# fateshelled/onnx_image_processing

Hardware: AMD Instinct MI355X
Metric: image-pairs/sec (640x480, K=512) (higher is better)
Workload: dtype f32; 1 GPU; Shi-Tomasi(3) + NMS(r=5)/top-k + sparse BAD(512, hard) + Sinkhorn(20, eps 0.05) + MNN(100, 0.1), 640x480 gray pairs, K=512 (BASELINE configs[1]); height=480, width=640, max_keypoints=512, parallelism=pair-sharded x1, input=float32 frames resident in HBM

## Files before the change

### include/mi355x_match.h

```cpp
#ifndef MI355X_MATCH_H
#define MI355X_MATCH_H

#include <stddef.h>
#include <stdint.h>

#define MI_API __attribute__((visibility("default")))

#ifdef __cplusplus
extern "C" {
#endif

typedef void *mi_stream_t;

enum {
  MI_OK = 0,
  MI_E_NULL = -1,
  MI_E_SHAPE = -2,
  MI_E_PARAM = -3,
  MI_E_CAPACITY = -4,
  MI_E_ALIGN = -5
};

enum { MI_BAD_RAW = 0, MI_BAD_SOFT = 1, MI_BAD_HARD = 2 };
enum { MI_DIST_L2 = 0, MI_DIST_L1 = 1 };
#define MI_DOTS_MIN_EPSILON 0.005
enum {
  MI_SOLVER_DEFAULT = 0,
  MI_SOLVER_MULTI_LAUNCH = 1,
  MI_SOLVER_NO_FORK = 2,
  MI_SOLVER_DOTS_BELOW_1024 = 4
};
enum {
  MI_SCHEDULE_UNDECIDED = -1,
  MI_SCHEDULE_CALLER_HELPER = 0,
  MI_SCHEDULE_TWO_HELPERS = 1,
  MI_SCHEDULE_UNSPLIT = 2
};

MI_API int mi_abi_version(void);
MI_API const char *mi_error_string(int code);
MI_API int mi_release_stream_resources(mi_stream_t stream);
MI_API int mi_sinkhorn_dots_schedule(mi_stream_t stream, int batch, int n, int m, int iterations);
MI_API int mi_sinkhorn_dots_set_schedule(mi_stream_t stream, int schedule);

MI_API int mi_corner_response(const float *image, int n, int h, int w, int block_size, float *score,
                       mi_stream_t stream);
MI_API int mi_corner_response_u8(const uint8_t *image, int n, int h, int w, int block_size, float *score,
                          mi_stream_t stream);
MI_API int mi_convert_u8_f32(const uint8_t *src, long long count, float *dst, mi_stream_t stream);
#define MI_TILE_COUNTER_BYTES 16640
MI_API int mi_corner_response_balanced(const void *image, int pixels_are_u8, int n, int h, int w, int block_size, float *score,
                                uint32_t *tile_counter, mi_stream_t stream);
MI_API int mi_corner_response_pair(const void *image_a, const void *image_b, int pixels_are_u8, int per_set, int h, int w,
                            int block_size, float *score, uint32_t *tile_counter, mi_stream_t stream);

MI_API int mi_nms_mask(const float *score, int n, int h, int w, int radius, float *mask, mi_stream_t stream);

MI_API int mi_candidate_layout(int h, int w, int *segments, int *segment_capacity);
MI_API int mi_nms_candidates(const float *score, int n, int h, int w, int radius, float score_threshold,
                      int border_margin, uint64_t *cand, uint32_t *count, mi_stream_t stream);
MI_API int mi_select_candidates(const float *score, const float *mask, int n, int h, int w,
                         float score_threshold, int border_margin, uint64_t *cand, uint32_t *count,
                         mi_stream_t stream);

MI_API int mi_topk_keypoints(const uint64_t *cand, const uint32_t *count, int segments, int segment_capacity,
                      int n, int w, int k, float *keypoints, float *kscores, mi_stream_t stream);

MI_API size_t mi_bad_plan_bytes(int num_pairs);
MI_API int mi_bad_plan_build(const uint32_t *pair_geom, const float *pair_thr, int num_pairs, void *plan,
                      mi_stream_t stream);
MI_API int mi_sparse_bad(const float *image, int n, int h, int w, const float *keypoints, int k,
                  const uint32_t *pair_geom, const float *pair_thr, int num_pairs, int mode,
                  float temperature, int normalize, float *desc, uint32_t *bits, const void *plan,
                  uint8_t *status, mi_stream_t stream);

MI_API int mi_sparse_bad_u8(const uint8_t *image, int n, int h, int w, const float *keypoints, int k,
                     const uint32_t *pair_geom, const float *pair_thr, int num_pairs, int mode,
                     float temperature, int normalize, float *desc, uint32_t *bits, const void *plan,
                     uint8_t *status, mi_stream_t stream);
MI_API int mi_sparse_bad_pair(const void *image_a, const void *image_b, int pixels_are_u8, int per_set, int h, int w,
                       const float *keypoints, int k, const uint32_t *pair_geom, const float *pair_thr, int num_pairs,
                       int mode, float temperature, int normalize, float *desc, uint32_t *bits, const void *plan,
                       uint8_t *status, mi_stream_t stream);

MI_API int mi_bad_dense(const float *image, int n, int h, int w, const uint32_t *pair_geom, const float *pair_thr,
                 int num_pairs, int mode, float temperature, float *out, mi_stream_t stream);
MI_API int mi_bad_dense_oriented(const float *image, const float *orientation, int n, int h, int w,
                          const uint32_t *pair_geom, const float *pair_thr, int num_pairs, int mode,
                          float temperature, float *out, mi_stream_t stream);
MI_API int mi_gather_descriptors(const float *descriptor_map, int batch, int d, int h, int w, const float *keypoints,
                          int nk, int bilinear, float *out, mi_stream_t stream);

MI_API int mi_angle_map(const float *image, int n, int h, int w, int patch_size, const float *moment_kernels,
                 float *angle, mi_stream_t stream);
MI_API int mi_angle_at_keypoints(const float *image, int n, int h, int w, const float *keypoints, int k,
                          int patch_size, const float *moment_kernels, float *theta, mi_stream_t stream);
MI_API int mi_angle_at_keypoints_pair(const float *image_a, const float *image_b, int per_set, int h, int w,
                               const float *keypoints, int k, int patch_size, const float *moment_kernels, float *theta,
                               mi_stream_t stream);

MI_API int mi_sparse_bad_oriented(const float *image, int n, int h, int w, const float *keypoints, int k,
                           const float *orientation_map, const float *keypoint_angles,
                           const uint32_t *pair_geom, const float *pair_thr, int num_pairs, int mode,
                           float temperature, int normalize, int bilinear, float max_reach, float *desc,
                           uint32_t *bits, uint8_t *status, mi_stream_t stream);
MI_API int mi_sparse_bad_oriented_pair(const float *image_a, const float *image_b, int per_set, int h, int w,
                                const float *keypoints, int k, const float *keypoint_angles, const uint32_t *pair_geom,
                                const float *pair_thr, int num_pairs, int mode, float temperature, int normalize,
                                int bilinear, float max_reach, float *desc, uint32_t *bits, uint8_t *status,
                                mi_stream_t stream);

MI_API int mi_cost_logscores_bits(const uint32_t *bits1, const uint32_t *bits2, int batch, int n, int m,
                           int num_bits, int normalized, double epsilon, float *z, int pitch,
                           mi_stream_t stream);
MI_API int mi_cost_logscores_f32(const float *desc1, const float *desc2, int batch, int n, int m, int d,
                          int distance, double epsilon, float *z, int pitch, mi_stream_t stream);

MI_API size_t mi_sinkhorn_workspace_bytes(int batch, int n, int m);
MI_API int mi_sinkhorn(const float *z, int batch, int n, int m, int pitch, float dustbin_logscore,
                int iterations, float *u, float *v, float *p, void *workspace, size_t workspace_bytes,
                mi_stream_t stream);

MI_API int mi_cost_dots_bits(const uint32_t *bits1, const uint32_t *bits2, int batch, int n, int m, int num_bits,
                      int normalized, uint16_t *dots, int pitch, float *row_info, float *col_info,
                      mi_stream_t stream);
MI_API size_t mi_sinkhorn_dots_workspace_bytes(int batch, int n, int m);
MI_API int mi_sinkhorn_dots(const uint16_t *dots, const float *row_info, const float *col_info, int batch, int n,
                     int m, int pitch, double epsilon, double unused_score, double sqnorm_bound, int iterations,
                     float *u, float *v, float *p, void *workspace, size_t workspace_bytes, int flags,
                     mi_stream_t stream);
MI_API const uint32_t *mi_sinkhorn_dots_status_word(const void *workspace, int batch, int n, int m);

MI_API int mi_match_filters(float *p, int batch, int n, int m, float ratio_threshold, float dustbin_margin,
                     uint8_t *valid, mi_stream_t stream);
MI_API int mi_match_filter_masks(const float *p, int batch, int n, int m, int has_dustbin, float ratio_threshold,
                          float dustbin_margin, uint8_t *valid, mi_stream_t stream);

MI_API int mi_mnn_extract(const float *p, int batch, int n, int m, const float *kpts1, const float *kpts2,
                   int max_matches, float threshold, uint64_t *row_best, uint64_t *col_best,
                   float *mk1, float *mk2, float *scores, uint8_t *valid, int32_t *match_ij,
                   mi_stream_t stream);

MI_API size_t mi_mnn_duals_workspace_bytes(int batch, int n, int m);
MI_API int mi_mnn_from_duals(const float *z, int batch, int n, int m, int pitch, const float *u, const float *v,
                      const float *kpts1, const float *kpts2, int max_matches, float threshold, void *workspace,
                      size_t workspace_bytes, float *mk1, float *mk2, float *scores, uint8_t *valid,
                      int32_t *match_ij, mi_stream_t stream);
MI_API int mi_mnn_from_duals_dots(const uint16_t *dots, const float *row_info, const float *col_info, int batch, int n,
                           int m, int pitch, double epsilon, const float *u, const float *v, const float *kpts1,
                           const float *kpts2, int max_matches, float threshold, void *workspace,
                           size_t workspace_bytes, const uint32_t *solver_status, float *mk1, float *mk2,
                           float *scores, uint8_t *valid, int32_t *match_ij, mi_stream_t stream);

MI_API int mi_akaze_diffuse(const float *l_in, int n, int h, int w, float kappa, float dt, float *l_out,
                     mi_stream_t stream);
#define MI_AKAZE_KAPPA_MIN 1e-3f
#define MI_AKAZE_KAPPA_MAX 1e6f
MI_API int mi_akaze_scale_fused(int iterations, int nms_size);
MI_API int mi_akaze_scale(const float *l_in, int n, int h, int w, int iterations, float kappa, float dt, float threshold,
                   int nms_size, float *l_out, float *scores, float *tmp, mi_stream_t stream);
MI_API int mi_akaze_scale_sets(const float *l_in_a, const float *l_in_b, int per_set, int h, int w, int iterations,
                        float kappa, float dt, float threshold, int nms_size, float *l_out, float *scores, float *tmp,
                        mi_stream_t stream);
MI_API int mi_akaze_scale_select(const float *l_in, int n, int h, int w, int iterations, float kappa, float dt,
                          float threshold, int nms_size, float *l_out, const float *prev_scores, int num_prev,
                          float *best, uint8_t *attain, float *tmp, mi_stream_t stream);
MI_API int mi_akaze_orientation_from_attain(const uint8_t *attain, const float *scale_theta, int num_scales, int n, int h,
                                     int w, const float *keypoints, int k, float *theta, mi_stream_t stream);
MI_API int mi_akaze_orientation_select(const float *scale_images, size_t scale_stride, int num_scales,
                                const uint8_t *attain, int n, int h, int w, const float *keypoints, int k,
                                int patch_size, const float *moment_kernels, float *theta, mi_stream_t stream);
MI_API int mi_akaze_hessian_scores(const float *l, int n, int h, int w, float threshold, int nms_size, float *scores,
                            mi_stream_t stream);
MI_API int mi_akaze_combine(const float *scale_scores, const float *scale_orientations, int num_scales, int n, int h,
                     int w, float *scores, float *orientations, mi_stream_t stream);
MI_API int mi_akaze_orientation_at_keypoints(const float *scale_scores, const float *scale_theta, int num_scales,
                                      int n, int h, int w, const float *keypoints, int k, float *theta,
                                      mi_stream_t stream);

MI_API int mi_core_maxima(const float *p, int batch, int n, int m, float *row_max, float *col_max, mi_stream_t stream);

MI_API int mi_normalise_keypoints(const float *keypoints, long long count, const float *k_inv, float *points,
                           mi_stream_t stream);

MI_API size_t mi_essential_matrix_workspace_bytes(int batch, int n, int m, int top_k);
MI_API int mi_essential_matrix(const float *p, int batch, int n, int m, const float *pts1, const float *pts2,
                        const uint8_t *valid1, const uint8_t *valid2, int top_k, int n_iter,
                        int n_iter_manifold, float *e, void *workspace, size_t workspace_bytes, mi_stream_t stream);
MI_API int mi_essential_matrix_dots(const uint16_t *dots, const float *row_info, const float *col_info, int pitch,
                             double epsilon, const float *u, const float *v, int batch, int n, int m,
                             const float *pts1, const float *pts2, const uint8_t *valid1, const uint8_t *valid2,
                             int top_k, int n_iter, int n_iter_manifold, float *e, void *workspace,
                             size_t workspace_bytes, mi_stream_t stream);

MI_API int mi_fast_score(const float *image, int n, int h, int w, float threshold, float *score, mi_stream_t stream);
MI_API int mi_dog_responses(const float *image, int n, int h, int w, const float *weights_1d, int num_scales,
                     int kernel_size, float *out, float *score, mi_stream_t stream);

typedef struct mi_match_params {
  int block_size;
  int nms_radius;
  int max_keypoints;
  float score_threshold;
  int border_margin;
  int num_pairs;
  const uint32_t *pair_geom;
  const float *pair_thr;
  const void *bad_plan;
  int normalize_descriptors;
  double epsilon;
  double unused_score;
  int sinkhorn_iterations;
  int max_matches;
  float match_threshold;
  int flags;
} mi_match_params;
MI_API size_t mi_match_pairs_workspace_bytes(int batch, int h, int w, const mi_match_params *params);
MI_API int mi_match_pairs(const float *image1, const float *image2, int batch, int h, int w,
                   const mi_match_params *params, float *keypoints1, float *keypoints2, float *matched1,
                   float *matched2, float *match_scores, uint8_t *match_valid, int32_t *match_ij,
                   void *workspace, size_t workspace_bytes, mi_stream_t stream);

MI_API int mi_match_pairs_u8(const uint8_t *image1, const uint8_t *image2, int batch, int h, int w,
                      const mi_match_params *params, float *keypoints1, float *keypoints2, float *matched1,
                      float *matched2, float *match_scores, uint8_t *match_valid, int32_t *match_ij,
                      void *workspace, size_t workspace_bytes, mi_stream_t stream);

MI_API size_t mi_voxel_downsample_workspace_bytes(int batch, int64_t total, int d);
MI_API int mi_voxel_downsample(const float *points, const int64_t *offsets, int batch, int64_t total, int d,
                               const float *leaf, float *out_points, uint8_t *out_mask, int64_t *out_counts,
                               void *workspace, size_t workspace_bytes, mi_stream_t stream);

MI_API int mi_depth_to_points(const void *depth, int depth_is_u16, int batch, int h, int w, const float *u_tab,
                              const float *v_tab, float z_scale, float *out_points, float *out_normals,
                              mi_stream_t stream);

MI_API int mi_depth_align(const void *depth, int depth_is_u16, int batch, int h, int w, const float *u_tab,
                          const float *v_tab, float z_scale, float rgb_cx, float rgb_cy, float rgb_fx, float rgb_fy,
                          const float *rotation, const float *translation, float *out, mi_stream_t stream);

enum { MI_PIX_U8 = 0, MI_PIX_U16 = 1, MI_PIX_I32 = 2, MI_PIX_F32 = 3 };
#define MI_THRESHOLD_MAX_BINS 65536
#define MI_THRESHOLD_MAX_CLASSES 5

MI_API int mi_histogram(const void *frames, int dtype, int batch, long long pixels, int min_val, int bins, int64_t *hist,
                        mi_stream_t stream);

MI_API int mi_otsu_threshold(const int64_t *hist, int batch, int bins, int min_val, int32_t *thresh, mi_stream_t stream);

MI_API size_t mi_multi_otsu_workspace_bytes(int batch, int bins, int n_class);
MI_API int mi_multi_otsu_threshold(const int64_t *hist, int batch, int bins, int min_val, int n_class, int32_t *thresholds,
                                   void *workspace, size_t workspace_bytes, mi_stream_t stream);

MI_API int mi_threshold_apply(const void *frames, int dtype, int batch, long long pixels, const int32_t *thresholds,
                              int n_thresh, int out_dtype, int binary, int low, int high, void *out, mi_stream_t stream);

#define MI_POSE_MAX_N 2048
#define MI_POSE_MAX_HYPOTHESES 65536
#define MI_POSE_MAX_REFINE_ROUNDS 8

MI_API int mi_essential_hypotheses(const float *pts1, const float *pts2, const uint8_t *valid, int batch, int n,
                                   int num_hypotheses, float threshold, uint32_t seed, float *e_h, float *cost,
                                   int32_t *count, mi_stream_t stream);

MI_API int mi_essential_refit(const float *pts1, const float *pts2, const uint8_t *mask, int batch, int n, float *e,
                              uint8_t *ok, mi_stream_t stream);

MI_API size_t mi_essential_ransac_workspace_bytes(int batch, int n, int num_hypotheses);
MI_API int mi_essential_ransac(const float *pts1, const float *pts2, const uint8_t *valid, int batch, int n,
                               int num_hypotheses, float threshold, int refine_rounds, uint32_t seed, float *e,
                               uint8_t *inlier, int32_t *best_h, int32_t *count, void *workspace, size_t workspace_bytes,
                               mi_stream_t stream);

MI_API int mi_recover_pose(const float *e, const float *pts1, const float *pts2, const uint8_t *mask, int batch, int n,
                           float distance_threshold, float *r, float *t, uint8_t *pose_mask, int32_t *count, uint8_t *ok,
                           mi_stream_t stream);

MI_API int mi_triangulate(const float *proj1, const float *proj2, const float *pts1, const float *pts2, int batch, int n,
                          float *points, uint8_t *finite, mi_stream_t stream);

enum { MI_INGEST_BGR = 0, MI_INGEST_RGB = 1 };
#define MI_INGEST_MAX_DIM 16384
MI_API int mi_ingest_frames(const uint8_t *src, int batch, int src_h, int src_w, int channels, long long row_pitch,
                            long long frame_pitch, int channel_order, void *dst, int dst_is_f32, int h, int w,
                            mi_stream_t stream);

#define MI_RIGID_MAX_N 2048

MI_API int mi_lift_keypoints(const float *keypoints, const void *depth, int depth_is_u16, int batch, int n, int h, int w,
                             const float *k_inv, float z_scale, float min_depth, float max_depth, const uint8_t *valid_in,
                             float *points, uint8_t *valid, mi_stream_t stream);

MI_API int mi_rigid_hypotheses(const float *pts1, const float *pts2, const uint8_t *valid, int batch, int n,
                               int num_hypotheses, float threshold, uint32_t seed, float *rt_h, float *cost, int32_t *count,
                               mi_stream_t stream);

MI_API int mi_rigid_refit(const float *pts1, const float *pts2, const uint8_t *mask, int batch, int n, float *r, float *t,
                          uint8_t *ok, mi_stream_t stream);

MI_API size_t mi_rigid_ransac_workspace_bytes(int batch, int n, int num_hypotheses);
MI_API int mi_rigid_ransac(const float *pts1, const float *pts2, const uint8_t *valid, int batch, int n, int num_hypotheses,
                           float threshold, int refine_rounds, uint32_t seed, float *r, float *t, uint8_t *inlier,
                           int32_t *best_h, int32_t *count, float *rmse, uint8_t *ok, void *workspace, size_t workspace_bytes,
                           mi_stream_t stream);

#define MI_ICP_MAX_STAGES 4
#define MI_ICP_MAX_ITERATIONS 64

MI_API int mi_surfel_maps(const void *depth, int depth_is_u16, int batch, int h, int w, const float *k_inv, float z_scale,
                          float min_depth, float max_depth, float normal_max_jump, float *vertex_out, float *normal_out,
                          mi_stream_t stream);

MI_API size_t mi_icp_workspace_bytes(int batch, int h, int w);

MI_API int mi_icp_linearise(const float *vertex1, const float *normal1, const float *vertex2, const float *normal2,
                            const float *r, const float *t, int batch, int h, int w, float fx, float fy, float cx, float cy,
                            int stride, float distance_threshold, float angle_threshold, double *sums, void *workspace,
                            size_t workspace_bytes, mi_stream_t stream);

MI_API int mi_icp_refine(const float *vertex1, const float *normal1, const float *vertex2, const float *normal2,
                         const float *r0, const float *t0, int batch, int h, int w, float fx, float fy, float cx, float cy,
                         const int32_t *strides, const int32_t *iterations, int stages, float distance_threshold,
                         float angle_threshold, int min_correspondences, float *r, float *t, float *information, float *rmse,
                         int32_t *count, int32_t *steps, uint8_t *ok, void *workspace, size_t workspace_bytes,
                         mi_stream_t stream);


MI_API int mi_intensity_maps(const void *gray, int gray_is_u8, int batch, int h, int w, float *intensity_out, mi_stream_t stream);

MI_API size_t mi_rgbd_workspace_bytes(int batch, int h, int w);

MI_API int mi_photo_linearise(const float *vertex1, const float *intensity1, const float *vertex2, const float *intensity2,
                              const float *r, const float *t, int batch, int h, int w, float fx, float fy, float cx, float cy,
                              int stride, float distance_threshold, float intensity_threshold, double *sums, void *workspace,
                              size_t workspace_bytes, mi_stream_t stream);

MI_API int mi_rgbd_refine(const float *vertex1, const float *normal1, const float *intensity1, const float *vertex2,
                          const float *normal2, const float *intensity2, const float *r0, const float *t0, int batch, int h,
                          int w, float fx, float fy, float cx, float cy, const int32_t *strides, const int32_t *iterations,
                          int stages, float distance_threshold, float angle_threshold, float photo_weight,
                          float intensity_threshold, int min_correspondences, float *r, float *t, float *information,
                          float *rmse, int32_t *count, float *rmse_photo, int32_t *count_photo, int32_t *steps, uint8_t *ok,
                          void *workspace, size_t workspace_bytes, mi_stream_t stream);


MI_API int mi_tsdf_reset(float *volume, int batch, int nz, int ny, int nx, mi_stream_t stream);

MI_API int mi_tsdf_integrate(float *volume, int batch, int nz, int ny, int nx, float origin_x, float origin_y, float origin_z,
                             float voxel_size, float truncation, float max_weight, const void *depth, int depth_is_u16, int frames,
                             int h, int w, float fx, float fy, float cx, float cy, float z_scale, float min_depth, float max_depth,
                             const float *r, const float *t, const uint8_t *active, mi_stream_t stream);

MI_API int mi_tsdf_raycast(const float *volume, int batch, int nz, int ny, int nx, float origin_x, float origin_y, float origin_z,
                           float voxel_size, float truncation, float step_fraction, const float *r, const float *t, int h, int w,
                           const float *k_inv, float min_depth, float max_depth, float *vertex_out, float *normal_out,
                           mi_stream_t stream);

MI_API int mi_pose_compose(const float *ra, const float *ta, const float *rb, const float *tb, int batch, float *r, float *t,
                           mi_stream_t stream);


MI_API size_t mi_tsdf_surface_workspace_bytes(int batch, int nz, int ny, int nx);

MI_API int mi_tsdf_surface(const float *volume, int batch, int nz, int ny, int nx, float origin_x, float origin_y, float origin_z,
                           float voxel_size, float min_weight, int max_vertices, int max_triangles, float *vertex_out,
                           float *normal_out, int32_t *triangle_out, int32_t *counts_out, void *workspace, size_t workspace_bytes,
                           mi_stream_t stream);


MI_API int mi_tsdf_gray_reset(float *intensity_volume, int batch, int nz, int ny, int nx, mi_stream_t stream);

MI_API int mi_tsdf_integrate_gray(float *volume, float *intensity_volume, int batch, int nz, int ny, int nx, float origin_x,
                                  float origin_y, float origin_z, float voxel_size, float truncation, float max_weight,
                                  const void *depth, int depth_is_u16, const void *gray, int gray_is_u8, int frames, int h, int w,
                                  float fx, float fy, float cx, float cy, float z_scale, float min_depth, float max_depth,
                                  const float *r, const float *t, const uint8_t *active, mi_stream_t stream);

MI_API int mi_tsdf_sample_gray(const float *intensity_volume, int batch, int nz, int ny, int nx, float origin_x, float origin_y,
                               float origin_z, float voxel_size, const float *points, int n, const float *r, const float *t,
                               float *intensity_out, mi_stream_t stream);

#define MI_PNP_MAX_N 2048

MI_API int mi_pnp_hypotheses(const float *pts3, const float *pts2, const uint8_t *valid, int batch, int n, int num_hypotheses,
                             float threshold, uint32_t seed, float *rt_h, float *cost, int32_t *count, mi_stream_t stream);

MI_API int mi_pnp_refit(const float *pts3, const float *pts2, const uint8_t *mask, const float *r0, const float *t0, int batch,
                        int n, float *r, float *t, float *info, uint8_t *ok, mi_stream_t stream);

MI_API size_t mi_pnp_ransac_workspace_bytes(int batch, int n, int num_hypotheses);
MI_API int mi_pnp_ransac(const float *pts3, const float *pts2, const uint8_t *valid, int batch, int n, int num_hypotheses,
                         float threshold, int refine_rounds, uint32_t seed, float *r, float *t, uint8_t *inlier,
                         int32_t *best_h, int32_t *count, float *rmse, float *info, uint8_t *ok, void *workspace,
                         size_t workspace_bytes, mi_stream_t stream);

#ifdef __cplusplus
}
#endif
#endif
```

### onnx_image_processing_amd/_native.py

```python
from __future__ import annotations

import ctypes
import os
from ctypes import c_char_p, c_double, c_float, c_int, c_size_t, c_uint32, c_void_p

import torch

_PKG = os.path.dirname(os.path.abspath(__file__))
LIB_PATH = os.environ.get("MI355X_MATCH_LIB") or os.path.join(_PKG, "lib", "libmi355x_match.so")

SIGNATURES = {
    "mi_abi_version": [],
    "mi_sinkhorn_dots_schedule": [c_void_p, c_int, c_int, c_int, c_int],
    "mi_sinkhorn_dots_set_schedule": [c_void_p, c_int],
    "mi_error_string": [c_int],
    "mi_release_stream_resources": [c_void_p],
    "mi_corner_response": [c_void_p, c_int, c_int, c_int, c_int, c_void_p, c_void_p],
    "mi_corner_response_u8": [c_void_p, c_int, c_int, c_int, c_int, c_void_p, c_void_p],
    "mi_convert_u8_f32": [c_void_p, ctypes.c_longlong, c_void_p, c_void_p],
    "mi_corner_response_balanced": [c_void_p, c_int, c_int, c_int, c_int, c_int, c_void_p, c_void_p, c_void_p],
    "mi_corner_response_pair": [c_void_p, c_void_p, c_int, c_int, c_int, c_int, c_int, c_void_p, c_void_p, c_void_p],
    "mi_nms_mask": [c_void_p, c_int, c_int, c_int, c_int, c_void_p, c_void_p],
    "mi_candidate_layout": [c_int, c_int, ctypes.POINTER(c_int), ctypes.POINTER(c_int)],
    "mi_nms_candidates": [c_void_p, c_int, c_int, c_int, c_int, c_float, c_int, c_void_p, c_void_p, c_void_p],
    "mi_select_candidates": [c_void_p, c_void_p, c_int, c_int, c_int, c_float, c_int, c_void_p, c_void_p, c_void_p],
    "mi_topk_keypoints": [c_void_p, c_void_p, c_int, c_int, c_int, c_int, c_int, c_void_p, c_void_p, c_void_p],
    "mi_bad_plan_bytes": [c_int],
    "mi_bad_plan_build": [c_void_p, c_void_p, c_int, c_void_p, c_void_p],
    "mi_sparse_bad": [c_void_p, c_int, c_int, c_int, c_void_p, c_int, c_void_p, c_void_p, c_int, c_int, c_float, c_int,
                      c_void_p, c_void_p, c_void_p, c_void_p, c_void_p],
    "mi_sparse_bad_u8": [c_void_p, c_int, c_int, c_int, c_void_p, c_int, c_void_p, c_void_p, c_int, c_int, c_float, c_int,
                         c_void_p, c_void_p, c_void_p, c_void_p, c_void_p],
    "mi_sparse_bad_pair": [c_void_p, c_void_p, c_int, c_int, c_int, c_int, c_void_p, c_int, c_void_p, c_void_p, c_int, c_int,
                           c_float, c_int, c_void_p, c_void_p, c_void_p, c_void_p, c_void_p],
    "mi_bad_dense": [c_void_p, c_int, c_int, c_int, c_void_p, c_void_p, c_int, c_int, c_float, c_void_p, c_void_p],
    "mi_bad_dense_oriented": [c_void_p, c_void_p, c_int, c_int, c_int, c_void_p, c_void_p, c_int, c_int, c_float, c_void_p,
                              c_void_p],
    "mi_gather_descriptors": [c_void_p, c_int, c_int, c_int, c_int, c_void_p, c_int, c_int, c_void_p, c_void_p],
    "mi_angle_map": [c_void_p, c_int, c_int, c_int, c_int, c_void_p, c_void_p, c_void_p],
    "mi_angle_at_keypoints": [c_void_p, c_int, c_int, c_int, c_void_p, c_int, c_int, c_void_p, c_void_p, c_void_p],
    "mi_sparse_bad_oriented": [c_void_p, c_int, c_int, c_int, c_void_p, c_int, c_void_p, c_void_p, c_void_p, c_void_p,
                               c_int, c_int, c_float, c_int, c_int, c_float, c_void_p, c_void_p, c_void_p, c_void_p],
    "mi_angle_at_keypoints_pair": [c_void_p, c_void_p, c_int, c_int, c_int, c_void_p, c_int, c_int, c_void_p, c_void_p,
                                   c_void_p],
    "mi_sparse_bad_oriented_pair": [c_void_p, c_void_p, c_int, c_int, c_int, c_void_p, c_int, c_void_p, c_void_p, c_void_p,
                                    c_int, c_int, c_float, c_int, c_int, c_float, c_void_p, c_void_p, c_void_p, c_void_p],
    "mi_cost_logscores_bits": [c_void_p, c_void_p, c_int, c_int, c_int, c_int, c_int, c_double, c_void_p, c_int, c_void_p],
    "mi_cost_logscores_f32": [c_void_p, c_void_p, c_int, c_int, c_int, c_int, c_int, c_double, c_void_p, c_int, c_void_p],
    "mi_sinkhorn_workspace_bytes": [c_int, c_int, c_int],
    "mi_sinkhorn": [c_void_p, c_int, c_int, c_int, c_int, c_float, c_int, c_void_p, c_void_p, c_void_p, c_void_p,
                    c_size_t, c_void_p],
    "mi_cost_dots_bits": [c_void_p, c_void_p, c_int, c_int, c_int, c_int, c_int, c_void_p, c_int, c_void_p, c_void_p,
                          c_void_p],
    "mi_sinkhorn_dots_workspace_bytes": [c_int, c_int, c_int],
    "mi_sinkhorn_dots": [c_void_p, c_void_p, c_void_p, c_int, c_int, c_int, c_int, c_double, c_double, c_double, c_int,
                         c_void_p, c_void_p, c_void_p, c_void_p, c_size_t, c_int, c_void_p],
    "mi_sinkhorn_dots_status_word": [c_void_p, c_int, c_int, c_int],
    "mi_match_filters": [c_void_p, c_int, c_int, c_int, c_float, c_float, c_void_p, c_void_p],
    "mi_match_filter_masks": [c_void_p, c_int, c_int, c_int, c_int, c_float, c_float, c_void_p, c_void_p],
    "mi_mnn_extract": [c_void_p, c_int, c_int, c_int, c_void_p, c_void_p, c_int, c_float, c_void_p, c_void_p,
                       c_void_p, c_void_p, c_void_p, c_void_p, c_void_p, c_void_p],
    "mi_mnn_duals_workspace_bytes": [c_int, c_int, c_int],
    "mi_mnn_from_duals": [c_void_p, c_int, c_int, c_int, c_int, c_void_p, c_void_p, c_void_p, c_void_p, c_int, c_float,
                          c_void_p, c_size_t, c_void_p, c_void_p, c_void_p, c_void_p, c_void_p, c_void_p],
    "mi_mnn_from_duals_dots": [c_void_p, c_void_p, c_void_p, c_int, c_int, c_int, c_int, c_double, c_void_p, c_void_p,
                               c_void_p, c_void_p, c_int, c_float, c_void_p, c_size_t, c_void_p, c_void_p, c_void_p,
                               c_void_p, c_void_p, c_void_p, c_void_p],
    "mi_core_maxima": [c_void_p, c_int, c_int, c_int, c_void_p, c_void_p, c_void_p],
    "mi_normalise_keypoints": [c_void_p, ctypes.c_longlong, c_void_p, c_void_p, c_void_p],
    "mi_essential_matrix_workspace_bytes": [c_int, c_int, c_int, c_int],
    "mi_essential_matrix": [c_void_p, c_int, c_int, c_int, c_void_p, c_void_p, c_void_p, c_void_p, c_int, c_int, c_int,
                            c_void_p, c_void_p, c_size_t, c_void_p],
    "mi_essential_matrix_dots": [c_void_p, c_void_p, c_void_p, c_int, c_double, c_void_p, c_void_p, c_int, c_int, c_int,
                                 c_void_p, c_void_p, c_void_p, c_void_p, c_int, c_int, c_int, c_void_p, c_void_p, c_size_t,
                                 c_void_p],
    "mi_fast_score": [c_void_p, c_int, c_int, c_int, c_float, c_void_p, c_void_p],
    "mi_dog_responses": [c_void_p, c_int, c_int, c_int, c_void_p, c_int, c_int, c_void_p, c_void_p, c_void_p],
    "mi_akaze_diffuse": [c_void_p, c_int, c_int, c_int, c_float, c_float, c_void_p, c_void_p],
    "mi_akaze_scale_fused": [c_int, c_int],
    "mi_akaze_scale": [c_void_p, c_int, c_int, c_int, c_int, c_float, c_float, c_float, c_int, c_void_p, c_void_p, c_void_p,
                       c_void_p],
    "mi_akaze_scale_sets": [c_void_p, c_void_p, c_int, c_int, c_int, c_int, c_float, c_float, c_float, c_int, c_void_p, c_void_p,
                            c_void_p, c_void_p],
    "mi_akaze_scale_select": [c_void_p, c_int, c_int, c_int, c_int, c_float, c_float, c_float, c_int, c_void_p, c_void_p,
                              c_int, c_void_p, c_void_p, c_void_p, c_void_p],
    "mi_akaze_orientation_from_attain": [c_void_p, c_void_p, c_int, c_int, c_int, c_int, c_void_p, c_int, c_void_p,
                                         c_void_p],
    "mi_akaze_orientation_select": [c_void_p, c_size_t, c_int, c_void_p, c_int, c_int, c_int, c_void_p, c_int, c_int,
                                    c_void_p, c_void_p, c_void_p],
    "mi_akaze_hessian_scores": [c_void_p, c_int, c_int, c_int, c_float, c_int, c_void_p, c_void_p],
    "mi_akaze_combine": [c_void_p, c_void_p, c_int, c_int, c_int, c_int, c_void_p, c_void_p, c_void_p],
    "mi_akaze_orientation_at_keypoints": [c_void_p, c_void_p, c_int, c_int, c_int, c_int, c_void_p, c_int, c_void_p,
                                          c_void_p],
    "mi_voxel_downsample_workspace_bytes": [c_int, ctypes.c_int64, c_int],
    "mi_voxel_downsample": [c_void_p, c_void_p, c_int, ctypes.c_int64, c_int, c_void_p, c_void_p, c_void_p, c_void_p,
                            c_void_p, c_size_t, c_void_p],
    "mi_depth_to_points": [c_void_p, c_int, c_int, c_int, c_int, c_void_p, c_void_p, c_float, c_void_p, c_void_p, c_void_p],
    "mi_depth_align": [c_void_p, c_int, c_int, c_int, c_int, c_void_p, c_void_p, c_float, c_float, c_float, c_float, c_float,
                       c_void_p, c_void_p, c_void_p, c_void_p],
    "mi_histogram": [c_void_p, c_int, c_int, ctypes.c_longlong, c_int, c_int, c_void_p, c_void_p],
    "mi_otsu_threshold": [c_void_p, c_int, c_int, c_int, c_void_p, c_void_p],
    "mi_multi_otsu_workspace_bytes": [c_int, c_int, c_int],
    "mi_multi_otsu_threshold": [c_void_p, c_int, c_int, c_int, c_int, c_void_p, c_void_p, c_size_t, c_void_p],
    "mi_threshold_apply": [c_void_p, c_int, c_int, ctypes.c_longlong, c_void_p, c_int, c_int, c_int, c_int, c_int, c_void_p,
                           c_void_p],
    "mi_essential_hypotheses": [c_void_p, c_void_p, c_void_p, c_int, c_int, c_int, c_float, c_uint32, c_void_p, c_void_p,
                                c_void_p, c_void_p],
    "mi_essential_refit": [c_void_p, c_void_p, c_void_p, c_int, c_int, c_void_p, c_void_p, c_void_p],
    "mi_essential_ransac_workspace_bytes": [c_int, c_int, c_int],
    "mi_essential_ransac": [c_void_p, c_void_p, c_void_p, c_int, c_int, c_int, c_float, c_int, c_uint32, c_void_p, c_void_p,
                            c_void_p, c_void_p, c_void_p, c_size_t, c_void_p],
    "mi_recover_pose": [c_void_p, c_void_p, c_void_p, c_void_p, c_int, c_int, c_float, c_void_p, c_void_p, c_void_p, c_void_p,
                        c_void_p, c_void_p],
    "mi_triangulate": [c_void_p, c_void_p, c_void_p, c_void_p, c_int, c_int, c_void_p, c_void_p, c_void_p],
    "mi_ingest_frames": [c_void_p, c_int, c_int, c_int, c_int, ctypes.c_longlong, ctypes.c_longlong, c_int, c_void_p, c_int,
                         c_int, c_int, c_void_p],
    "mi_lift_keypoints": [c_void_p, c_void_p, c_int, c_int, c_int, c_int, c_int, c_void_p, c_float, c_float, c_float, c_void_p,
                          c_void_p, c_void_p, c_void_p],
    "mi_rigid_hypotheses": [c_void_p, c_void_p, c_void_p, c_int, c_int, c_int, c_float, c_uint32, c_void_p, c_void_p, c_void_p,
                            c_void_p],
    "mi_rigid_refit": [c_void_p, c_void_p, c_void_p, c_int, c_int, c_void_p, c_void_p, c_void_p, c_void_p],
    "mi_rigid_ransac_workspace_bytes": [c_int, c_int, c_int],
    "mi_rigid_ransac": [c_void_p, c_void_p, c_void_p, c_int, c_int, c_int, c_float, c_int, c_uint32, c_void_p, c_void_p, c_void_p,
                        c_void_p, c_void_p, c_void_p, c_void_p, c_void_p, c_size_t, c_void_p],
    "mi_pnp_hypotheses": [c_void_p, c_void_p, c_void_p, c_int, c_int, c_int, c_float, c_uint32, c_void_p, c_void_p, c_void_p,
                          c_void_p],
    "mi_pnp_refit": [c_void_p, c_void_p, c_void_p, c_void_p, c_void_p, c_int, c_int, c_void_p, c_void_p, c_void_p, c_void_p,
                     c_void_p],
    "mi_pnp_ransac_workspace_bytes": [c_int, c_int, c_int],
    "mi_pnp_ransac": [c_void_p, c_void_p, c_void_p, c_int, c_int, c_int, c_float, c_int, c_uint32, c_void_p, c_void_p, c_void_p,
                      c_void_p, c_void_p, c_void_p, c_void_p, c_void_p, c_void_p, c_size_t, c_void_p],
    "mi_surfel_maps": [c_void_p, c_int, c_int, c_int, c_int, c_void_p, c_float, c_float, c_float, c_float, c_void_p, c_void_p,
                       c_void_p],
    "mi_icp_workspace_bytes": [c_int, c_int, c_int],
    "mi_icp_linearise": [c_void_p, c_void_p, c_void_p, c_void_p, c_void_p, c_void_p, c_int, c_int, c_int, c_float, c_float,
                         c_float, c_float, c_int, c_float, c_float, c_void_p, c_void_p, c_size_t, c_void_p],
    "mi_icp_refine": [c_void_p, c_void_p, c_void_p, c_void_p, c_void_p, c_void_p, c_int, c_int, c_int, c_float, c_float, c_float,
                      c_float, c_void_p, c_void_p, c_int, c_float, c_float, c_int, c_void_p, c_void_p, c_void_p, c_void_p,
                      c_void_p, c_void_p, c_void_p, c_void_p, c_size_t, c_void_p],
    "mi_intensity_maps": [c_void_p, c_int, c_int, c_int, c_int, c_void_p, c_void_p],
    "mi_rgbd_workspace_bytes": [c_int, c_int, c_int],
    "mi_photo_linearise": [c_void_p, c_void_p, c_void_p, c_void_p, c_void_p, c_void_p, c_int, c_int, c_int, c_float, c_float,
                           c_float, c_float, c_int, c_float, c_float, c_void_p, c_void_p, c_size_t, c_void_p],
    "mi_rgbd_refine": [c_void_p, c_void_p, c_void_p, c_void_p, c_void_p, c_void_p, c_void_p, c_void_p, c_int, c_int, c_int,
                       c_float, c_float, c_float, c_float, c_void_p, c_void_p, c_int, c_float, c_float, c_float, c_float, c_int,
                       c_void_p, c_void_p, c_void_p, c_void_p, c_void_p, c_void_p, c_void_p, c_void_p, c_void_p, c_void_p,
                       c_size_t, c_void_p],
    "mi_tsdf_reset": [c_void_p, c_int, c_int, c_int, c_int, c_void_p],
    "mi_tsdf_integrate": [c_void_p, c_int, c_int, c_int, c_int, c_float, c_float, c_float, c_float, c_float, c_float, c_void_p,
                          c_int, c_int, c_int, c_int, c_float, c_float, c_float, c_float, c_float, c_float, c_float, c_void_p,
                          c_void_p, c_void_p, c_void_p],
    "mi_tsdf_raycast": [c_void_p, c_int, c_int, c_int, c_int, c_float, c_float, c_float, c_float, c_float, c_float, c_void_p,
                        c_void_p, c_int, c_int, c_void_p, c_float, c_float, c_void_p, c_void_p, c_void_p],
    "mi_pose_compose": [c_void_p, c_void_p, c_void_p, c_void_p, c_int, c_void_p, c_void_p, c_void_p],
    "mi_tsdf_surface_workspace_bytes": [c_int, c_int, c_int, c_int],
    "mi_tsdf_surface": [c_void_p, c_int, c_int, c_int, c_int, c_float, c_float, c_float, c_float, c_float, c_int, c_int, c_void_p,
                        c_void_p, c_void_p, c_void_p, c_void_p, c_size_t, c_void_p],
    "mi_tsdf_gray_reset": [c_void_p, c_int, c_int, c_int, c_int, c_void_p],
    "mi_tsdf_integrate_gray": [c_void_p, c_void_p, c_int, c_int, c_int, c_int, c_float, c_float, c_float, c_float, c_float, c_float,
                               c_void_p, c_int, c_void_p, c_int, c_int, c_int, c_int, c_float, c_float, c_float, c_float, c_float,
                               c_float, c_float, c_void_p, c_void_p, c_void_p, c_void_p],
    "mi_tsdf_sample_gray": [c_void_p, c_int, c_int, c_int, c_int, c_float, c_float, c_float, c_float, c_void_p, c_int, c_void_p,
                            c_void_p, c_void_p, c_void_p],
}


class MatchParams(ctypes.Structure):
    _fields_ = [("block_size", c_int), ("nms_radius", c_int), ("max_keypoints", c_int), ("score_threshold", c_float),
                ("border_margin", c_int), ("num_pairs", c_int), ("pair_geom", c_void_p), ("pair_thr", c_void_p),
                ("bad_plan", c_void_p), ("normalize_descriptors", c_int), ("epsilon", c_double),
                ("unused_score", c_double), ("sinkhorn_iterations", c_int), ("max_matches", c_int),
                ("match_threshold", c_float), ("flags", c_int)]


SIGNATURES["mi_match_pairs_workspace_bytes"] = [c_int, c_int, c_int, ctypes.POINTER(MatchParams)]
SIGNATURES["mi_match_pairs"] = [c_void_p, c_void_p, c_int, c_int, c_int, ctypes.POINTER(MatchParams), c_void_p, c_void_p,
                                c_void_p, c_void_p, c_void_p, c_void_p, c_void_p, c_void_p, c_size_t, c_void_p]
DEBUG_SIGNATURES = {"mi_debug_set": [c_int, c_int], "mi_debug_topk_stamps": [c_void_p], "mi_debug_clock_probe": [c_void_p],
                    "mi_debug_bad_plan_passes": [c_void_p, c_int, ctypes.POINTER(c_int), ctypes.POINTER(c_int)],
                    "mi_debug_sinkhorn_dots_form": [c_int, c_int, c_int, c_int, c_int, c_int],
                    "mi_debug_tuner_script": [c_int, ctypes.POINTER(c_int), ctypes.POINTER(c_int), ctypes.POINTER(ctypes.c_double), ctypes.POINTER(c_int)],
                    "mi_debug_akaze_math_check": [c_int, c_float, c_uint32, c_uint32, c_void_p, c_void_p, c_void_p]}
SIGNATURES["mi_match_pairs_u8"] = SIGNATURES["mi_match_pairs"]
_RESTYPE = {"mi_essential_matrix_workspace_bytes": c_size_t, "mi_sinkhorn_dots_status_word": c_void_p, "mi_match_pairs_workspace_bytes": c_size_t, "mi_error_string": c_char_p, "mi_sinkhorn_workspace_bytes": c_size_t, "mi_bad_plan_bytes": c_size_t,
            "mi_sinkhorn_dots_workspace_bytes": c_size_t, "mi_mnn_duals_workspace_bytes": c_size_t,
            "mi_voxel_downsample_workspace_bytes": c_size_t, "mi_multi_otsu_workspace_bytes": c_size_t,
            "mi_essential_ransac_workspace_bytes": c_size_t, "mi_rigid_ransac_workspace_bytes": c_size_t,
            "mi_pnp_ransac_workspace_bytes": c_size_t,
            "mi_icp_workspace_bytes": c_size_t, "mi_rgbd_workspace_bytes": c_size_t, "mi_tsdf_surface_workspace_bytes": c_size_t}

MI_BAD_RAW, MI_BAD_SOFT, MI_BAD_HARD = 0, 1, 2
MI_DIST_L2, MI_DIST_L1 = 0, 1
MI_PIX_U8, MI_PIX_U16, MI_PIX_I32, MI_PIX_F32 = 0, 1, 2, 3
MI_INGEST_BGR, MI_INGEST_RGB = 0, 1

DEBUG_LIB_PATH = os.path.join(_PKG, "lib", "libmi355x_match_debug.so")

_lib = None
_product = None
_debug = None


def _open(path: str, signatures: dict) -> ctypes.CDLL:
    if not os.path.exists(path):
        raise RuntimeError(
            f"{path} not found: the HIP library is not built. Run "
            "`python -m onnx_image_processing_amd.build` (there is no CPU fallback)."
        )
    lib = ctypes.CDLL(path)
    for name, argtypes in signatures.items():
        fn = getattr(lib, name)
        fn.argtypes = argtypes
        fn.restype = _RESTYPE.get(name, c_int)
    return lib


def load() -> ctypes.CDLL:
    global _lib, _product
    if _lib is None:
        if _product is None:
            _product = _open(LIB_PATH, SIGNATURES)
        _lib = _product
    return _lib


class debug_library:

    def __enter__(self) -> ctypes.CDLL:
        global _lib, _debug
        load()
        if _debug is None:
            _debug = _open(DEBUG_LIB_PATH, {**SIGNATURES, **DEBUG_SIGNATURES})
        self._outer = _lib
        _lib = _debug
        return _debug

    def __exit__(self, *exc) -> None:
        global _lib
        _debug.mi_debug_set(0, 0)
        _lib = self._outer


def use_debug_library() -> ctypes.CDLL:
    return debug_library().__enter__()


def check(code: int, what: str) -> None:
    if code != 0:
        msg = load().mi_error_string(code)
        raise RuntimeError(f"{what} failed ({code}): {msg.decode() if msg else '?'}")


def stream_ptr() -> int:
    return torch.cuda.current_stream().cuda_stream


def dev(t: torch.Tensor, dtype: torch.dtype, what: str) -> int:
    if not t.is_cuda:
        raise RuntimeError(
            f"{what} must live on the GPU (got device {t.device}); this package has no CPU path"
        )
    if t.dtype != dtype:
        raise RuntimeError(f"{what} must be {dtype}, got {t.dtype}")
    if not t.is_contiguous():
        raise RuntimeError(f"{what} must be contiguous")
    return t.data_ptr()


_timers: dict | None = None


_timed_names = None


def enable_timing(on: bool, only=None) -> None:
    global _timers, _timed_names
    _timers = {} if on else None
    _timed_names = set(only) if (on and only) else None


def timings_ms() -> dict:
    torch.cuda.synchronize()
    return {k: [s.elapsed_time(e) for s, e in v] for k, v in (_timers or {}).items()}


def call(name: str, *args) -> None:
    fn = getattr(load(), name)
    if _timers is None or (_timed_names is not None and name not in _timed_names):
        check(fn(*args), name)
        return
    start, end = torch.cuda.Event(enable_timing=True), torch.cuda.Event(enable_timing=True)
    start.record()
    rc = fn(*args)
    end.record()
    check(rc, name)
    _timers.setdefault(name, []).append((start, end))
```

### onnx_image_processing_amd/csrc/common.h

```cpp
#pragma once
#include <hip/hip_runtime.h>
#include <stdint.h>

#include "../../include/mi355x_match.h"

#define MI_WAVE 64

#define MI_ENTER() (void)hipGetLastError()
static inline int mi_launch_status() {
  hipError_t e = hipGetLastError();
  return e == hipSuccess ? MI_OK : (int)e;
}
#define MI_CHECK_LAUNCH()                          \
  do {                                             \
    const int _mi_e = mi_launch_status();          \
    if (_mi_e != MI_OK) return _mi_e;              \
  } while (0)

static inline int ceil_div(int a, int b) { return (a + b - 1) / b; }

template <typename W>
static __global__ __launch_bounds__(256) void mi_zero_kernel(W *__restrict__ p, size_t n) {
  const size_t i = (size_t)blockIdx.x * 256 + threadIdx.x;
  if (i < n) p[i] = W{};
}
static inline int mi_zero_async(void *p, size_t bytes, hipStream_t s) {
  if (bytes == 0) return MI_OK;
  if (((uintptr_t)p % 4) != 0 || bytes % 4 != 0) return MI_E_ALIGN;
  if (((uintptr_t)p % 16) == 0 && bytes % 16 == 0) {
    const size_t n = bytes / 16;
    hipLaunchKernelGGL(mi_zero_kernel<uint4>, dim3((unsigned)((n + 255) / 256)), dim3(256), 0, s, reinterpret_cast<uint4 *>(p), n);
  } else {
    const size_t n = bytes / 4;
    hipLaunchKernelGGL(mi_zero_kernel<uint32_t>, dim3((unsigned)((n + 255) / 256)), dim3(256), 0, s, reinterpret_cast<uint32_t *>(p), n);
  }
  return mi_launch_status();
}

struct MiSets {
  const void *a;
  const void *b;
  int per_set;
};
static inline MiSets mi_one_set(const void *p, int n) { return MiSets{p, nullptr, n}; }
template <typename T>
__device__ __forceinline__ const T *mi_set_item(const MiSets &s, int i, size_t item_elems) {
  const bool second = i >= s.per_set;
  return static_cast<const T *>(second ? s.b : s.a) + (size_t)(second ? i - s.per_set : i) * item_elems;
}

__device__ __forceinline__ int clampi(int v, int lo, int hi) { return v < lo ? lo : (v > hi ? hi : v); }

__device__ __forceinline__ unsigned xcd_contiguous_id(unsigned bid, unsigned nblocks) {
  const unsigned q = nblocks >> 3, r = nblocks & 7u;
  const unsigned xcd = bid & 7u, k = bid >> 3;
  const unsigned base = (xcd < r) ? xcd * (q + 1u) : r * (q + 1u) + (xcd - r) * q;
  return base + k;
}

#define MI_DPP(old, src, ctrl, rmask) \
  __builtin_bit_cast(float, __builtin_amdgcn_update_dpp(__builtin_bit_cast(int, old), __builtin_bit_cast(int, src), ctrl, rmask, 0xf, false))
__device__ __forceinline__ float wave_max_dpp(float v) {
  v = fmaxf(v, MI_DPP(v, v, 0xB1, 0xf));
  v = fmaxf(v, MI_DPP(v, v, 0x4E, 0xf));
  v = fmaxf(v, MI_DPP(v, v, 0x141, 0xf));
  v = fmaxf(v, MI_DPP(v, v, 0x140, 0xf));
  v = fmaxf(v, MI_DPP(v, v, 0x142, 0xa));
  v = fmaxf(v, MI_DPP(v, v, 0x143, 0xc));
  return __builtin_bit_cast(float, __builtin_amdgcn_readlane(__builtin_bit_cast(int, v), 63));
}
__device__ __forceinline__ float wave_sum_dpp(float v) {
  v += MI_DPP(0.0f, v, 0xB1, 0xf);
  v += MI_DPP(0.0f, v, 0x4E, 0xf);
  v += MI_DPP(0.0f, v, 0x141, 0xf);
  v += MI_DPP(0.0f, v, 0x140, 0xf);
  v += MI_DPP(0.0f, v, 0x142, 0xa);
  v += MI_DPP(0.0f, v, 0x143, 0xc);
  return __builtin_bit_cast(float, __builtin_amdgcn_readlane(__builtin_bit_cast(int, v), 63));
}

#define MI_SWAP32(a, b, ra, rb)                                                                              \
  {                                                                                                           \
    auto _r = __builtin_amdgcn_permlane32_swap(__builtin_bit_cast(unsigned, a), __builtin_bit_cast(unsigned, b), \
                                               false, false);                                                \
    const unsigned _r0 = _r[0], _r1 = _r[1];  \
    ra = __builtin_bit_cast(float, _r0);                                                                      \
    rb = __builtin_bit_cast(float, _r1);                                                                      \
  }
#define MI_SWAP16(a, b, ra, rb)                                                                              \
  {                                                                                                           \
    auto _r = __builtin_amdgcn_permlane16_swap(__builtin_bit_cast(unsigned, a), __builtin_bit_cast(unsigned, b), \
                                               false, false);                                                \
    const unsigned _r0 = _r[0], _r1 = _r[1];                                                                  \
    ra = __builtin_bit_cast(float, _r0);                                                                      \
    rb = __builtin_bit_cast(float, _r1);                                                                      \
  }
__device__ __forceinline__ float mi_readlane_f(float v, int lane) {
  return __builtin_bit_cast(float, __builtin_amdgcn_readlane(__builtin_bit_cast(int, v), lane));
}
__device__ __forceinline__ void wave_max4(float *v) {
  float a0, a1, b0, b1, c0, c1;
  MI_SWAP32(v[0], v[1], a0, a1);
  MI_SWAP32(v[2], v[3], b0, b1);
  const float m01 = fmaxf(a0, a1), m23 = fmaxf(b0, b1);
  MI_SWAP16(m01, m23, c0, c1);
  float m = fmaxf(c0, c1);
  m = fmaxf(m, MI_DPP(m, m, 0xB1, 0xf));
  m = fmaxf(m, MI_DPP(m, m, 0x4E, 0xf));
  m = fmaxf(m, MI_DPP(m, m, 0x141, 0xf));
  m = fmaxf(m, MI_DPP(m, m, 0x140, 0xf));
  v[0] = mi_readlane_f(m, 0);
  v[2] = mi_readlane_f(m, 16);
  v[1] = mi_readlane_f(m, 32);
  v[3] = mi_readlane_f(m, 48);
}
#define MI_ROW_OF_GROUP(g) ((g) == 1 ? 2 : (g) == 2 ? 1 : (g))
__device__ __forceinline__ float wave_sum4_rows(const float *v) {
  float a0, a1, b0, b1, c0, c1;
  MI_SWAP32(v[0], v[1], a0, a1);
  MI_SWAP32(v[2], v[3], b0, b1);
  const float m01 = a0 + a1, m23 = b0 + b1;
  MI_SWAP16(m01, m23, c0, c1);
  float m = c0 + c1;
  m += MI_DPP(0.0f, m, 0xB1, 0xf);
  m += MI_DPP(0.0f, m, 0x4E, 0xf);
  m += MI_DPP(0.0f, m, 0x141, 0xf);
  m += MI_DPP(0.0f, m, 0x140, 0xf);
  return m;
}
__device__ __forceinline__ void wave_sum4(float *v) {
  float a0, a1, b0, b1, c0, c1;
  MI_SWAP32(v[0], v[1], a0, a1);
  MI_SWAP32(v[2], v[3], b0, b1);
  const float m01 = a0 + a1, m23 = b0 + b1;
  MI_SWAP16(m01, m23, c0, c1);
  float m = c0 + c1;
  m += MI_DPP(0.0f, m, 0xB1, 0xf);
  m += MI_DPP(0.0f, m, 0x4E, 0xf);
  m += MI_DPP(0.0f, m, 0x141, 0xf);
  m += MI_DPP(0.0f, m, 0x140, 0xf);
  v[0] = mi_readlane_f(m, 0);
  v[2] = mi_readlane_f(m, 16);
  v[1] = mi_readlane_f(m, 32);
  v[3] = mi_readlane_f(m, 48);
}

__device__ __forceinline__ float mi_prob_exp(float t) { return __builtin_amdgcn_exp2f(t * 1.4426950408889634f); }

__device__ __forceinline__ float mi_z_from_dot(float dot, float2 row, float2 col, float neg_inv_eps) {
  return __builtin_fmaf(dot * col.x, -2.0f * neg_inv_eps * row.x, col.y * neg_inv_eps) + row.y * neg_inv_eps;
}

__device__ __forceinline__ float wave_max(float v) {
#pragma unroll
  for (int o = 32; o > 0; o >>= 1) v = fmaxf(v, __shfl_xor(v, o, 64));
  return v;
}
__device__ __forceinline__ float wave_sum(float v) {
#pragma unroll
  for (int o = 32; o > 0; o >>= 1) v += __shfl_xor(v, o, 64);
  return v;
}

static inline bool mi_akaze_kappa_ok(float kappa) { return kappa >= MI_AKAZE_KAPPA_MIN && kappa <= MI_AKAZE_KAPPA_MAX; }
#define MI_AKAZE_STREAM_MAX_PREV 3
int mi_akaze_stream_supported(int h, int w, int iterations, int nms_size, const void *l_in, const void *l_out,
                              const void *scores);
int mi_akaze_scale_stream(const float *l_in, const float *l_in_b, int per_set, int n, int h, int w, int iterations, float kappa, float dt, float threshold,
                          int nms_size, float *l_out, float *scores, int mode, const float *prev_scores, int num_prev,
                          uint8_t *attain, mi_stream_t stream);

int mi_corner_response_sets(MiSets images, int pix_u8, int n, int h, int w, int block_size, float *score,
                            unsigned *tile_ctr, mi_stream_t stream);
int mi_topk_keypoints_sets(const uint64_t *cand, const uint32_t *count, int segments, int segment_capacity, int n, int w,
                           int k, MiSets keypoints, float *kscores, mi_stream_t stream);
int mi_sparse_bad_sets(MiSets images, int pix_u8, int n, int h, int w, MiSets keypoints, int k, const uint32_t *pair_geom,
                       const float *pair_thr, int num_pairs, int mode, float temperature, int normalize, float *desc,
                       uint32_t *bits, const void *plan, uint8_t *status, mi_stream_t stream);
int mi_cost_dots_bits_zeroing(const uint32_t *bits1, const uint32_t *bits2, int batch, int n, int m, int num_bits,
                              int normalized, uint16_t *dots, int pitch, float *row_info, float *col_info,
                              void *zero_ptr, size_t zero_bytes, mi_stream_t stream);
size_t mi_sinkhorn_dots_handoff_region(void *workspace, int batch, int n, int m, int flags, void **region);
int mi_sinkhorn_dots_impl(const uint16_t *dots, const float *row_info, const float *col_info, int batch, int n, int m,
                          int pitch, double epsilon, double unused_score, double sqnorm_bound, int iterations, float *u,
                          float *v, float *p, void *workspace, size_t workspace_bytes, int flags, int prezeroed,
                          mi_stream_t stream);

struct MiFork {
  int parts;
  hipStream_t stream[2];
  void *handle;
  int trial_entry, trial, first_side;
};
int mi_fork_begin(hipStream_t s, int batch, int n, int m, int key, MiFork *f);
int mi_fork_end(hipStream_t s, MiFork *f);
```

### onnx_image_processing_amd/csrc/mnn.hip

```cpp
#include "common.h"
#include "hooks.h"

#include <math.h>

namespace {

constexpr int MX_THREADS = 1024;
constexpr int MX_MAX = 4096;

__device__ __forceinline__ uint64_t best_key(float p, uint32_t idx) {
  return ((uint64_t)__float_as_uint(p) << 32) | (uint64_t)(0xFFFFFFFFu - idx);
}
__device__ __forceinline__ uint64_t wave_max_u64(uint64_t k) {
#pragma unroll
  for (int o = 32; o > 0; o >>= 1) {
    const uint64_t other = __shfl_xor(k, o, 64);
    k = other > k ? other : k;
  }
  return k;
}

__global__ __launch_bounds__(256) void mnn_row_kernel(const float *__restrict__ p, int n, int m,
                                                      uint64_t *__restrict__ row_best) {
  const int lane = threadIdx.x & 63, wave = threadIdx.x >> 6;
  const int b = blockIdx.y, i = blockIdx.x * 4 + wave;
  if (i >= n) return;
  const float *pr = p + ((size_t)b * (n + 1) + i) * (size_t)(m + 1);
  uint64_t k = 0ull;
  for (int j = lane; j < m; j += 64) {
    const uint64_t c = best_key(pr[j], (uint32_t)j);
    k = c > k ? c : k;
  }
  k = wave_max_u64(k);
  if (lane == 0) row_best[(size_t)b * n + i] = k;
}

__global__ __launch_bounds__(256) void mnn_col_kernel(const float *__restrict__ p, int n, int m,
                                                      uint64_t *__restrict__ col_best) {
  __shared__ uint64_t red[4][64];
  const int lane = threadIdx.x & 63, wave = threadIdx.x >> 6;
  const int b = blockIdx.y, j = blockIdx.x * 64 + lane;
  const float *pb = p + (size_t)b * (n + 1) * (size_t)(m + 1);
  uint64_t k = 0ull;
  if (j < m) {
    for (int i = wave; i < n; i += 4) {
      const uint64_t c = best_key(pb[(size_t)i * (m + 1) + j], (uint32_t)i);
      k = c > k ? c : k;
    }
  }
  red[wave][lane] = k;
  __syncthreads();
  if (wave == 0 && j < m) {
    for (int w = 1; w < 4; ++w) k = red[w][lane] > k ? red[w][lane] : k;
    col_best[(size_t)b * m + j] = k;
  }
}

template <int Q>
__global__ __launch_bounds__(512) void mnn_p_kernel(const float *__restrict__ p, int n, int m, uint64_t *__restrict__ row_best,
                                                    unsigned long long *__restrict__ col_best) {
  constexpr int NW = 8, RW = 4;
  __shared__ uint64_t red[NW][Q * 64];
  const int lane = threadIdx.x & 63, wave = __builtin_amdgcn_readfirstlane(threadIdx.x >> 6);
  const int b = blockIdx.y, row0 = ((int)blockIdx.x * NW + wave) * RW;
  float x[RW][Q];
#pragma unroll
  for (int r = 0; r < RW; ++r) {
    const float *pr = p + ((size_t)b * (n + 1) + min(row0 + r, n - 1)) * (size_t)(m + 1);
#pragma unroll
    for (int q = 0; q < Q; ++q) x[r][q] = pr[min(q * 64 + lane, m - 1)];
  }
  float cbest[Q];
  int cidx[Q];
#pragma unroll
  for (int q = 0; q < Q; ++q) { cbest[q] = -1.0f; cidx[q] = 0; }
#pragma unroll
  for (int r = 0; r < RW; ++r) {
    const int i = row0 + r;
    const bool live = i < n;
    float rbest = -1.0f;
    int rj = 0;
#pragma unroll
    for (int q = 0; q < Q; ++q) {
      const int j = q * 64 + lane;
      const float v = (live && j < m) ? x[r][q] : -1.0f;
      if (v > rbest) { rbest = v; rj = j; }
      if (v > cbest[q]) { cbest[q] = v; cidx[q] = i; }
    }
    uint64_t key = rbest >= 0.0f ? best_key(rbest, (uint32_t)rj) : 0ull;
    key = wave_max_u64(key);
    if (lane == 0 && live) row_best[(size_t)b * n + i] = key;
  }
#pragma unroll
  for (int q = 0; q < Q; ++q) red[wave][q * 64 + lane] = cbest[q] >= 0.0f ? best_key(cbest[q], (uint32_t)cidx[q]) : 0ull;
  __syncthreads();
  for (int c = threadIdx.x; c < Q * 64 && c < m; c += 64 * NW) {
    uint64_t k = red[0][c];
#pragma unroll
    for (int w = 1; w < NW; ++w) k = red[w][c] > k ? red[w][c] : k;
    if (k != 0ull) atomicMax(col_best + (size_t)b * m + c, (unsigned long long)k);
  }
}

__global__ __launch_bounds__(MX_THREADS) void mnn_select_kernel(
    int n, int m, const uint64_t *__restrict__ row_best, const uint64_t *__restrict__ col_best,
    const uint64_t *__restrict__ col_part, int nb,
    const float *__restrict__ kpts1, const float *__restrict__ kpts2, int max_matches, float threshold,
    const uint32_t *__restrict__ solver_status,
    float *__restrict__ mk1, float *__restrict__ mk2, float *__restrict__ scores,
    uint8_t *__restrict__ valid, int32_t *__restrict__ match_ij) {
  __shared__ uint64_t keys[MX_MAX];
  const bool dead = solver_status && *solver_status != 0u;
  __shared__ uint64_t cmerged[1024];
  const int t = threadIdx.x, b = blockIdx.x;
  const uint64_t *rb = row_best + (size_t)b * n;
  const uint64_t *cb = col_best + (size_t)b * m;
  if (col_part) {
    for (int j = t; j < m; j += MX_THREADS) {
      uint64_t k = 0ull;
      int band = 0;
      for (; band + 8 <= nb; band += 8) {
        uint64_t c[8];
#pragma unroll
        for (int q = 0; q < 8; ++q) c[q] = col_part[((size_t)b * nb + band + q) * m + j];
#pragma unroll
        for (int q = 0; q < 8; ++q) k = c[q] > k ? c[q] : k;
      }
      for (; band < nb; ++band) {
        const uint64_t c = col_part[((size_t)b * nb + band) * m + j];
        k = c > k ? c : k;
      }
      cmerged[j] = k;
    }
    __syncthreads();
    cb = cmerged;
  }
  int npad = 2;
  while (npad < n) npad <<= 1;
  for (int i = t; i < npad; i += MX_THREADS) {
    uint64_t key = 0ull;
    if (i < n) {
      const uint64_t r = rb[i];
      const uint32_t jw = 0xFFFFFFFFu - (uint32_t)(r & 0xFFFFFFFFull);
      const bool has = r != 0ull && jw < (uint32_t)m;
      const uint32_t j = has ? jw : 0u;
      const float val = __uint_as_float((uint32_t)(r >> 32));
      const uint32_t ib = 0xFFFFFFFFu - (uint32_t)(cb[j] & 0xFFFFFFFFull);
      const bool ok = has && !dead && (ib == (uint32_t)i) && (val >= threshold);
      key = ((uint64_t)(ok ? (uint32_t)(r >> 32) + 1u : 0u) << 32) | (uint64_t)(0xFFFFFFFFu - (uint32_t)i);
    }
    keys[i] = key;
  }
  __syncthreads();
  const uint64_t *sorted = keys;
  if (npad >= 128 && npad <= MX_THREADS) {
    uint64_t *ordered = keys + MX_THREADS;
    uint32_t *above_of = reinterpret_cast<uint32_t *>(keys + 2 * MX_THREADS);
    const int tpk = MX_THREADS / npad, slice = npad / tpk;
    const int ki = t & (npad - 1), part = t / npad;
    if (t < npad) { above_of[t] = 0u; ordered[t] = 0ull; }
    const uint64_t mine = keys[ki];
    uint32_t above = 0;
    if (mine != 0ull) {
      const ulonglong2 *lst = reinterpret_cast<const ulonglong2 *>(keys + part * slice);
#pragma unroll 8
      for (int j = 0; j < slice / 2; ++j) {
        const ulonglong2 two = lst[j];
        above += (two.x > mine ? 1u : 0u) + (two.y > mine ? 1u : 0u);
      }
    }
    __syncthreads();
    if (mine != 0ull && above) atomicAdd(&above_of[ki], above);
    __syncthreads();
    if (part == 0 && mine != 0ull) ordered[above_of[ki]] = mine;
    __syncthreads();
    sorted = ordered;
  } else {
    for (int size = 2; size <= npad; size <<= 1) {
      for (int stride = size >> 1; stride > 0; stride >>= 1) {
        for (int i = t; i < (npad >> 1); i += MX_THREADS) {
          const int pos = 2 * i - (i & (stride - 1));
          const int par = pos + stride;
          const bool desc = ((pos & size) == 0);
          const uint64_t a = keys[pos], c = keys[par];
          if ((a < c) == desc) { keys[pos] = c; keys[par] = a; }
        }
        __syncthreads();
      }
    }
  }
  const int cnt = max_matches < n ? max_matches : n;
  for (int s = t; s < max_matches; s += MX_THREADS) {
    float sc = 0.0f;
    uint32_t i = 0;
    bool matched = false;
    if (s < cnt) {
      const uint64_t key = sorted[s];
      i = 0xFFFFFFFFu - (uint32_t)(key & 0xFFFFFFFFull);
      const uint32_t hi = (uint32_t)(key >> 32);
      matched = hi != 0u;
      sc = matched ? __uint_as_float(hi - 1u) : -1.0f;
    }
    const uint32_t jw = 0xFFFFFFFFu - (uint32_t)(rb[i] & 0xFFFFFFFFull);
    const uint32_t j = jw < (uint32_t)m ? jw : 0u;
    const size_t o = (size_t)b * max_matches + s;
    mk1[o * 2 + 0] = kpts1[((size_t)b * n + i) * 2 + 0];
    mk1[o * 2 + 1] = kpts1[((size_t)b * n + i) * 2 + 1];
    mk2[o * 2 + 0] = kpts2[((size_t)b * m + j) * 2 + 0];
    mk2[o * 2 + 1] = kpts2[((size_t)b * m + j) * 2 + 1];
    scores[o] = sc;
    const bool ok = sc > 0.0f;
    valid[o] = ok ? 1 : 0;
    if (match_ij) {
      match_ij[o * 2 + 0] = ok ? (int32_t)i : -1;
      match_ij[o * 2 + 1] = ok ? (int32_t)j : -1;
    }
  }
}

struct ZSourceF32 {
  const float *z;
  int pitch;
  struct Raw { float4 a, c; };
  struct Row {};
  __device__ __forceinline__ Raw load_raw(int b, int n, int i, int j, int m) const {
    const float *src = z + ((size_t)b * n + i) * pitch + j;
    Raw r;
    r.a = make_float4(0.f, 0.f, 0.f, 0.f);
    r.c = r.a;
    if (j < m) r.a = *reinterpret_cast<const float4 *>(src);
    if (j + 4 < m) r.c = *reinterpret_cast<const float4 *>(src + 4);
    return r;
  }
  __device__ __forceinline__ void decode(const Raw &r, float (&out)[8]) const {
    out[0] = r.a.x; out[1] = r.a.y; out[2] = r.a.z; out[3] = r.a.w;
    out[4] = r.c.x; out[5] = r.c.y; out[6] = r.c.z; out[7] = r.c.w;
  }
  __device__ __forceinline__ Row load_row(int, int, int) const { return Row(); }
  __device__ __forceinline__ void begin_row(const Row &) {}
  __device__ __forceinline__ float col(int, int) const { return 0.0f; }
  __device__ __forceinline__ void finish(float (&)[8], const float2 (&)[8]) const {}
};

struct ZSourceDots {
  const uint16_t *dots;
  int pitch;
  const float2 *row_info, *col_info;
  float neg_inv_eps;
  float2 ri;
  typedef uint4 Raw;
  typedef float2 Row;
  __device__ __forceinline__ Raw load_raw(int b, int n, int i, int j, int m) const {
    return *reinterpret_cast<const uint4 *>(dots + ((size_t)b * n + i) * pitch + min(j, pitch - 8));
  }
  __device__ __forceinline__ void decode(const Raw &r, float (&out)[8]) const {
    const uint32_t w[4] = {r.x, r.y, r.z, r.w};
#pragma unroll
    for (int q = 0; q < 8; ++q) out[q] = (float)((q & 1) ? (w[q >> 1] >> 16) : (w[q >> 1] & 0xFFFFu));
  }
  __device__ __forceinline__ Row load_row(int b, int n, int i) const { return row_info[(size_t)b * n + i]; }
  __device__ __forceinline__ void begin_row(const Row &r) { ri = r; }
  __device__ __forceinline__ void finish(float (&x)[8], const float2 (&ci)[8]) const {
#pragma unroll
    for (int q = 0; q < 8; ++q) x[q] = mi_z_from_dot(x[q], ri, ci[q], neg_inv_eps);
  }
};

template <typename SRC, int E8, int RW, int NW, bool FULL = false, bool SPLIT = false>
__global__ __launch_bounds__(64 * NW) __attribute__((amdgpu_waves_per_eu(SPLIT ? 8 : 1, 8))) void mnn_band_kernel(SRC src, int n, int m, const float *__restrict__ u,
                                                           const float *__restrict__ v,
                                                           const float2 *__restrict__ col_info,
                                                           uint64_t *__restrict__ row_best,
                                                           uint64_t *__restrict__ col_part) {
  static_assert(!SPLIT || (E8 == 1 && NW % 2 == 0), "the split form runs the one-chunk code on wave pairs");
  constexpr int RG = SPLIT ? NW / 2 : NW;
  constexpr int BAND = RG * RW;
  constexpr int NC = 512 * E8 * (SPLIT ? 2 : 1);
  __shared__ uint64_t red[RG][NC];
  __shared__ uint64_t halfkey[SPLIT ? NW : 1][RW];
  const int lane = threadIdx.x & 63, wave = __builtin_amdgcn_readfirstlane(threadIdx.x >> 6);
  const int b = blockIdx.y, band = blockIdx.x, nb = gridDim.x;
  const int rg = SPLIT ? wave >> 1 : wave, half = SPLIT ? wave & 1 : 0, cbase = half * 512;
  const int row0 = band * BAND + rg * RW;

  typename SRC::Raw raw[RW][E8];
  typename SRC::Row rowd[RW];
  float uis[RW];
#pragma unroll
  for (int r = 0; r < RW; ++r) {
    const int ic = min(row0 + r, n - 1);
    uis[r] = u[(size_t)b * (n + 1) + ic];
    rowd[r] = src.load_row(b, n, ic);
#pragma unroll
    for (int e = 0; e < E8; ++e) raw[r][e] = src.load_raw(b, n, ic, cbase + e * 512 + lane * 8, m);
  }
  __shared__ float s_v[NC];
  __shared__ float2 s_ci[NC];
  {
    constexpr int PER = NC / (64 * NW);
    float tv[PER];
    float2 tc[PER];
#pragma unroll
    for (int q = 0; q < PER; ++q) {
      const int c = threadIdx.x + q * 64 * NW;
      tv[q] = c < m ? v[(size_t)b * (m + 1) + c] : 0.0f;
      tc[q] = (col_info && c < m) ? col_info[(size_t)b * m + c] : make_float2(0.f, 0.f);
    }
#pragma unroll
    for (int q = 0; q < PER; ++q) {
      const int c = threadIdx.x + q * 64 * NW;
      s_v[c] = tv[q];
      s_ci[c] = tc[q];
    }
  }
  __syncthreads();
  float vv[E8][8];
  float2 ci[E8][8];
#pragma unroll
  for (int e = 0; e < E8; ++e)
#pragma unroll
    for (int q = 0; q < 8; ++q) {
      vv[e][q] = s_v[cbase + e * 512 + lane * 8 + q];
      ci[e][q] = s_ci[cbase + e * 512 + lane * 8 + q];
    }

  float cbest[E8][8];
  int cidx[E8][8];
#pragma unroll
  for (int e = 0; e < E8; ++e)
#pragma unroll
    for (int q = 0; q < 8; ++q) { cbest[e][q] = -1.0f; cidx[e][q] = 0; }

#pragma unroll
  for (int r = 0; r < RW; ++r) {
    const int i = row0 + r;
    const bool live = i < n;
    const float ui = uis[r];
    src.begin_row(rowd[r]);
    float rbest = -1.0f;
    int rj = 0;
#pragma unroll
    for (int e = 0; e < E8; ++e) {
      float x[8];
      src.decode(raw[r][e], x);
      src.finish(x, ci[e]);
#pragma unroll
      for (int q = 0; q < 8; ++q) {
        const int j = cbase + e * 512 + lane * 8 + q;
        float p = mi_prob_exp((x[q] + ui) + vv[e][q]);
        if constexpr (!FULL) p = (live && j < m) ? p : -1.0f;
        if (p > rbest) { rbest = p; rj = j; }
        if (p > cbest[e][q]) { cbest[e][q] = p; cidx[e][q] = i; }
      }
    }
    uint64_t key = rbest >= 0.0f ? best_key(rbest, (uint32_t)rj) : 0ull;
    key = wave_max_u64(key);
    if constexpr (SPLIT) {
      if (lane == 0) halfkey[wave][r] = key;
    } else {
      if (lane == 0 && live) row_best[(size_t)b * n + i] = key;
    }
  }
#pragma unroll
  for (int e = 0; e < E8; ++e)
#pragma unroll
    for (int q = 0; q < 8; ++q)
      red[rg][cbase + e * 512 + lane * 8 + q] = cbest[e][q] >= 0.0f ? best_key(cbest[e][q], (uint32_t)cidx[e][q]) : 0ull;
  __syncthreads();
  if constexpr (SPLIT) {
    if (half == 0 && lane < RW && row0 + lane < n) {
      const uint64_t a = halfkey[wave][lane], c = halfkey[wave + 1][lane];
      row_best[(size_t)b * n + row0 + lane] = c > a ? c : a;
    }
  }
  for (int c = threadIdx.x; c < NC && c < m; c += 64 * NW) {
    uint64_t k = red[0][c];
#pragma unroll
    for (int w = 1; w < RG; ++w) k = red[w][c] > k ? red[w][c] : k;
    col_part[((size_t)b * nb + band) * m + c] = k;
  }
}

__global__ __launch_bounds__(256) void mnn_colmerge_kernel(const uint64_t *__restrict__ col_part, int nb, int m,
                                                           uint64_t *__restrict__ col_best) {
  const int b = blockIdx.y, j = blockIdx.x * 256 + threadIdx.x;
  if (j >= m) return;
  uint64_t k = 0ull;
  int band = 0;
  for (; band + 8 <= nb; band += 8) {
    uint64_t c[8];
#pragma unroll
    for (int q = 0; q < 8; ++q) c[q] = col_part[((size_t)b * nb + band + q) * m + j];
#pragma unroll
    for (int q = 0; q < 8; ++q) k = c[q] > k ? c[q] : k;
  }
  for (; band < nb; ++band) {
    const uint64_t c = col_part[((size_t)b * nb + band) * m + j];
    k = c > k ? c : k;
  }
  col_best[(size_t)b * m + j] = k;
}

constexpr int DUALS_BAND = 32;

struct DualsWork {
  uint64_t *row_best, *col_best, *col_part;
};
size_t duals_bytes(int batch, int n, int m) {
  return ((size_t)batch * n + (size_t)batch * m + (size_t)batch * ceil_div(n, DUALS_BAND) * m) * sizeof(uint64_t);
}
DualsWork duals_carve(void *workspace, int batch, int n, int m) {
  DualsWork w;
  w.row_best = reinterpret_cast<uint64_t *>(workspace);
  w.col_best = w.row_best + (size_t)batch * n;
  w.col_part = w.col_best + (size_t)batch * m;
  return w;
}

template <typename SRC>
int mnn_from_source(SRC src, const float2 *col_info, int batch, int n, int m, const float *u, const float *v,
                    const float *kpts1, const float *kpts2, int max_matches, float threshold, void *workspace,
                    size_t workspace_bytes, const uint32_t *solver_status, float *mk1, float *mk2, float *scores,
                    uint8_t *valid, int32_t *match_ij, hipStream_t s) {
  if (!u || !v || !kpts1 || !kpts2 || !workspace || !mk1 || !mk2 || !scores || !valid) return MI_E_NULL;
  if (batch <= 0 || n <= 0 || m <= 0 || batch > 65535) return MI_E_SHAPE;
  if (n > MX_MAX || m > 1024 || max_matches <= 0) return MI_E_PARAM;
  if (((uintptr_t)workspace % 8) != 0) return MI_E_ALIGN;
  if (workspace_bytes < duals_bytes(batch, n, m)) return MI_E_CAPACITY;
  const DualsWork w = duals_carve(workspace, batch, n, m);
  const int nb = ceil_div(n, DUALS_BAND);
  const bool full = n % DUALS_BAND == 0;
  if (m == 512 && full) {
    hipLaunchKernelGGL((mnn_band_kernel<SRC, 1, 4, 8, true>), dim3(nb, batch), dim3(512), 0, s, src, n, m, u, v, col_info,
                       w.row_best, w.col_part);
  } else if (m <= 512) {
    hipLaunchKernelGGL((mnn_band_kernel<SRC, 1, 4, 8>), dim3(nb, batch), dim3(512), 0, s, src, n, m, u, v, col_info,
                       w.row_best, w.col_part);
  } else if (MI_HOOK(mnn_pair_waves, 1) == 0) {
    hipLaunchKernelGGL((mnn_band_kernel<SRC, 2, 4, 8>), dim3(nb, batch), dim3(512), 0, s, src, n, m, u, v, col_info,
                       w.row_best, w.col_part);
  } else if (m == 1024 && full) {
    hipLaunchKernelGGL((mnn_band_kernel<SRC, 1, 4, 16, true, true>), dim3(nb, batch), dim3(1024), 0, s, src, n, m, u, v,
                       col_info, w.row_best, w.col_part);
  } else {
    hipLaunchKernelGGL((mnn_band_kernel<SRC, 1, 4, 16, false, true>), dim3(nb, batch), dim3(1024), 0, s, src, n, m, u, v,
                       col_info, w.row_best, w.col_part);
  }
  if (batch <= 32) {
    hipLaunchKernelGGL(mnn_select_kernel, dim3(batch), dim3(MX_THREADS), 0, s, n, m, w.row_best, w.col_best,
                       (const uint64_t *)w.col_part, nb, kpts1, kpts2, max_matches, threshold, solver_status, mk1, mk2,
                       scores, valid, match_ij);
    return mi_launch_status();
  }
  hipLaunchKernelGGL(mnn_colmerge_kernel, dim3(ceil_div(m, 256), batch), dim3(256), 0, s, w.col_part, nb, m,
                     w.col_best);
  hipLaunchKernelGGL(mnn_select_kernel, dim3(batch), dim3(MX_THREADS), 0, s, n, m, w.row_best, w.col_best,
                     (const uint64_t *)nullptr, 0, kpts1, kpts2, max_matches, threshold, solver_status, mk1, mk2, scores,
                     valid, match_ij);
  return mi_launch_status();
}

}

extern "C" size_t mi_mnn_duals_workspace_bytes(int batch, int n, int m) {
  if (batch <= 0 || n <= 0 || m <= 0 || m > 1024 || n > MX_MAX) return 0;
  return duals_bytes(batch, n, m);
}

extern "C" int mi_mnn_from_duals(const float *z, int batch, int n, int m, int pitch, const float *u, const float *v,
                                 const float *kpts1, const float *kpts2, int max_matches, float threshold,
                                 void *workspace, size_t workspace_bytes, float *mk1, float *mk2, float *scores,
                                 uint8_t *valid, int32_t *match_ij, mi_stream_t stream) {
  MI_ENTER();
  if (!z) return MI_E_NULL;
  if (pitch < m || pitch % 4 != 0 || ((uintptr_t)z % 16) != 0) return MI_E_ALIGN;
  ZSourceF32 src;
  src.z = z;
  src.pitch = pitch;
  return mnn_from_source(src, nullptr, batch, n, m, u, v, kpts1, kpts2, max_matches, threshold, workspace,
                         workspace_bytes, nullptr, mk1, mk2, scores, valid, match_ij, (hipStream_t)stream);
}

extern "C" int mi_mnn_from_duals_dots(const uint16_t *dots, const float *row_info, const float *col_info, int batch,
                                      int n, int m, int pitch, double epsilon, const float *u, const float *v,
                                      const float *kpts1, const float *kpts2, int max_matches, float threshold,
                                      void *workspace, size_t workspace_bytes, const uint32_t *solver_status,
                                      float *mk1, float *mk2, float *scores, uint8_t *valid, int32_t *match_ij,
                                      mi_stream_t stream) {
  MI_ENTER();
  if (!dots || !row_info || !col_info) return MI_E_NULL;
  if (pitch < m || pitch % 8 != 0 || ((uintptr_t)dots % 16) != 0) return MI_E_ALIGN;
  if (!(epsilon > 0.0)) return MI_E_PARAM;
  ZSourceDots src;
  src.dots = dots;
  src.pitch = pitch;
  src.row_info = reinterpret_cast<const float2 *>(row_info);
  src.col_info = reinterpret_cast<const float2 *>(col_info);
  src.neg_inv_eps = (float)(-1.0 / epsilon);
  src.ri = make_float2(0.f, 0.f);
  if (solver_status && ((uintptr_t)solver_status % 4) != 0) return MI_E_ALIGN;
  return mnn_from_source(src, src.col_info, batch, n, m, u, v, kpts1, kpts2, max_matches, threshold, workspace,
                         workspace_bytes, solver_status, mk1, mk2, scores, valid, match_ij, (hipStream_t)stream);
}

extern "C" int mi_mnn_extract(const float *p, int batch, int n, int m, const float *kpts1, const float *kpts2,
                              int max_matches, float threshold, uint64_t *row_best, uint64_t *col_best,
                              float *mk1, float *mk2, float *scores, uint8_t *valid, int32_t *match_ij,
                              mi_stream_t stream) {
  MI_ENTER();
  if (!p || !kpts1 || !kpts2 || !row_best || !col_best || !mk1 || !mk2 || !scores || !valid) return MI_E_NULL;
  if (batch <= 0 || n <= 0 || m <= 0 || batch > 65535) return MI_E_SHAPE;
  if (n > MX_MAX || max_matches <= 0) return MI_E_PARAM;
  if (((uintptr_t)row_best % 8) != 0 || ((uintptr_t)col_best % 8) != 0) return MI_E_ALIGN;
  hipStream_t s = (hipStream_t)stream;
  if (m <= 1024 && MI_HOOK(mnn_one_pass, 1) != 0) {
    const int e = mi_zero_async(col_best, (size_t)batch * m * sizeof(uint64_t), s);
    if (e != MI_OK) return e;
    if (m <= 512)
      hipLaunchKernelGGL(mnn_p_kernel<8>, dim3(ceil_div(n, 32), batch), dim3(512), 0, s, p, n, m, row_best,
                         reinterpret_cast<unsigned long long *>(col_best));
    else
      hipLaunchKernelGGL(mnn_p_kernel<16>, dim3(ceil_div(n, 32), batch), dim3(512), 0, s, p, n, m, row_best,
                         reinterpret_cast<unsigned long long *>(col_best));
  } else {
    hipLaunchKernelGGL(mnn_row_kernel, dim3(ceil_div(n, 4), batch), dim3(256), 0, s, p, n, m, row_best);
    hipLaunchKernelGGL(mnn_col_kernel, dim3(ceil_div(m, 64), batch), dim3(256), 0, s, p, n, m, col_best);
  }
  hipLaunchKernelGGL(mnn_select_kernel, dim3(batch), dim3(MX_THREADS), 0, s, n, m, row_best, col_best,
                     (const uint64_t *)nullptr, 0, kpts1, kpts2, max_matches, threshold, (const uint32_t *)nullptr, mk1,
                     mk2, scores, valid, match_ij);
  return mi_launch_status();
}

namespace {
template <bool REWRITE, bool HAS_DUST>
__global__ __launch_bounds__(256) void match_filters_kernel(float *__restrict__ p, int n, int m, size_t row_stride,
                                                            size_t plane_stride, float ratio_threshold,
                                                            float dustbin_margin, uint8_t *__restrict__ valid) {
  const int lane = threadIdx.x & 63, wave = threadIdx.x >> 6;
  const int b = blockIdx.y, i = blockIdx.x * 4 + wave;
  if (i >= n) return;
  float *pr = p + (size_t)b * plane_stride + (size_t)i * row_stride;
  float a1 = -INFINITY, a2 = -INFINITY;
  for (int j0 = 0; j0 < m; j0 += 512) {
    float x[8];
#pragma unroll
    for (int q = 0; q < 8; ++q) {
      const int j = j0 + q * 64 + lane;
      x[q] = j < m ? pr[j] : -INFINITY;
    }
#pragma unroll
    for (int q = 0; q < 8; ++q) {
      if (x[q] > a1) { a2 = a1; a1 = x[q]; } else if (x[q] > a2) { a2 = x[q]; }
    }
  }
#pragma unroll
  for (int o = 32; o > 0; o >>= 1) {
    const float b1 = __shfl_xor(a1, o, 64), b2 = __shfl_xor(a2, o, 64);
    const float hi = fmaxf(a1, b1), lo = fminf(a1, b1);
    a2 = fmaxf(lo, fmaxf(a2, b2));
    a1 = hi;
  }
  const float best = a1;
  const float second = (m >= 2) ? a2 : 0.0f;
  const float dust = HAS_DUST ? pr[m] : 0.0f;
  bool ok = true;
  if (ratio_threshold > 0.0f) ok = ok && (best / (second + 1e-8f) >= ratio_threshold);
  if (HAS_DUST && dustbin_margin >= 0.0f) ok = ok && ((best - dust) >= dustbin_margin);
  if (lane == 0) valid[(size_t)b * n + i] = ok ? 1 : 0;
  if (REWRITE && !ok) {
    for (int j = lane; j < m; j += 64) pr[j] = pr[j] * 0.0f;
    if (lane == 0) pr[m] = 1.0f + 0.0f * dust;
  }
}
}

extern "C" int mi_match_filters(float *p, int batch, int n, int m, float ratio_threshold, float dustbin_margin,
                                uint8_t *valid, mi_stream_t stream) {
  MI_ENTER();
  if (!p || !valid) return MI_E_NULL;
  if (batch <= 0 || n <= 0 || m <= 0 || batch > 65535) return MI_E_SHAPE;
  hipLaunchKernelGGL((match_filters_kernel<true, true>), dim3(ceil_div(n, 4), batch), dim3(256), 0, (hipStream_t)stream, p,
                     n, m, (size_t)(m + 1), (size_t)(n + 1) * (size_t)(m + 1), ratio_threshold, dustbin_margin, valid);
  return mi_launch_status();
}

extern "C" int mi_match_filter_masks(const float *p, int batch, int n, int m, int has_dustbin, float ratio_threshold,
                                     float dustbin_margin, uint8_t *valid, mi_stream_t stream) {
  MI_ENTER();
  if (!p || !valid) return MI_E_NULL;
  if (batch <= 0 || n <= 0 || m <= 0 || batch > 65535) return MI_E_SHAPE;
  if (!has_dustbin && dustbin_margin >= 0.0f) return MI_E_PARAM;
  float *q = const_cast<float *>(p);
  const dim3 grid(ceil_div(n, 4), batch);
  if (has_dustbin)
    hipLaunchKernelGGL((match_filters_kernel<false, true>), grid, dim3(256), 0, (hipStream_t)stream, q, n, m,
                       (size_t)(m + 1), (size_t)(n + 1) * (size_t)(m + 1), ratio_threshold, dustbin_margin, valid);
  else
    hipLaunchKernelGGL((match_filters_kernel<false, false>), grid, dim3(256), 0, (hipStream_t)stream, q, n, m, (size_t)m,
                       (size_t)n * (size_t)m, ratio_threshold, dustbin_margin, valid);
  return mi_launch_status();
}

namespace {
__global__ __launch_bounds__(256) void core_rowmax_kernel(const float *__restrict__ p, int n, int m,
                                                          float *__restrict__ out) {
  const int lane = threadIdx.x & 63, wave = threadIdx.x >> 6;
  const int b = blockIdx.y, i = blockIdx.x * 4 + wave;
  if (i >= n) return;
  const float *pr = p + ((size_t)b * (n + 1) + i) * (size_t)(m + 1);
  float mx = -INFINITY;
  for (int j = lane; j < m; j += 64) mx = fmaxf(mx, pr[j]);
  mx = wave_max_dpp(mx);
  if (lane == 0) out[(size_t)b * n + i] = mx;
}
__global__ __launch_bounds__(256) void core_colmax_kernel(const float *__restrict__ p, int n, int m,
                                                          float *__restrict__ out) {
  const int b = blockIdx.y, j = blockIdx.x * 256 + threadIdx.x;
  if (j >= m) return;
  const float *pb = p + (size_t)b * (n + 1) * (size_t)(m + 1) + j;
  float mx = -INFINITY;
  for (int i = 0; i < n; ++i) mx = fmaxf(mx, pb[(size_t)i * (m + 1)]);
  out[(size_t)b * m + j] = mx;
}
}

extern "C" int mi_core_maxima(const float *p, int batch, int n, int m, float *row_max, float *col_max,
                              mi_stream_t stream) {
  MI_ENTER();
  if (!p || !row_max || !col_max) return MI_E_NULL;
  if (batch <= 0 || n <= 0 || m <= 0 || batch > 65535) return MI_E_SHAPE;
  hipLaunchKernelGGL(core_rowmax_kernel, dim3(ceil_div(n, 4), batch), dim3(256), 0, (hipStream_t)stream, p, n, m, row_max);
  hipLaunchKernelGGL(core_colmax_kernel, dim3(ceil_div(m, 256), batch), dim3(256), 0, (hipStream_t)stream, p, n, m,
                     col_max);
  return mi_launch_status();
}

extern "C" int mi_abi_version(void) { return 3; }

extern "C" const char *mi_error_string(int code) {
  switch (code) {
    case MI_OK: return "ok";
    case MI_E_NULL: return "required pointer is NULL";
    case MI_E_SHAPE: return "non-positive or inconsistent extent";
    case MI_E_PARAM: return "parameter outside the supported set";
    case MI_E_CAPACITY: return "workspace or capacity too small";
    case MI_E_ALIGN: return "pointer or pitch not aligned as documented";
    default: return code > 0 ? hipGetErrorString((hipError_t)code) : "unknown error";
  }
}
```

### onnx_image_processing_amd/csrc/sinkhorn_dots.hip

```cpp
#include "common.h"

#include <mutex>
#include "sk_tuner.h"
#include "stream_registry.h"

#include <math.h>

#include <atomic>

#include "hooks.h"

namespace {

__device__ __forceinline__ int ceil_div_dev(int a, int b) { return (a + b - 1) / b; }
__device__ __forceinline__ float sk_exp(float d) { return __builtin_amdgcn_exp2f(d * 1.4426950408889634f); }

constexpr float SKD_L2E = 1.4426950408889634f, SKD_LN2 = 0.6931471805599453f;

struct ZParams {
  float neg_inv_eps;
  float dust;
  float g_bound;
  float d_bound;
};

__device__ __forceinline__ float z_of(float dot, float2 row, float2 col, float neg_inv_eps) {
  return mi_z_from_dot(dot, row, col, neg_inv_eps);
}

constexpr int SKD_AUX = 20;
constexpr float SKD_FAST_LIMIT = 90.0f;

__device__ __forceinline__ void publish_wave_max(float x, float *__restrict__ aux_pair) {
  x = wave_max_dpp(x);
  if ((threadIdx.x & 63) == 0) aux_pair[blockIdx.x * 4 + (threadIdx.x >> 6)] = x;
}

__device__ __forceinline__ float max32_lane31(float v) {
  asm volatile(
      "s_nop 1\n\tv_max_f32_dpp %0, %0, %0 quad_perm:[1,0,3,2] row_mask:0xf bank_mask:0xf\n\t"
      "s_nop 1\n\tv_max_f32_dpp %0, %0, %0 quad_perm:[2,3,0,1] row_mask:0xf bank_mask:0xf\n\t"
      "s_nop 1\n\tv_max_f32_dpp %0, %0, %0 row_half_mirror row_mask:0xf bank_mask:0xf\n\t"
      "s_nop 1\n\tv_max_f32_dpp %0, %0, %0 row_mirror row_mask:0xf bank_mask:0xf\n\t"
      "s_nop 1\n\tv_max_f32_dpp %0, %0, %0 row_bcast:15 row_mask:0xa bank_mask:0xf\n\t"
      "s_nop 0"
      : "+v"(v));
  return __builtin_bit_cast(float, __builtin_amdgcn_readlane(__builtin_bit_cast(int, v), 31));
}

__device__ __forceinline__ float combine_column(const float *__restrict__ part_b, int nparts, int m, int j,
                                                float vold, float log_n) {
  const float *p = part_b + j;
  const size_t stride = (size_t)(m + 1);
  const float bj = p[(size_t)(nparts - 1) * stride];
  float s = 0.0f;
  int k = 0;
  for (; k + 16 <= nparts - 1; k += 16) {
    float t[16];
#pragma unroll
    for (int q = 0; q < 16; ++q) t[q] = p[(size_t)(k + q) * stride];
#pragma unroll
    for (int q = 0; q < 16; ++q) s += t[q];
  }
  for (; k + 4 <= nparts - 1; k += 4) {
    float t[4];
#pragma unroll
    for (int q = 0; q < 4; ++q) t[q] = p[(size_t)(k + q) * stride];
#pragma unroll
    for (int q = 0; q < 4; ++q) s += t[q];
  }
  for (; k < nparts - 1; ++k) s += p[(size_t)k * stride];
  const float a = s > 0.0f ? __builtin_amdgcn_logf(s) * SKD_LN2 : -INFINITY;
  const float hi = fmaxf(a, bj), lo = fminf(a, bj);
  const float lse = hi + __builtin_amdgcn_logf(1.0f + __builtin_amdgcn_exp2f((lo - hi) * SKD_L2E)) * SKD_LN2;
  return (vold + ((j == m) ? log_n : 0.0f)) - lse;
}

__device__ __forceinline__ float mix_mul_lo(uint32_t w, float t) {
  float p;
  asm("v_fma_mix_f32 %0, %1, %2, 0 op_sel_hi:[1,0,0]" : "=v"(p) : "v"(w), "v"(t));
  return p;
}
__device__ __forceinline__ float mix_mul_hi(uint32_t w, float t) {
  float p;
  asm("v_fma_mix_f32 %0, %1, %2, 0 op_sel:[1,0,0] op_sel_hi:[1,0,0]" : "=v"(p) : "v"(w), "v"(t));
  return p;
}

template <int E8, int RW, int NW, bool FAST, bool MIX = false, bool SPLIT = false>
__global__ __launch_bounds__(64 * NW) void sk_band_dots_kernel(const uint16_t *__restrict__ dots, int n, int m,
                                                               int pitch, const float2 *__restrict__ row_info,
                                                               ZParams zp, const float *__restrict__ v,
                                                               float *__restrict__ u, float *__restrict__ part,
                                                               float log_m, int v_is_zero,
                                                               const float *__restrict__ wp,
                                                               const float *__restrict__ tp, int cpitch,
                                                               const float *__restrict__ aux) {
  static_assert(!SPLIT || (E8 == 1 && RW == 4 && NW % 2 == 0 && FAST), "the split form is the one-chunk bounded-shift kernel");
  constexpr int RG = SPLIT ? NW / 2 : NW;
  constexpr int BAND = RG * RW;
  constexpr int NT = 64 * NW;
  constexpr int NC = 512 * E8;
  constexpr int NCW = SPLIT ? 2 * NC : NC;
  __shared__ float red[RG][NCW + 1];
  __shared__ float halfsum[SPLIT ? NW : 1][4];
  const int lane = threadIdx.x & 63, wave = __builtin_amdgcn_readfirstlane(threadIdx.x >> 6);
  const int b = blockIdx.y, band = blockIdx.x, nb = gridDim.x - 1;
  const float *vb = v + (size_t)b * (m + 1);
  float *pb = part + ((size_t)b * (nb + 1) + band) * (size_t)(m + 1);
  const float vd = v_is_zero ? 0.0f : vb[m];
  const float dust = zp.dust;
  const int rg = SPLIT ? wave >> 1 : wave, half = SPLIT ? wave & 1 : 0, cbase = half * NC;
  const int row0 = band * BAND + rg * RW;

  if (band == nb) {
    auto scr = [&](int w, int i) -> float & { if constexpr (SPLIT) return halfsum[w][i]; else return red[w][i]; };
    float mx = dust + vd;
    for (int j = threadIdx.x; j < m; j += NT) mx = fmaxf(mx, dust + (v_is_zero ? 0.0f : vb[j]));
    mx = wave_max_dpp(mx);
    if (lane == 0) scr(wave, 0) = mx;
    __syncthreads();
    mx = scr(0, 0);
#pragma unroll
    for (int w = 1; w < NW; ++w) mx = fmaxf(mx, scr(w, 0));
    float s = 0.0f;
    for (int j = threadIdx.x; j < m; j += NT) s += expf((dust + (v_is_zero ? 0.0f : vb[j])) - mx);
    s = wave_sum_dpp(s);
    if (lane == 0) scr(wave, 1) = s;
    __syncthreads();
    s = scr(0, 1);
#pragma unroll
    for (int w = 1; w < NW; ++w) s += scr(w, 1);
    s += expf((dust + vd) - mx);
    const float un = log_m - (logf(s) + mx);
    if (threadIdx.x == 0) u[(size_t)b * (n + 1) + n] = un;
    for (int j = threadIdx.x; j <= m; j += NT) pb[j] = (dust + un) + (v_is_zero ? 0.0f : vb[j]);
    return;
  }

  float4 tl[E8][2], wl[E8][2];
#pragma unroll
  for (int e = 0; e < E8; ++e) {
    const int j = cbase + e * 512 + lane * 8;
    tl[e][0] = *reinterpret_cast<const float4 *>(tp + (size_t)b * cpitch + j);
    tl[e][1] = *reinterpret_cast<const float4 *>(tp + (size_t)b * cpitch + j + 4);
    wl[e][0] = *reinterpret_cast<const float4 *>(wp + (size_t)b * cpitch + j);
    wl[e][1] = *reinterpret_cast<const float4 *>(wp + (size_t)b * cpitch + j + 4);
  }
  uint4 raw[RW][E8];
#pragma unroll
  for (int r = 0; r < RW; ++r) {
    const int i = min(row0 + r, n - 1);
    const uint16_t *src = dots + ((size_t)b * n + i) * pitch;
#pragma unroll
    for (int e = 0; e < E8; ++e) {
      const int j = cbase + e * 512 + lane * 8;
      raw[r][e] = *reinterpret_cast<const uint4 *>(src + min(j, pitch - 8));
    }
  }

  float tq[E8][8], wq[E8][8];
#pragma unroll
  for (int e = 0; e < E8; ++e) {
    const float4 t0 = tl[e][0], t1 = tl[e][1], w0 = wl[e][0], w1 = wl[e][1];
    tq[e][0] = t0.x; tq[e][1] = t0.y; tq[e][2] = t0.z; tq[e][3] = t0.w;
    tq[e][4] = t1.x; tq[e][5] = t1.y; tq[e][6] = t1.z; tq[e][7] = t1.w;
    wq[e][0] = w0.x; wq[e][1] = w0.y; wq[e][2] = w0.z; wq[e][3] = w0.w;
    wq[e][4] = w1.x; wq[e][5] = w1.y; wq[e][6] = w1.z; wq[e][7] = w1.w;
  }
  const float xd0 = dust + vd;

  float nm_pair = 0.0f;
  if constexpr (FAST) {
    static_assert(SKD_AUX <= 64, "one aux slot per lane");
    static_assert(SKD_AUX <= 32, "max32_to_lane31 folds the low 32 lanes");
    const float wmax = max32_lane31(lane < SKD_AUX ? aux[(size_t)b * SKD_AUX + lane] : -INFINITY);
    const float S = fmaxf(wmax + zp.g_bound, xd0 + zp.d_bound);
    nm_pair = -(S * SKD_L2E);
#pragma unroll
    for (int e = 0; e < E8; ++e)
#pragma unroll
      for (int q = 0; q < 8; ++q) wq[e][q] = __builtin_fmaf(wq[e][q], SKD_L2E, nm_pair);
  }

  float colsum[E8][8];
#pragma unroll
  for (int e = 0; e < E8; ++e)
#pragma unroll
    for (int q = 0; q < 8; ++q) colsum[e][q] = 0.0f;
  float dustcol = 0.0f;
  float x[RW][E8][8];
  float mx[RW], xd[RW], ci[RW];
  bool live[RW];
  constexpr bool ROWS = RW == 4;
  const int myrow = MI_ROW_OF_GROUP(lane >> 4);
  float civ = 0.0f, giv = 0.0f, xdv = 0.0f;
  if constexpr (ROWS) {
    const float2 riv = row_info[(size_t)b * n + min(row0 + myrow, n - 1)];
    const float g0 = -2.0f * zp.neg_inv_eps * riv.x;
    giv = FAST ? g0 * SKD_L2E : g0;
    if constexpr (MIX) giv *= 16777216.0f;
    civ = riv.y * zp.neg_inv_eps;
    xdv = xd0 - civ;
  }
#pragma unroll
  for (int r = 0; r < RW; ++r) {
    const int i = row0 + r;
    live[r] = i < n;
    float gi;
    if constexpr (ROWS) {
      gi = mi_readlane_f(giv, 16 * MI_ROW_OF_GROUP(r));
      if constexpr (!FAST) { ci[r] = mi_readlane_f(civ, 16 * MI_ROW_OF_GROUP(r)); xd[r] = xd0 - ci[r]; }
    } else {
      const float2 ri = row_info[(size_t)b * n + min(i, n - 1)];
      const float g0 = -2.0f * zp.neg_inv_eps * ri.x;
      gi = FAST ? g0 * SKD_L2E : g0;
      if constexpr (MIX) gi *= 16777216.0f;
      ci[r] = ri.y * zp.neg_inv_eps;
      xd[r] = xd0 - ci[r];
    }
#pragma unroll
    for (int e = 0; e < E8; ++e) {
      const uint32_t w4[4] = {raw[r][e].x, raw[r][e].y, raw[r][e].z, raw[r][e].w};
      if constexpr (E8 == 1) {
#pragma unroll
        for (int q = 0; q < 8; q += 2) {
          typedef float v2f __attribute__((ext_vector_type(2)));
          const v2f tt = {tq[e][q], tq[e][q + 1]}, ww = {wq[e][q], wq[e][q + 1]}, gg = {gi, gi};
          v2f dt;
          if constexpr (MIX) {
            dt.x = mix_mul_lo(w4[q >> 1], tt.x);
            dt.y = mix_mul_hi(w4[q >> 1], tt.y);
          } else {
            const v2f dot = {(float)(w4[q >> 1] & 0xFFFFu), (float)(w4[q >> 1] >> 16)};
            dt = dot * tt;
          }
          const v2f xx = __builtin_elementwise_fma(dt, gg, ww);
          x[r][e][q] = xx.x;
          x[r][e][q + 1] = xx.y;
        }
      } else {
#pragma unroll
        for (int q = 0; q < 8; ++q) {
          float dt;
          if constexpr (MIX) dt = (q & 1) ? mix_mul_hi(w4[q >> 1], tq[e][q]) : mix_mul_lo(w4[q >> 1], tq[e][q]);
          else dt = (float)((q & 1) ? (w4[q >> 1] >> 16) : (w4[q >> 1] & 0xFFFFu)) * tq[e][q];
          x[r][e][q] = __builtin_fmaf(dt, gi, wq[e][q]);
        }
      }
      if constexpr (!FAST)
        mx[r] = fmaxf(e == 0 ? xd[r] : mx[r], fmaxf(fmaxf(fmaxf(x[r][e][0], x[r][e][1]), fmaxf(x[r][e][2], x[r][e][3])),
                                                    fmaxf(fmaxf(x[r][e][4], x[r][e][5]), fmaxf(x[r][e][6], x[r][e][7]))));
    }
  }
  float nm[RW], s[RW], ed[RW];
  if constexpr (FAST) {
#pragma unroll
    for (int r = 0; r < RW; ++r) {
      nm[r] = nm_pair;
      s[r] = 0.0f;
#pragma unroll
      for (int e = 0; e < E8; ++e) {
#pragma unroll
        for (int q = 0; q < 8; ++q) x[r][e][q] = __builtin_amdgcn_exp2f(x[r][e][q]);
        const float tree = ((x[r][e][0] + x[r][e][1]) + (x[r][e][2] + x[r][e][3])) + ((x[r][e][4] + x[r][e][5]) + (x[r][e][6] + x[r][e][7]));
        s[r] = e == 0 ? tree : s[r] + tree;
      }
      if constexpr (!ROWS) ed[r] = __builtin_amdgcn_exp2f(__builtin_fmaf(xd[r], SKD_L2E, nm[r]));
    }
  } else {
    if constexpr (RW % 4 == 0) {
#pragma unroll
      for (int r = 0; r < RW; r += 4) wave_max4(mx + r);
    } else {
#pragma unroll
      for (int r = 0; r < RW; ++r) mx[r] = wave_max_dpp(mx[r]);
    }
#pragma unroll
    for (int r = 0; r < RW; ++r) {
      nm[r] = -(mx[r] * SKD_L2E);
      s[r] = 0.0f;
#pragma unroll
      for (int e = 0; e < E8; ++e) {
#pragma unroll
        for (int q = 0; q < 8; ++q)
          x[r][e][q] = __builtin_amdgcn_exp2f(__builtin_fmaf(x[r][e][q], SKD_L2E, nm[r]));
        const float tree = ((x[r][e][0] + x[r][e][1]) + (x[r][e][2] + x[r][e][3])) + ((x[r][e][4] + x[r][e][5]) + (x[r][e][6] + x[r][e][7]));
        s[r] = e == 0 ? tree : s[r] + tree;
      }
      if constexpr (!ROWS) ed[r] = __builtin_amdgcn_exp2f(__builtin_fmaf(xd[r], SKD_L2E, nm[r]));
    }
  }
  float wgtv = 0.0f, edv = 0.0f;
  if constexpr (ROWS) {
    float nmv = nm[0];
    if constexpr (!FAST) nmv = myrow == 1 ? nm[1] : myrow == 2 ? nm[2] : myrow == 3 ? nm[3] : nm[0];
    edv = __builtin_amdgcn_exp2f(__builtin_fmaf(xdv, SKD_L2E, nmv));
    float rowsum = wave_sum4_rows(s);
    if constexpr (SPLIT) {
      if ((lane & 15) == 0) halfsum[wave][lane >> 4] = rowsum;
      __syncthreads();
      const float other = halfsum[wave ^ 1][lane >> 4];
      rowsum = half == 0 ? rowsum + other : other + rowsum;
    }
    const float stv = rowsum + edv;
    const bool livev = row0 + myrow < n;
    if ((lane & 15) == 0 && livev && half == 0)
      u[(size_t)b * (n + 1) + row0 + myrow] = (nmv - __builtin_amdgcn_logf(stv)) * SKD_LN2 - civ;
    wgtv = livev ? __builtin_amdgcn_rcpf(stv) : 0.0f;
  } else {
#pragma unroll
    for (int r = 0; r < RW; ++r) s[r] = wave_sum_dpp(s[r]);
  }
#pragma unroll
  for (int r = 0; r < RW; ++r) {
    float wgt;
    if constexpr (ROWS) {
      wgt = mi_readlane_f(wgtv, 16 * MI_ROW_OF_GROUP(r));
      ed[r] = mi_readlane_f(edv, 16 * MI_ROW_OF_GROUP(r));
    } else {
      const float st = s[r] + ed[r];
      if (lane == 0 && live[r])
        u[(size_t)b * (n + 1) + row0 + r] = (nm[r] - __builtin_amdgcn_logf(st)) * SKD_LN2 - ci[r];
      wgt = live[r] ? __builtin_amdgcn_rcpf(st) : 0.0f;
    }
#pragma unroll
    for (int e = 0; e < E8; ++e)
#pragma unroll
      for (int q = 0; q < 8; ++q) colsum[e][q] = __builtin_fmaf(x[r][e][q], wgt, colsum[e][q]);
    dustcol = __builtin_fmaf(ed[r], wgt, dustcol);
  }
#pragma unroll
  for (int e = 0; e < E8; ++e)
#pragma unroll
    for (int q = 0; q < 8; ++q) red[rg][cbase + e * 512 + lane * 8 + q] = colsum[e][q];
  if (lane == 0 && half == 0) red[rg][NCW] = dustcol;
  __syncthreads();
  for (int c = threadIdx.x; c <= NCW; c += NT) {
    const int j = (c == NCW) ? m : c;
    if (c < NCW && j >= m) continue;
    float t = red[0][c];
#pragma unroll
    for (int w = 1; w < RG; ++w) t += red[w][c];
    pb[j] = t;
  }
}

__global__ __launch_bounds__(256) void sk_vcombine_dots_kernel(const float *__restrict__ part, int m, int nparts,
                                                               float *__restrict__ v, float log_n,
                                                               int v_is_zero, const float2 *__restrict__ col_info,
                                                               float neg_inv_eps, float *__restrict__ wp,
                                                               int cpitch, float *__restrict__ aux) {
  const int b = blockIdx.y;
  const int j = blockIdx.x * 256 + threadIdx.x;
  float w = -INFINITY;
  if (j <= m) {
    const float vold = v_is_zero ? 0.0f : v[(size_t)b * (m + 1) + j];
    const float vnew = combine_column(part + (size_t)b * nparts * (size_t)(m + 1), nparts, m, j, vold, log_n);
    v[(size_t)b * (m + 1) + j] = vnew;
    if (j < m) {
      w = col_info[(size_t)b * m + j].y * neg_inv_eps + vnew;
      wp[(size_t)b * cpitch + j] = w;
    }
  }
  publish_wave_max(w, aux + (size_t)b * SKD_AUX);
}

__global__ __launch_bounds__(256) void sk_dots_init_kernel(const float2 *__restrict__ col_info, int m, int cpitch,
                                                           float neg_inv_eps, float *__restrict__ wp,
                                                           float *__restrict__ tp, float *__restrict__ aux,
                                                           unsigned *__restrict__ status) {
  const int b = blockIdx.y;
  const int j = blockIdx.x * 256 + threadIdx.x;
  if (b == 0 && j == 0) *status = 0u;
  const float2 c = (j < m) ? col_info[(size_t)b * m + j] : make_float2(0.0f, 0.0f);
  const float w = (j < m) ? c.y * neg_inv_eps : -INFINITY;
  tp[(size_t)b * cpitch + j] = c.x;
  wp[(size_t)b * cpitch + j] = w;
  publish_wave_max(w, aux + (size_t)b * SKD_AUX);
  if (blockIdx.x == 0 && threadIdx.x >= 4 * gridDim.x && threadIdx.x < SKD_AUX) aux[(size_t)b * SKD_AUX + threadIdx.x] = -INFINITY;
}

__global__ __launch_bounds__(256) void sk_exp_dots_kernel(const uint16_t *__restrict__ dots, int n, int m, int pitch,
                                                          const float2 *__restrict__ row_info,
                                                          const float2 *__restrict__ col_info, ZParams zp,
                                                          const float *__restrict__ u, const float *__restrict__ v,
                                                          float *__restrict__ p) {
  const int lane = threadIdx.x & 63, wave = threadIdx.x >> 6;
  const int b = blockIdx.y;
  const int i = blockIdx.x * 4 + wave;
// ... 790 lines not shown
```

### onnx_image_processing_amd/distributed.py

```python
from __future__ import annotations

import os

import torch
import torch.distributed as dist

RECORD_FIELDS = 6


def env_world() -> tuple[int, int, int]:
    return (int(os.environ.get("RANK", "0")), int(os.environ.get("WORLD_SIZE", "1")),
            int(os.environ.get("LOCAL_RANK", "0")))


def init(backend: str | None = None, force: bool = False) -> tuple[int, int, int]:
    rank, world, local = env_world()
    if (world > 1 or force) and not dist.is_initialized():
        os.environ.setdefault("MASTER_ADDR", "127.0.0.1")
        if world == 1 and "MASTER_PORT" not in os.environ:
            import socket
            with socket.socket() as sck:
                sck.bind(("127.0.0.1", 0))
                os.environ["MASTER_PORT"] = str(sck.getsockname()[1])
        os.environ.setdefault("HSA_ENABLE_IPC_MODE_LEGACY", "0")
        if backend is None:
            backend = "nccl" if torch.cuda.is_available() else "gloo"
        kw = {}
        if backend == "nccl":
            torch.cuda.set_device(local)
            kw["device_id"] = torch.device("cuda", local)
        dist.init_process_group(backend=backend, rank=rank, world_size=world, **kw)
    return rank, world, local


def shard_range(total: int, rank: int, world: int) -> tuple[int, int]:
    if total < 0 or world <= 0 or not (0 <= rank < world):
        raise ValueError(f"bad shard request total={total} rank={rank} world={world}")
    base, extra = divmod(total, world)
    begin = rank * base + min(rank, extra)
    return begin, begin + base + (1 if rank < extra else 0)


def pack_records(mk1: torch.Tensor, mk2: torch.Tensor, scores: torch.Tensor, valid: torch.Tensor) -> torch.Tensor:
    return torch.cat([mk1, mk2, scores.unsqueeze(-1), valid.to(scores.dtype).unsqueeze(-1)], dim=-1).contiguous()


def unpack_records(rec: torch.Tensor):
    return rec[..., 0:2], rec[..., 2:4], rec[..., 4], rec[..., 5] > 0.5


def shard_sizes(total: int, world: int) -> list[int]:
    return [e - b for b, e in (shard_range(total, r, world) for r in range(world))]


def gather_records(rec: torch.Tensor, dst: int = 0, total: int | None = None,
                   collective: str = "gather") -> torch.Tensor | None:
    if collective not in ("gather", "all_gather"):
        raise ValueError(f"collective must be 'gather' or 'all_gather', got {collective!r}")
    if not dist.is_initialized() or dist.get_world_size() == 1:
        if total is not None and rec.shape[0] != total:
            raise ValueError(f"single process holds {rec.shape[0]} rows but total={total}")
        return rec
    world, rank = dist.get_world_size(), dist.get_rank()
    sizes = None
    if total is not None:
        sizes = shard_sizes(total, world)
        if rec.shape[0] != sizes[rank]:
            raise ValueError(f"rank {rank} holds {rec.shape[0]} rows, shard_range({total}, {rank}, {world}) says {sizes[rank]}")
        rows = max(sizes)
        if rec.shape[0] < rows:
            pad = torch.zeros((rows - rec.shape[0],) + tuple(rec.shape[1:]), dtype=rec.dtype, device=rec.device)
            rec = torch.cat([rec, pad], dim=0)
    rec = rec.contiguous()
    if collective == "gather":
        out = [torch.empty_like(rec) for _ in range(world)] if rank == dst else None
        dist.gather(rec, out, dst=dst)
        if rank != dst:
            return None
    else:
        full = torch.empty((world * rec.shape[0],) + tuple(rec.shape[1:]), dtype=rec.dtype, device=rec.device)
        dist.all_gather_into_tensor(full, rec)
        if rank != dst:
            return None
        out = list(full.split(rec.shape[0], dim=0)) if rec.shape[0] > 0 else [rec] * world
    if sizes is not None:
        out = [slab[:sz] for slab, sz in zip(out, sizes)]
    return torch.cat(out, dim=0)


class PendingGather:

    def __init__(self, work, out, rank, dst, sizes, rec):
        self._work, self._out, self._rank, self._dst, self._sizes, self._rec = work, out, rank, dst, sizes, rec

    def wait(self) -> torch.Tensor | None:
        if self._work is not None:
            self._work.wait()
            self._work = None
        if self._rank != self._dst:
            return None
        out = self._out
        if self._sizes is not None:
            out = [slab[:sz] for slab, sz in zip(out, self._sizes)]
        return out[0] if len(out) == 1 else torch.cat(out, dim=0)


def gather_records_async(rec: torch.Tensor, dst: int = 0, total: int | None = None) -> PendingGather:
    if not dist.is_initialized():
        if total is not None and rec.shape[0] != total:
            raise ValueError(f"single process holds {rec.shape[0]} rows but total={total}")
        return PendingGather(None, [rec], 0, 0, None, rec)
    world, rank = dist.get_world_size(), dist.get_rank()
    sizes = None
    if total is not None:
        sizes = shard_sizes(total, world)
        if rec.shape[0] != sizes[rank]:
            raise ValueError(f"rank {rank} holds {rec.shape[0]} rows, shard_range({total}, {rank}, {world}) says {sizes[rank]}")
        rows = max(sizes)
        if rec.shape[0] < rows:
            pad = torch.zeros((rows - rec.shape[0],) + tuple(rec.shape[1:]), dtype=rec.dtype, device=rec.device)
            rec = torch.cat([rec, pad], dim=0)
    rec = rec.contiguous()
    out = [torch.empty_like(rec) for _ in range(world)] if rank == dst else None
    work = dist.gather(rec, out, dst=dst, async_op=True)
    return PendingGather(work, out, rank, dst, sizes, rec)


def barrier_max_ms(elapsed_ms: float, device: torch.device | str) -> float:
    if not dist.is_initialized() or dist.get_world_size() == 1:
        return elapsed_ms
    t = torch.tensor([elapsed_ms], dtype=torch.float64, device=device)
    dist.all_reduce(t, op=dist.ReduceOp.MAX)
    return float(t.item())
```

### onnx_image_processing_amd/ops.py

```python
from __future__ import annotations

import torch

from . import _native as N

F32 = torch.float32


U8 = torch.uint8


def convert_u8(image: torch.Tensor) -> torch.Tensor:
    src = image.contiguous()
    out = torch.empty(src.shape, dtype=F32, device=src.device)
    if src.numel():
        N.call("mi_convert_u8_f32", N.dev(src, U8, "image"), src.numel(), out.data_ptr(), N.stream_ptr())
    return out


class ImagePair:

    def __init__(self, a: torch.Tensor, b: torch.Tensor):
        if a.shape != b.shape or a.dtype != b.dtype or a.device != b.device:
            raise RuntimeError(f"image batches differ: {tuple(a.shape)} {a.dtype} {a.device} vs {tuple(b.shape)} {b.dtype} {b.device}")
        self.a, self.b = a, b

    @property
    def device(self):
        return self.a.device

    @property
    def dtype(self):
        return self.a.dtype

    @property
    def shape(self):
        return torch.Size((2 * self.a.shape[0],) + tuple(self.a.shape[1:]))


def _images(image, what: str, keep_u8: bool = False):
    if isinstance(image, ImagePair):
        return ImagePair(_images(image.a, what, keep_u8), _images(image.b, what, keep_u8))
    if image.dim() != 4 or image.shape[1] != 1:
        raise RuntimeError(f"{what} must have shape (N, 1, H, W), got {tuple(image.shape)}")
    if image.dtype == U8:
        return image.contiguous() if keep_u8 else convert_u8(image)
    return image.float().contiguous()


TILE_COUNTER_BYTES = 16640

MI_SOLVER_DEFAULT, MI_SOLVER_MULTI_LAUNCH, MI_SOLVER_NO_FORK = 0, 1, 2
MI_SOLVER_DOTS_BELOW_1024 = 4
_solver_flags = MI_SOLVER_DEFAULT


def set_solver_flags(flags: int) -> None:
    global _solver_flags
    if not isinstance(flags, int) or flags & ~(MI_SOLVER_MULTI_LAUNCH | MI_SOLVER_NO_FORK):
        raise ValueError("solver flags must be MI_SOLVER_DEFAULT (0) or an OR of MI_SOLVER_MULTI_LAUNCH (1) and "
                         f"MI_SOLVER_NO_FORK (2), got {flags}")
    _solver_flags = int(flags)


MI_SCHEDULE_UNDECIDED, MI_SCHEDULE_CALLER_HELPER, MI_SCHEDULE_TWO_HELPERS, MI_SCHEDULE_UNSPLIT = -1, 0, 1, 2


def sinkhorn_schedule(batch: int, n: int, m: int, iterations: int) -> int:
    return int(N.load().mi_sinkhorn_dots_schedule(N.stream_ptr(), int(batch), int(n), int(m), int(iterations)))


def set_sinkhorn_schedule(schedule: int) -> None:
    N.check(N.load().mi_sinkhorn_dots_set_schedule(N.stream_ptr(), int(schedule)), "mi_sinkhorn_dots_set_schedule")


def corner_response(image: torch.Tensor, block_size: int) -> torch.Tensor:
    img = _images(image, "image", keep_u8=True)
    n, _, h, w = img.shape
    out = torch.empty(img.shape, dtype=F32, device=img.device)
    u8 = img.dtype == U8
    ctr = torch.empty(TILE_COUNTER_BYTES // 4, dtype=torch.int32, device=img.device)
    if isinstance(img, ImagePair):
        N.call("mi_corner_response_pair", N.dev(img.a, U8 if u8 else F32, "image"), N.dev(img.b, U8 if u8 else F32, "image"),
               int(u8), n // 2, h, w, int(block_size), N.dev(out, F32, "score"), ctr.data_ptr(), N.stream_ptr())
        return out
    N.call("mi_corner_response_balanced", N.dev(img, U8 if u8 else F32, "image"), int(u8), n, h, w, int(block_size),
           N.dev(out, F32, "score"), ctr.data_ptr(), N.stream_ptr())
    return out


def _score_maps(scores: torch.Tensor) -> torch.Tensor:
    if scores.dim() != 3:
        raise RuntimeError(f"scores must have shape (B, H, W), got {tuple(scores.shape)}")
    return scores.float().contiguous()


def nms_mask(scores: torch.Tensor, radius: int) -> torch.Tensor:
    s = _score_maps(scores)
    b, h, w = s.shape
    mask = torch.empty_like(s)
    N.call("mi_nms_mask", N.dev(s, F32, "scores"), b, h, w, int(radius), N.dev(mask, F32, "mask"), N.stream_ptr())
    return mask


def candidate_layout(h: int, w: int) -> tuple[int, int]:
    import ctypes
    seg, cap = ctypes.c_int(0), ctypes.c_int(0)
    N.check(N.load().mi_candidate_layout(int(h), int(w), ctypes.byref(seg), ctypes.byref(cap)), "mi_candidate_layout")
    return seg.value, cap.value


def _candidate_buffers(b: int, h: int, w: int, device):
    seg, cap = candidate_layout(h, w)
    cand = torch.empty((b, seg, cap), dtype=torch.int64, device=device)
    count = torch.empty((b, seg), dtype=torch.int32, device=device)
    return cand, count, seg, cap


def _topk_from_candidates(cand, count, seg, cap, b, h, w, k):
    if h * w < k:
        raise RuntimeError(f"selected index k out of range (k={k} > H*W={h * w})")
    kpts = torch.empty((b, k, 2), dtype=F32, device=cand.device)
    ksc = torch.empty((b, k), dtype=F32, device=cand.device)
    N.call("mi_topk_keypoints", cand.data_ptr(), count.data_ptr(), seg, cap, b, w, int(k), kpts.data_ptr(),
           ksc.data_ptr(), N.stream_ptr())
    return kpts, ksc


def nms_topk(scores: torch.Tensor, radius: int, k: int, score_threshold: float = 0.0, border_margin: int = 0):
    s = _score_maps(scores)
    b, h, w = s.shape
    cand, count, seg, cap = _candidate_buffers(b, h, w, s.device)
    N.call("mi_nms_candidates", N.dev(s, F32, "scores"), b, h, w, int(radius), float(score_threshold),
           int(border_margin), cand.data_ptr(), count.data_ptr(), N.stream_ptr())
    return _topk_from_candidates(cand, count, seg, cap, b, h, w, k)


def select_topk(scores: torch.Tensor, mask: torch.Tensor, k: int, score_threshold: float = 0.0,
                border_margin: int = 0):
    s = _score_maps(scores)
    mk = _score_maps(mask)
    if mk.shape != s.shape:
        raise RuntimeError(f"nms_mask shape {tuple(mk.shape)} != scores shape {tuple(s.shape)}")
    b, h, w = s.shape
    cand, count, seg, cap = _candidate_buffers(b, h, w, s.device)
    N.call("mi_select_candidates", N.dev(s, F32, "scores"), N.dev(mk, F32, "nms_mask"), b, h, w,
           float(score_threshold), int(border_margin), cand.data_ptr(), count.data_ptr(), N.stream_ptr())
    return _topk_from_candidates(cand, count, seg, cap, b, h, w, k)


def bad_plan(pair_geom: torch.Tensor, pair_thr: torch.Tensor) -> torch.Tensor:
    p = pair_geom.numel()
    nbytes = int(N.load().mi_bad_plan_bytes(p))
    plan = torch.empty(((nbytes + 15) // 16 * 2,), dtype=torch.int64, device=pair_geom.device)
    N.call("mi_bad_plan_build", N.dev(pair_geom, torch.int32, "pair_geom"), N.dev(pair_thr, F32, "pair_thr"), p,
           plan.data_ptr(), N.stream_ptr())
    return plan


def sparse_bad(image: torch.Tensor, keypoints: torch.Tensor, pair_geom: torch.Tensor, pair_thr: torch.Tensor,
               mode: int, temperature: float, normalize: bool, want_desc: bool = True, want_bits: bool = False,
               plan: torch.Tensor | None = None):
    img = _images(image, "image", keep_u8=True)
    n, _, h, w = img.shape
    if keypoints.dim() != 3 or keypoints.shape[0] != n or keypoints.shape[2] != 2:
        raise RuntimeError(f"keypoints must have shape ({n}, K, 2), got {tuple(keypoints.shape)}")
    kp = keypoints.float().contiguous()
    k = kp.shape[1]
    p = pair_geom.numel()
    desc = torch.empty((n, k, p), dtype=F32, device=img.device) if want_desc else None
    bits = torch.empty((n, k, p // 32), dtype=torch.int32, device=img.device) if want_bits else None
    u8 = img.dtype == U8
    if isinstance(img, ImagePair):
        N.call("mi_sparse_bad_pair", N.dev(img.a, U8 if u8 else F32, "image"), N.dev(img.b, U8 if u8 else F32, "image"),
               int(u8), n // 2, h, w, N.dev(kp, F32, "keypoints"), k,
               N.dev(pair_geom, torch.int32, "pair_geom"), N.dev(pair_thr, F32, "pair_thr"), p, int(mode),
               float(temperature), int(bool(normalize)), desc.data_ptr() if want_desc else None,
               bits.data_ptr() if want_bits else None, plan.data_ptr() if plan is not None else None,
               torch.empty((n * k,), dtype=torch.uint8, device=img.device).data_ptr() if plan is not None else None,
               N.stream_ptr())
        return desc, bits
    N.call("mi_sparse_bad_u8" if u8 else "mi_sparse_bad", N.dev(img, U8 if u8 else F32, "image"), n, h, w,
           N.dev(kp, F32, "keypoints"), k,
           N.dev(pair_geom, torch.int32, "pair_geom"), N.dev(pair_thr, F32, "pair_thr"), p, int(mode),
           float(temperature), int(bool(normalize)), desc.data_ptr() if want_desc else None,
           bits.data_ptr() if want_bits else None, plan.data_ptr() if plan is not None else None,
           torch.empty((n * k,), dtype=torch.uint8, device=img.device).data_ptr() if plan is not None else None,
           N.stream_ptr())
    return desc, bits


def bad_dense(image: torch.Tensor, pair_geom: torch.Tensor, pair_thr: torch.Tensor, mode: int,
              temperature: float) -> torch.Tensor:
    img = _images(image, "x")
    n, _, h, w = img.shape
    p = pair_geom.numel()
    out = torch.empty((n, p, h, w), dtype=F32, device=img.device)
    N.call("mi_bad_dense", N.dev(img, F32, "x"), n, h, w, N.dev(pair_geom, torch.int32, "pair_geom"),
           N.dev(pair_thr, F32, "pair_thr"), p, int(mode), float(temperature), out.data_ptr(), N.stream_ptr())
    return out


def bad_dense_oriented(image: torch.Tensor, orientation: torch.Tensor, pair_geom: torch.Tensor, pair_thr: torch.Tensor,
                       mode: int, temperature: float) -> torch.Tensor:
    img = _images(image, "x")
    n, _, h, w = img.shape
    ori = orientation.float().contiguous()
    if tuple(ori.shape) != (n, 1, h, w):
        raise RuntimeError(f"orientation must have shape ({n}, 1, {h}, {w}), got {tuple(ori.shape)}")
    p = pair_geom.numel()
    out = torch.empty((n, p, h, w), dtype=F32, device=img.device)
    N.call("mi_bad_dense_oriented", N.dev(img, F32, "x"), N.dev(ori, F32, "orientation"), n, h, w,
           N.dev(pair_geom, torch.int32, "pair_geom"), N.dev(pair_thr, F32, "pair_thr"), p, int(mode),
           float(temperature), out.data_ptr(), N.stream_ptr())
    return out


def gather_descriptors(descriptor_map: torch.Tensor, keypoints: torch.Tensor, bilinear: bool) -> torch.Tensor:
    if descriptor_map.dim() != 4 or keypoints.dim() != 3 or keypoints.shape[0] != descriptor_map.shape[0]:
        raise RuntimeError(f"expected (B,D,H,W) and (B,N,2), got {tuple(descriptor_map.shape)} {tuple(keypoints.shape)}")
    dm = descriptor_map.float().contiguous()
    kp = keypoints.float().contiguous()
    b, d, h, w = dm.shape
    out = torch.empty((b, kp.shape[1], d), dtype=F32, device=dm.device)
    N.call("mi_gather_descriptors", N.dev(dm, F32, "descriptor_map"), b, d, h, w, N.dev(kp, F32, "keypoints"),
           kp.shape[1], int(bool(bilinear)), out.data_ptr(), N.stream_ptr())
    return out


def angle_map(image: torch.Tensor, moment_kernels: torch.Tensor, patch_size: int) -> torch.Tensor:
    img = _images(image, "image")
    n, _, h, w = img.shape
    out = torch.empty_like(img)
    N.call("mi_angle_map", N.dev(img, F32, "image"), n, h, w, int(patch_size),
           N.dev(moment_kernels.contiguous(), F32, "moment_kernels"), out.data_ptr(), N.stream_ptr())
    return out


def angle_at_keypoints(image: torch.Tensor, keypoints: torch.Tensor, moment_kernels: torch.Tensor,
                       patch_size: int) -> torch.Tensor:
    img = _images(image, "image")
    n, _, h, w = img.shape
    kp = keypoints.float().contiguous()
    theta = torch.empty((n, kp.shape[1]), dtype=F32, device=img.device)
    if isinstance(img, ImagePair):
        N.call("mi_angle_at_keypoints_pair", N.dev(img.a, F32, "image"), N.dev(img.b, F32, "image"), n // 2, h, w,
               N.dev(kp, F32, "keypoints"), kp.shape[1], int(patch_size),
               N.dev(moment_kernels.contiguous(), F32, "moment_kernels"), theta.data_ptr(), N.stream_ptr())
        return theta
    N.call("mi_angle_at_keypoints", N.dev(img, F32, "image"), n, h, w, N.dev(kp, F32, "keypoints"), kp.shape[1],
           int(patch_size), N.dev(moment_kernels.contiguous(), F32, "moment_kernels"), theta.data_ptr(),
           N.stream_ptr())
    return theta


def sparse_bad_oriented(image: torch.Tensor, keypoints: torch.Tensor, orientation: torch.Tensor,
                        pair_geom: torch.Tensor, pair_thr: torch.Tensor, mode: int, temperature: float,
                        normalize: bool, want_desc: bool = True, want_bits: bool = False, bilinear: bool = False,
                        max_reach: float = 0.0):
    img = _images(image, "image")
    n, _, h, w = img.shape
    if keypoints.dim() != 3 or keypoints.shape[0] != n or keypoints.shape[2] != 2:
        raise RuntimeError(f"keypoints must have shape ({n}, K, 2), got {tuple(keypoints.shape)}")
    kp = keypoints.float().contiguous()
    k = kp.shape[1]
    ang = orientation.float().contiguous()
    if ang.dim() == 4 and tuple(ang.shape) == (n, 1, h, w):
        amap, akp = N.dev(ang, F32, "orientation"), None
    elif ang.dim() == 2 and tuple(ang.shape) == (n, k):
        amap, akp = None, N.dev(ang, F32, "orientation")
    else:
        raise RuntimeError(f"orientation must be ({n}, 1, {h}, {w}) or ({n}, {k}), got {tuple(ang.shape)}")
    p = pair_geom.numel()
    desc = torch.empty((n, k, p), dtype=F32, device=img.device) if want_desc else None
    bits = torch.empty((n, k, p // 32), dtype=torch.int32, device=img.device) if want_bits else None
    status = torch.empty((n, k), dtype=torch.uint8, device=img.device)
    if isinstance(img, ImagePair):
        if akp is None:
            raise RuntimeError("an ImagePair takes per-keypoint angles (2B, K), not a dense orientation map")
        N.call("mi_sparse_bad_oriented_pair", N.dev(img.a, F32, "image"), N.dev(img.b, F32, "image"), n // 2, h, w,
               N.dev(kp, F32, "keypoints"), k, akp, N.dev(pair_geom, torch.int32, "pair_geom"),
               N.dev(pair_thr, F32, "pair_thr"), p, int(mode), float(temperature), int(bool(normalize)),
               int(bool(bilinear)), float(max_reach), desc.data_ptr() if want_desc else None,
               bits.data_ptr() if want_bits else None, status.data_ptr(), N.stream_ptr())
        return desc, bits
    N.call("mi_sparse_bad_oriented", N.dev(img, F32, "image"), n, h, w, N.dev(kp, F32, "keypoints"), k, amap, akp,
           N.dev(pair_geom, torch.int32, "pair_geom"), N.dev(pair_thr, F32, "pair_thr"), p, int(mode),
           float(temperature), int(bool(normalize)), int(bool(bilinear)), float(max_reach),
           desc.data_ptr() if want_desc else None, bits.data_ptr() if want_bits else None, status.data_ptr(),
           N.stream_ptr())
    return desc, bits


def _pitch(m: int) -> int:
    return (m + 3) // 4 * 4


def cost_logscores_bits(bits1: torch.Tensor, bits2: torch.Tensor, normalized: bool, epsilon: float):
    b, n, words = bits1.shape
    m = bits2.shape[1]
    pitch = _pitch(m)
    z = torch.empty((b, n, pitch), dtype=F32, device=bits1.device)
    N.call("mi_cost_logscores_bits", N.dev(bits1, torch.int32, "bits1"), N.dev(bits2, torch.int32, "bits2"), b, n, m,
           words * 32, int(bool(normalized)), float(epsilon), z.data_ptr(), pitch, N.stream_ptr())
    return z, pitch


def cost_logscores_f32(desc1: torch.Tensor, desc2: torch.Tensor, distance: int, epsilon: float):
    if desc1.dim() != 3 or desc2.dim() != 3 or desc1.shape[0] != desc2.shape[0] or desc1.shape[2] != desc2.shape[2]:
        raise RuntimeError(f"descriptor shapes do not match: {tuple(desc1.shape)} vs {tuple(desc2.shape)}")
    d1 = desc1.float().contiguous()
    d2 = desc2.float().contiguous()
    b, n, d = d1.shape
    m = d2.shape[1]
    pitch = _pitch(m)
    z = torch.empty((b, n, pitch), dtype=F32, device=d1.device)
    N.call("mi_cost_logscores_f32", N.dev(d1, F32, "desc1"), N.dev(d2, F32, "desc2"), b, n, m, d, int(distance),
           float(epsilon), z.data_ptr(), pitch, N.stream_ptr())
    return z, pitch


def sinkhorn(z: torch.Tensor, m: int, pitch: int, dustbin_logscore: float, iterations: int,
             return_duals: bool = False, use_workspace: bool = True, want_p: bool = True):
    b, n, _ = z.shape
    u = torch.empty((b, n + 1), dtype=F32, device=z.device)
    v = torch.empty((b, m + 1), dtype=F32, device=z.device)
    p = torch.empty((b, n + 1, m + 1), dtype=F32, device=z.device) if want_p else None
    wbytes = int(N.load().mi_sinkhorn_workspace_bytes(b, n, m))
    work = torch.empty((max(wbytes, 8) // 8,), dtype=torch.int64, device=z.device) if use_workspace else None
    N.call("mi_sinkhorn", N.dev(z, F32, "z"), b, n, m, pitch, float(dustbin_logscore), int(iterations),
           u.data_ptr(), v.data_ptr(), p.data_ptr() if p is not None else None,
           work.data_ptr() if work is not None else None, wbytes if work is not None else 0, N.stream_ptr())
    return (p, u, v) if (return_duals or not want_p) else p


DOTS_MIN_EPSILON = 0.005


def dots_supported(b: int, n: int, m: int, epsilon: float = 1.0) -> bool:
    return epsilon >= DOTS_MIN_EPSILON and int(N.load().mi_sinkhorn_dots_workspace_bytes(b, n, m)) > 0


def sinkhorn_bits(bits1: torch.Tensor, bits2: torch.Tensor, normalized: bool, epsilon: float, unused_score: float,
                  iterations: int, return_duals: bool = False, want_p: bool = True, return_state: bool = False):
    b, n, words = bits1.shape
    m = bits2.shape[1]
    dev = bits1.device
    wbytes = int(N.load().mi_sinkhorn_dots_workspace_bytes(b, n, m)) if epsilon >= DOTS_MIN_EPSILON else 0
    if wbytes == 0:
        if return_state or not want_p:
            raise RuntimeError(f"the dot-product Sinkhorn form supports M <= 1024 and epsilon >= {DOTS_MIN_EPSILON}, "
                               f"got M = {m}, epsilon = {epsilon}")
        z, pitch = cost_logscores_bits(bits1, bits2, normalized, epsilon)
        return sinkhorn(z, m, pitch, -unused_score / epsilon, iterations, return_duals=return_duals)
    pitch = (m + 7) // 8 * 8
    dots = torch.empty((b, n, pitch), dtype=torch.int16, device=dev)
    row_info = torch.empty((b, n, 2), dtype=F32, device=dev)
    col_info = torch.empty((b, m, 2), dtype=F32, device=dev)
    N.call("mi_cost_dots_bits", N.dev(bits1, torch.int32, "bits1"), N.dev(bits2, torch.int32, "bits2"), b, n, m,
           words * 32, int(bool(normalized)), dots.data_ptr(), pitch, row_info.data_ptr(), col_info.data_ptr(),
           N.stream_ptr())
    u = torch.empty((b, n + 1), dtype=F32, device=dev)
    v = torch.empty((b, m + 1), dtype=F32, device=dev)
    p = torch.empty((b, n + 1, m + 1), dtype=F32, device=dev) if want_p else None
    work = torch.empty(((wbytes + 7) // 8,), dtype=torch.int64, device=dev)
    N.call("mi_sinkhorn_dots", dots.data_ptr(), row_info.data_ptr(), col_info.data_ptr(), b, n, m, pitch,
           float(epsilon), float(unused_score), 1.0 if normalized else float(words * 32), int(iterations),
           u.data_ptr(), v.data_ptr(), p.data_ptr() if p is not None else None, work.data_ptr(), wbytes,
           _solver_flags | (MI_SOLVER_DOTS_BELOW_1024 if words * 32 < 1024 else 0), N.stream_ptr())
    if return_state:
        status = N.load().mi_sinkhorn_dots_status_word(work.data_ptr(), b, n, m)
        return p, u, v, (dots, row_info, col_info, pitch, (work, status))
    return (p, u, v) if (return_duals or not want_p) else p


def match_filters(p: torch.Tensor, ratio_threshold: float, dustbin_margin: float):
    b, n1, m1 = p.shape
    valid = torch.empty((b, n1 - 1), dtype=torch.bool, device=p.device)
    N.call("mi_match_filters", N.dev(p, F32, "P"), b, n1 - 1, m1 - 1, float(ratio_threshold), float(dustbin_margin),
           valid.data_ptr(), N.stream_ptr())
    return p, valid


def match_filter_masks(p: torch.Tensor, has_dustbin: bool, ratio_threshold: float, dustbin_margin: float) -> torch.Tensor:
    pp = p.float().contiguous()
    b, n, m = pp.shape[0], pp.shape[1] - int(has_dustbin), pp.shape[2] - int(has_dustbin)
    valid = torch.empty((b, n), dtype=torch.bool, device=pp.device)
    N.call("mi_match_filter_masks", N.dev(pp, F32, "P"), b, n, m, int(has_dustbin), float(ratio_threshold),
           float(dustbin_margin), valid.data_ptr(), N.stream_ptr())
    return valid


def mnn_extract(p: torch.Tensor, kpts1: torch.Tensor, kpts2: torch.Tensor, max_matches: int, threshold: float,
                return_indices: bool = False):
    if p.dim() != 3:
        raise RuntimeError(f"P must have shape (B, N+1, M+1), got {tuple(p.shape)}")
    pp = p.float().contiguous()
    k1 = kpts1.float().contiguous()
    k2 = kpts2.float().contiguous()
    b, n, m = pp.shape[0], k1.shape[1], k2.shape[1]
    if pp.shape[1] != n + 1 or pp.shape[2] != m + 1:
        raise RuntimeError(f"P shape {tuple(pp.shape)} does not match keypoints ({n}, {m})")
    dev = pp.device
    row_best = torch.empty((b, n), dtype=torch.int64, device=dev)
    col_best = torch.empty((b, m), dtype=torch.int64, device=dev)
    mk1 = torch.empty((b, max_matches, 2), dtype=F32, device=dev)
    mk2 = torch.empty((b, max_matches, 2), dtype=F32, device=dev)
    sc = torch.empty((b, max_matches), dtype=F32, device=dev)
    valid = torch.empty((b, max_matches), dtype=torch.bool, device=dev)
    ij = torch.empty((b, max_matches, 2), dtype=torch.int32, device=dev)
    N.call("mi_mnn_extract", N.dev(pp, F32, "P"), b, n, m, N.dev(k1, F32, "keypoints1"), N.dev(k2, F32, "keypoints2"),
           int(max_matches), float(threshold), row_best.data_ptr(), col_best.data_ptr(), mk1.data_ptr(),
           mk2.data_ptr(), sc.data_ptr(), valid.data_ptr(), ij.data_ptr(), N.stream_ptr())
    out = (mk1, mk2, sc, valid)
    return out + (ij,) if return_indices else out


def _mnn_outputs(b, max_matches, dev):
    return (torch.empty((b, max_matches, 2), dtype=F32, device=dev), torch.empty((b, max_matches, 2), dtype=F32, device=dev),
            torch.empty((b, max_matches), dtype=F32, device=dev), torch.empty((b, max_matches), dtype=torch.bool, device=dev),
            torch.empty((b, max_matches, 2), dtype=torch.int32, device=dev))


def mnn_duals_supported(b: int, n: int, m: int) -> bool:
    return int(N.load().mi_mnn_duals_workspace_bytes(b, n, m)) > 0


def mnn_from_duals(z: torch.Tensor, m: int, pitch: int, u: torch.Tensor, v: torch.Tensor, kpts1: torch.Tensor,
                   kpts2: torch.Tensor, max_matches: int, threshold: float, return_indices: bool = False):
    b, n, _ = z.shape
    k1, k2 = kpts1.float().contiguous(), kpts2.float().contiguous()
    wbytes = int(N.load().mi_mnn_duals_workspace_bytes(b, n, m))
    if wbytes == 0:
        raise RuntimeError(f"mnn_from_duals supports N <= 4096 and M <= 1024, got ({n}, {m})")
    work = torch.empty((wbytes // 8,), dtype=torch.int64, device=z.device)
    mk1, mk2, sc, valid, ij = _mnn_outputs(b, max_matches, z.device)
    N.call("mi_mnn_from_duals", N.dev(z, F32, "z"), b, n, m, pitch, N.dev(u, F32, "u"), N.dev(v, F32, "v"),
           N.dev(k1, F32, "keypoints1"), N.dev(k2, F32, "keypoints2"), int(max_matches), float(threshold),
           work.data_ptr(), wbytes, mk1.data_ptr(), mk2.data_ptr(), sc.data_ptr(), valid.data_ptr(), ij.data_ptr(),
           N.stream_ptr())
    out = (mk1, mk2, sc, valid)
    return out + (ij,) if return_indices else out


def mnn_from_duals_dots(state, m: int, epsilon: float, u: torch.Tensor, v: torch.Tensor, kpts1: torch.Tensor,
                        kpts2: torch.Tensor, max_matches: int, threshold: float, return_indices: bool = False):
    dots, row_info, col_info, pitch = state[:4]
    status = state[4][1] if len(state) > 4 else None
    b, n, _ = dots.shape
    k1, k2 = kpts1.float().contiguous(), kpts2.float().contiguous()
    wbytes = int(N.load().mi_mnn_duals_workspace_bytes(b, n, m))
    if wbytes == 0:
        raise RuntimeError(f"mnn_from_duals_dots supports N <= 4096 and M <= 1024, got ({n}, {m})")
    work = torch.empty((wbytes // 8,), dtype=torch.int64, device=dots.device)
    mk1, mk2, sc, valid, ij = _mnn_outputs(b, max_matches, dots.device)
    N.call("mi_mnn_from_duals_dots", dots.data_ptr(), row_info.data_ptr(), col_info.data_ptr(), b, n, m, pitch,
           float(epsilon), N.dev(u, F32, "u"), N.dev(v, F32, "v"), N.dev(k1, F32, "keypoints1"),
           N.dev(k2, F32, "keypoints2"), int(max_matches), float(threshold), work.data_ptr(), wbytes, status,
           mk1.data_ptr(), mk2.data_ptr(), sc.data_ptr(), valid.data_ptr(), ij.data_ptr(), N.stream_ptr())
    out = (mk1, mk2, sc, valid)
    return out + (ij,) if return_indices else out



def akaze_diffuse(image: torch.Tensor, iterations: int, kappa: float, dt: float = 0.25) -> torch.Tensor:
    img = _images(image, "image")
    n, _, h, w = img.shape
    if iterations <= 0:
        return img
    bufs = [torch.empty_like(img), torch.empty_like(img) if iterations > 1 else None]
    cur = img
    for i in range(int(iterations)):
        dst = bufs[i & 1]
        N.call("mi_akaze_diffuse", N.dev(cur, F32, "image"), n, h, w, float(kappa), float(dt), dst.data_ptr(),
               N.stream_ptr())
        cur = dst
    return cur


def akaze_scale(image: torch.Tensor, iterations: int, kappa: float, dt: float, threshold: float, nms_size: int,
                scores_out: torch.Tensor | None = None, image_out: torch.Tensor | None = None):
    img = _images(image, "image")
    n, _, h, w = img.shape
    out = image_out if image_out is not None else torch.empty_like(img)
    scores = scores_out if scores_out is not None else torch.empty_like(img)
    fused = bool(N.load().mi_akaze_scale_fused(int(iterations), int(nms_size)))
    tmp = None if fused or iterations <= 1 else torch.empty_like(img)
    N.call("mi_akaze_scale", N.dev(img, F32, "image"), n, h, w, int(iterations), float(kappa), float(dt), float(threshold),
           int(nms_size), N.dev(out, F32, "image_out"), N.dev(scores, F32, "scores"), tmp.data_ptr() if tmp is not None else None,
           N.stream_ptr())
    return out, scores


def akaze_scale_sets(image1: torch.Tensor, image2: torch.Tensor, iterations: int, kappa: float, dt: float, threshold: float,
                     nms_size: int, scores_out: torch.Tensor, image_out: torch.Tensor):
    a, b = _images(image1, "image1"), _images(image2, "image2")
    if a.shape != b.shape:
        raise RuntimeError(f"image shapes differ: {tuple(a.shape)} vs {tuple(b.shape)}")
    n, _, h, w = a.shape
    if tuple(image_out.shape) != (2 * n, 1, h, w) or tuple(scores_out.shape) != (2 * n, 1, h, w):
        raise RuntimeError("image_out / scores_out must be (2N,1,H,W)")
    fused = bool(N.load().mi_akaze_scale_fused(int(iterations), int(nms_size)))
    tmp = None if fused or iterations <= 1 else torch.empty_like(a)
    N.call("mi_akaze_scale_sets", N.dev(a, F32, "image1"), N.dev(b, F32, "image2"), n, h, w, int(iterations), float(kappa),
           float(dt), float(threshold), int(nms_size), N.dev(image_out, F32, "image_out"), N.dev(scores_out, F32, "scores"),
           tmp.data_ptr() if tmp is not None else None, N.stream_ptr())
    return image_out, scores_out


AKAZE_KAPPA_MIN, AKAZE_KAPPA_MAX = 1e-3, 1e6


def akaze_kappa_fused(kappa: float) -> bool:
    return AKAZE_KAPPA_MIN <= float(kappa) <= AKAZE_KAPPA_MAX


def akaze_attain(scale_scores: torch.Tensor, scores: torch.Tensor) -> torch.Tensor:
    bits = torch.zeros(scores.shape, dtype=torch.int32, device=scores.device)
    for s in range(scale_scores.shape[0]):
        bits |= (scale_scores[s] == scores).to(torch.int32) << s
    return bits.to(U8)


def akaze_scale_select(image: torch.Tensor, iterations: int, kappa: float, dt: float, threshold: float, nms_size: int,
                       prev_scores: torch.Tensor | None, image_out: torch.Tensor | None = None):
    img = _images(image, "image")
    n, _, h, w = img.shape
    num_prev = 0 if prev_scores is None else int(prev_scores.shape[0])
    if num_prev > 7:
        raise RuntimeError(f"at most 8 scales, got {num_prev + 1}")
    if num_prev and tuple(prev_scores.shape[1:]) != (n, 1, h, w):
        raise RuntimeError(f"prev_scores must be (S-1,{n},1,{h},{w}), got {tuple(prev_scores.shape)}")
    out = image_out if image_out is not None else torch.empty_like(img)
    best = torch.empty_like(img)
    attain = torch.empty((n, 1, h, w), dtype=U8, device=img.device)
    fused = bool(N.load().mi_akaze_scale_fused(int(iterations), int(nms_size)))
    tmp = None if fused or iterations <= 1 else torch.empty_like(img)
    N.call("mi_akaze_scale_select", N.dev(img, F32, "image"), n, h, w, int(iterations), float(kappa), float(dt),
           float(threshold), int(nms_size), N.dev(out, F32, "image_out"),
           N.dev(prev_scores, F32, "prev_scores") if num_prev else None, num_prev, best.data_ptr(), attain.data_ptr(),
           tmp.data_ptr() if tmp is not None else None, N.stream_ptr())
    return out, best, attain


def akaze_orientation_from_attain(attain: torch.Tensor, scale_theta: torch.Tensor, keypoints: torch.Tensor) -> torch.Tensor:
    n, _, h, w = attain.shape
    s = int(scale_theta.shape[0])
    kp = keypoints.float().contiguous()
    k = kp.shape[1]
    theta = torch.empty((n, k), dtype=F32, device=attain.device)
    N.call("mi_akaze_orientation_from_attain", N.dev(attain, U8, "attain"), N.dev(scale_theta, F32, "scale_theta"), s, n,
           h, w, N.dev(kp, F32, "keypoints"), k, theta.data_ptr(), N.stream_ptr())
    return theta


def akaze_orientation_select(scale_images: torch.Tensor, attain: torch.Tensor, keypoints: torch.Tensor,
                             moment_kernels: torch.Tensor, patch_size: int) -> torch.Tensor:
    s, n, _, h, w = scale_images.shape
    kp = keypoints.float().contiguous()
    k = kp.shape[1]
    theta = torch.empty((n, k), dtype=F32, device=attain.device)
    N.call("mi_akaze_orientation_select", N.dev(scale_images, F32, "scale_images"), n * h * w, s,
           N.dev(attain, U8, "attain"), n, h, w, N.dev(kp, F32, "keypoints"), k, int(patch_size),
           N.dev(moment_kernels.float().contiguous(), F32, "moment_kernels"), theta.data_ptr(), N.stream_ptr())
    return theta


def akaze_hessian_scores(image: torch.Tensor, threshold: float, nms_size: int,
                         out: torch.Tensor | None = None) -> torch.Tensor:
    img = _images(image, "image")
    n, _, h, w = img.shape
    if out is None:
        out = torch.empty_like(img)
    N.call("mi_akaze_hessian_scores", N.dev(img, F32, "image"), n, h, w, float(threshold), int(nms_size),
           N.dev(out, F32, "scores"), N.stream_ptr())
    return out


def akaze_combine(scale_scores: torch.Tensor, scale_orientations: torch.Tensor | None):
    s, n, _, h, w = scale_scores.shape
    scores = torch.empty((n, 1, h, w), dtype=F32, device=scale_scores.device)
    oris = torch.empty_like(scores) if scale_orientations is not None else None
    N.call("mi_akaze_combine", N.dev(scale_scores, F32, "scale_scores"),
           N.dev(scale_orientations, F32, "scale_orientations") if scale_orientations is not None else None,
           s, n, h, w, scores.data_ptr(), oris.data_ptr() if oris is not None else None, N.stream_ptr())
    return scores, oris


def akaze_orientation_at_keypoints(scale_scores: torch.Tensor, scale_theta: torch.Tensor,
                                   keypoints: torch.Tensor) -> torch.Tensor:
    s, n, _, h, w = scale_scores.shape
    kp = keypoints.float().contiguous()
    k = kp.shape[1]
    theta = torch.empty((n, k), dtype=F32, device=scale_scores.device)
    N.call("mi_akaze_orientation_at_keypoints", N.dev(scale_scores, F32, "scale_scores"),
           N.dev(scale_theta, F32, "scale_theta"), s, n, h, w, N.dev(kp, F32, "keypoints"), k, theta.data_ptr(),
           N.stream_ptr())
    return theta



def _validity_bytes(valid: torch.Tensor | None) -> torch.Tensor | None:
    if valid is None:
        return None
    if valid.dtype == torch.bool:
        return valid.contiguous().view(torch.uint8)
    return (valid != 0).contiguous().view(torch.uint8)


def essential_matrix(p: torch.Tensor, pts1_n: torch.Tensor, pts2_n: torch.Tensor, valid1: torch.Tensor | None,
                     valid2: torch.Tensor | None, top_k: int, n_iter: int, n_iter_manifold: int,
                     banded: bool = True) -> torch.Tensor:
    if p.dim() != 3:
        raise RuntimeError(f"P must have shape (B, N+1, M+1), got {tuple(p.shape)}")
    pp = p.float().contiguous()
    b, n, m = pp.shape[0], pp.shape[1] - 1, pp.shape[2] - 1
    q1, q2 = pts1_n.float().contiguous(), pts2_n.float().contiguous()
    if tuple(q1.shape) != (b, n, 2) or tuple(q2.shape) != (b, m, 2):
        raise RuntimeError(f"points must be ({b},{n},2) and ({b},{m},2), got {tuple(q1.shape)}, {tuple(q2.shape)}")
    if (valid1 is None) != (valid2 is None):
        raise RuntimeError("valid1 and valid2 must be given together")
    v1, v2 = _validity_bytes(valid1), _validity_bytes(valid2)
    e = torch.empty((b, 3, 3), dtype=F32, device=pp.device)
    wbytes = int(N.load().mi_essential_matrix_workspace_bytes(b, n, m, int(top_k))) if banded else 0
    work = torch.empty(((wbytes + 7) // 8,), dtype=torch.int64, device=pp.device) if wbytes else None
    N.call("mi_essential_matrix", N.dev(pp, F32, "P"), b, n, m, N.dev(q1, F32, "pts1"), N.dev(q2, F32, "pts2"),
           N.dev(v1, torch.uint8, "valid1") if v1 is not None else None,
           N.dev(v2, torch.uint8, "valid2") if v2 is not None else None, int(top_k), int(n_iter), int(n_iter_manifold),
           e.data_ptr(), work.data_ptr() if work is not None else None, wbytes, N.stream_ptr())
    return e


def essential_matrix_dots(state, m: int, epsilon: float, u: torch.Tensor, v: torch.Tensor, pts1_n: torch.Tensor,
                          pts2_n: torch.Tensor, valid1: torch.Tensor | None, valid2: torch.Tensor | None, top_k: int,
                          n_iter: int, n_iter_manifold: int, banded: bool = True) -> torch.Tensor:
    dots, row_info, col_info, pitch = state[:4]
    b, n = dots.shape[0], dots.shape[1]
    q1, q2 = pts1_n.float().contiguous(), pts2_n.float().contiguous()
    if tuple(q1.shape) != (b, n, 2) or tuple(q2.shape) != (b, m, 2):
        raise RuntimeError(f"points must be ({b},{n},2) and ({b},{m},2), got {tuple(q1.shape)}, {tuple(q2.shape)}")
    if (valid1 is None) != (valid2 is None):
        raise RuntimeError("valid1 and valid2 must be given together")
    v1, v2 = _validity_bytes(valid1), _validity_bytes(valid2)
    e = torch.empty((b, 3, 3), dtype=F32, device=dots.device)
    wbytes = int(N.load().mi_essential_matrix_workspace_bytes(b, n, m, int(top_k))) if banded else 0
    work = torch.empty(((wbytes + 7) // 8,), dtype=torch.int64, device=dots.device) if wbytes else None
    N.call("mi_essential_matrix_dots", dots.data_ptr(), row_info.data_ptr(), col_info.data_ptr(), int(pitch), float(epsilon),
           N.dev(u, F32, "u"), N.dev(v, F32, "v"), b, n, m, N.dev(q1, F32, "pts1"), N.dev(q2, F32, "pts2"),
           N.dev(v1, torch.uint8, "valid1") if v1 is not None else None,
           N.dev(v2, torch.uint8, "valid2") if v2 is not None else None, int(top_k), int(n_iter), int(n_iter_manifold),
           e.data_ptr(), work.data_ptr() if work is not None else None, wbytes, N.stream_ptr())
    return e



def fast_score(image: torch.Tensor, threshold: float) -> torch.Tensor:
    img = _images(image, "image")
    n, _, h, w = img.shape
    out = torch.empty_like(img)
    N.call("mi_fast_score", N.dev(img, F32, "image"), n, h, w, float(threshold), out.data_ptr(), N.stream_ptr())
    return out


def dog_responses(image: torch.Tensor, weights_1d: torch.Tensor, want_maps: bool = True, want_score: bool = False):
    img = _images(image, "image")
    n, _, h, w = img.shape
    s, ks = weights_1d.shape
    out = torch.empty((n, s - 1, h, w), dtype=F32, device=img.device) if want_maps else None
    score = torch.empty((n, 1, h, w), dtype=F32, device=img.device) if want_score else None
    N.call("mi_dog_responses", N.dev(img, F32, "image"), n, h, w, N.dev(weights_1d.contiguous(), F32, "weights_1d"), s,
           ks, out.data_ptr() if out is not None else None, score.data_ptr() if score is not None else None,
           N.stream_ptr())
    return out, score


def normalise_keypoints(keypoints: torch.Tensor, k_inv: torch.Tensor) -> torch.Tensor:
    kp = keypoints.float().contiguous()
    ki = k_inv.float().contiguous()
    out = torch.empty_like(kp)
    N.call("mi_normalise_keypoints", N.dev(kp, F32, "keypoints"), kp.numel() // 2, N.dev(ki, F32, "K_inv"),
           out.data_ptr(), N.stream_ptr())
    return out


def core_maxima(p: torch.Tensor):
    pp = p.float().contiguous()
    b, n, m = pp.shape[0], pp.shape[1] - 1, pp.shape[2] - 1
    r = torch.empty((b, n), dtype=F32, device=pp.device)
    c = torch.empty((b, m), dtype=F32, device=pp.device)
    N.call("mi_core_maxima", N.dev(pp, F32, "P"), b, n, m, r.data_ptr(), c.data_ptr(), N.stream_ptr())
    return r, c


def match_pairs(image1: torch.Tensor, image2: torch.Tensor, *, block_size: int, nms_radius: int, max_keypoints: int,
                score_threshold: float, border_margin: int, pair_geom: torch.Tensor, pair_thr: torch.Tensor,
                plan: torch.Tensor | None, normalize_descriptors: bool, epsilon: float, unused_score: float,
                sinkhorn_iterations: int, max_matches: int, match_threshold: float, want_ij: bool = False):
    u8 = image1.dtype == U8 and image2.dtype == U8
    a, b2 = _images(image1, "image1", keep_u8=u8), _images(image2, "image2", keep_u8=u8)
    if a.shape != b2.shape:
        raise RuntimeError(f"image shapes differ: {tuple(a.shape)} vs {tuple(b2.shape)}")
    n, _, h, w = a.shape
    dev = a.device
    prm = N.MatchParams(int(block_size), int(nms_radius), int(max_keypoints), float(score_threshold), int(border_margin),
                        int(pair_geom.numel()), N.dev(pair_geom, torch.int32, "pair_geom"), N.dev(pair_thr, F32, "pair_thr"),
                        plan.data_ptr() if plan is not None else None, int(bool(normalize_descriptors)), float(epsilon),
                        float(unused_score), int(sinkhorn_iterations), int(max_matches), float(match_threshold),
                        _solver_flags)
    import ctypes
    wbytes = int(N.load().mi_match_pairs_workspace_bytes(n, h, w, ctypes.byref(prm)))
    if wbytes == 0:
        raise RuntimeError("mi_match_pairs does not cover these parameters (K <= 1024, P % 64 == 0, odd block size ...)")
    work = torch.empty(((wbytes + 7) // 8,), dtype=torch.int64, device=dev)
    k, mx = int(max_keypoints), int(max_matches)
    kp1 = torch.empty((n, k, 2), dtype=F32, device=dev)
    kp2 = torch.empty((n, k, 2), dtype=F32, device=dev)
    mk1 = torch.empty((n, mx, 2), dtype=F32, device=dev)
    mk2 = torch.empty((n, mx, 2), dtype=F32, device=dev)
    sc = torch.empty((n, mx), dtype=F32, device=dev)
    valid = torch.empty((n, mx), dtype=torch.bool, device=dev)
    ij = torch.empty((n, mx, 2), dtype=torch.int32, device=dev) if want_ij else None
    N.call("mi_match_pairs_u8" if u8 else "mi_match_pairs", N.dev(a, U8 if u8 else F32, "image1"),
           N.dev(b2, U8 if u8 else F32, "image2"), n, h, w, ctypes.byref(prm), kp1.data_ptr(),
           kp2.data_ptr(), mk1.data_ptr(), mk2.data_ptr(), sc.data_ptr(), valid.data_ptr(),
           ij.data_ptr() if ij is not None else None, work.data_ptr(), wbytes, N.stream_ptr())
    out = (kp1, kp2, mk1, mk2, sc, valid)
    return out + (ij,) if want_ij else out



def _leaf_array(leaf_size, batch: int, device) -> torch.Tensor:
    if isinstance(leaf_size, torch.Tensor):
        if leaf_size.is_cuda:
            lf = leaf_size.to(device=device, dtype=F32).reshape(-1)
            if lf.numel() == 1:
                return lf.expand(batch).contiguous() if batch > 1 else lf.contiguous()
            if lf.numel() != batch:
                raise RuntimeError(f"leaf_size has {lf.numel()} values for {batch} clouds")
            return lf.contiguous()
        leaf_size = leaf_size.reshape(-1).tolist()
        if len(leaf_size) == 1:
            leaf_size = leaf_size[0]
    if isinstance(leaf_size, (list, tuple)):
        if len(leaf_size) != batch:
            raise RuntimeError(f"leaf_size has {len(leaf_size)} values for {batch} clouds")
        return torch.tensor([float(x) for x in leaf_size], dtype=F32).to(device)
    return torch.full((batch,), float(leaf_size), dtype=F32, device=device)


def _voxel_launch(pts: torch.Tensor, offsets: torch.Tensor, batch: int, leaf: torch.Tensor):
    total, d = pts.shape
    if d < 3:
        raise RuntimeError(f"points must have at least 3 columns, got {d}")
    if total >= 2 ** 31:
        raise RuntimeError(f"{total} points: at most 2^31 - 1 per call")
    dev = pts.device
    out = torch.empty((total, d), dtype=F32, device=dev)
    mask = torch.empty((total,), dtype=torch.bool, device=dev)
    counts = torch.empty((batch,), dtype=torch.int64, device=dev)
    wbytes = N.load().mi_voxel_downsample_workspace_bytes(batch, total, d)
    work = torch.empty(((wbytes + 15) // 16 * 2,), dtype=torch.int64, device=dev)
    N.call("mi_voxel_downsample", pts.data_ptr() if total else None, N.dev(offsets, torch.int64, "offsets"), batch, total,
           d, N.dev(leaf, F32, "leaf_size"), out.data_ptr() if total else None, mask.data_ptr() if total else None,
           counts.data_ptr(), work.data_ptr(), work.numel() * 8, N.stream_ptr())
# ... 884 lines not shown
```

Before: 215,700 image-pairs/sec.

## Write MNN outputs as packed records and restructure dual-space argmax with mixed-precision decode

The MNN select kernel now writes keypoints, score and valid flag straight into one packed 6-float record, and Python exposes mk1/mk2/scores as views tagged so pack_records can return the buffer without a torch.cat. The duals band kernel is restructured: it precomputes per-row and per-column constants, decodes fp16 dots with v_fma_mix when bits < 1024, keeps all four rows' probabilities and finds row argmax through a batched wave_max4 plus ballots instead of per-row 64-bit wave reductions. This aims to remove a concat/copy pass and cut ALU and cross-lane reduction work, at the cost of more registers and fragile view/version tagging.

```diff
diff --git a/include/mi355x_match.h b/include/mi355x_match.h
--- a/include/mi355x_match.h
+++ b/include/mi355x_match.h
@@ -151,6 +151,15 @@
                            const float *kpts2, int max_matches, float threshold, void *workspace,
                            size_t workspace_bytes, const uint32_t *solver_status, float *mk1, float *mk2,
                            float *scores, uint8_t *valid, int32_t *match_ij, mi_stream_t stream);
+MI_API int mi_mnn_from_duals_records(const float *z, int batch, int n, int m, int pitch, const float *u, const float *v,
+                              const float *kpts1, const float *kpts2, int max_matches, float threshold,
+                              void *workspace, size_t workspace_bytes, float *record, uint8_t *valid,
+                              int32_t *match_ij, mi_stream_t stream);
+MI_API int mi_mnn_from_duals_dots_records(const uint16_t *dots, const float *row_info, const float *col_info, int batch,
+                                   int n, int m, int pitch, double epsilon, const float *u, const float *v,
+                                   const float *kpts1, const float *kpts2, int max_matches, float threshold,
+                                   void *workspace, size_t workspace_bytes, const uint32_t *solver_status, int flags,
+                                   float *record, uint8_t *valid, int32_t *match_ij, mi_stream_t stream);
 
 MI_API int mi_akaze_diffuse(const float *l_in, int n, int h, int w, float kappa, float dt, float *l_out,
                      mi_stream_t stream);
diff --git a/onnx_image_processing_amd/_native.py b/onnx_image_processing_amd/_native.py
--- a/onnx_image_processing_amd/_native.py
+++ b/onnx_image_processing_amd/_native.py
@@ -66,6 +66,11 @@
     "mi_mnn_from_duals_dots": [c_void_p, c_void_p, c_void_p, c_int, c_int, c_int, c_int, c_double, c_void_p, c_void_p,
                                c_void_p, c_void_p, c_int, c_float, c_void_p, c_size_t, c_void_p, c_void_p, c_void_p,
                                c_void_p, c_void_p, c_void_p, c_void_p],
+    "mi_mnn_from_duals_records": [c_void_p, c_int, c_int, c_int, c_int, c_void_p, c_void_p, c_void_p, c_void_p, c_int,
+                                  c_float, c_void_p, c_size_t, c_void_p, c_void_p, c_void_p, c_void_p],
+    "mi_mnn_from_duals_dots_records": [c_void_p, c_void_p, c_void_p, c_int, c_int, c_int, c_int, c_double, c_void_p,
+                                       c_void_p, c_void_p, c_void_p, c_int, c_float, c_void_p, c_size_t, c_void_p, c_int,
+                                       c_void_p, c_void_p, c_void_p, c_void_p],
     "mi_core_maxima": [c_void_p, c_int, c_int, c_int, c_void_p, c_void_p, c_void_p],
     "mi_normalise_keypoints": [c_void_p, ctypes.c_longlong, c_void_p, c_void_p, c_void_p],
     "mi_essential_matrix_workspace_bytes": [c_int, c_int, c_int, c_int],
diff --git a/onnx_image_processing_amd/csrc/common.h b/onnx_image_processing_amd/csrc/common.h
--- a/onnx_image_processing_amd/csrc/common.h
+++ b/onnx_image_processing_amd/csrc/common.h
@@ -151,6 +151,17 @@
   return __builtin_fmaf(dot * col.x, -2.0f * neg_inv_eps * row.x, col.y * neg_inv_eps) + row.y * neg_inv_eps;
 }
 
+__device__ __forceinline__ float mix_mul_lo(uint32_t w, float t) {
+  float p;
+  asm("v_fma_mix_f32 %0, %1, %2, 0 op_sel_hi:[1,0,0]" : "=v"(p) : "v"(w), "v"(t));
+  return p;
+}
+__device__ __forceinline__ float mix_mul_hi(uint32_t w, float t) {
+  float p;
+  asm("v_fma_mix_f32 %0, %1, %2, 0 op_sel:[1,0,0] op_sel_hi:[1,0,0]" : "=v"(p) : "v"(w), "v"(t));
+  return p;
+}
+
 __device__ __forceinline__ float wave_max(float v) {
 #pragma unroll
   for (int o = 32; o > 0; o >>= 1) v = fmaxf(v, __shfl_xor(v, o, 64));
diff --git a/onnx_image_processing_amd/csrc/mnn.hip b/onnx_image_processing_amd/csrc/mnn.hip
--- a/onnx_image_processing_amd/csrc/mnn.hip
+++ b/onnx_image_processing_amd/csrc/mnn.hip
@@ -107,7 +107,7 @@
     const uint64_t *__restrict__ col_part, int nb,
     const float *__restrict__ kpts1, const float *__restrict__ kpts2, int max_matches, float threshold,
     const uint32_t *__restrict__ solver_status,
-    float *__restrict__ mk1, float *__restrict__ mk2, float *__restrict__ scores,
+    float *__restrict__ mk1, float *__restrict__ mk2, float *__restrict__ scores, float *__restrict__ record,
     uint8_t *__restrict__ valid, int32_t *__restrict__ match_ij) {
   __shared__ uint64_t keys[MX_MAX];
   const bool dead = solver_status && *solver_status != 0u;
@@ -204,12 +204,21 @@
     const uint32_t jw = 0xFFFFFFFFu - (uint32_t)(rb[i] & 0xFFFFFFFFull);
     const uint32_t j = jw < (uint32_t)m ? jw : 0u;
     const size_t o = (size_t)b * max_matches + s;
-    mk1[o * 2 + 0] = kpts1[((size_t)b * n + i) * 2 + 0];
-    mk1[o * 2 + 1] = kpts1[((size_t)b * n + i) * 2 + 1];
-    mk2[o * 2 + 0] = kpts2[((size_t)b * m + j) * 2 + 0];
-    mk2[o * 2 + 1] = kpts2[((size_t)b * m + j) * 2 + 1];
-    scores[o] = sc;
+    const float y1 = kpts1[((size_t)b * n + i) * 2 + 0], x1 = kpts1[((size_t)b * n + i) * 2 + 1];
+    const float y2 = kpts2[((size_t)b * m + j) * 2 + 0], x2 = kpts2[((size_t)b * m + j) * 2 + 1];
     const bool ok = sc > 0.0f;
+    if (record) {
+      float2 *rec = reinterpret_cast<float2 *>(record + o * 6);
+      rec[0] = make_float2(y1, x1);
+      rec[1] = make_float2(y2, x2);
+      rec[2] = make_float2(sc, ok ? 1.0f : 0.0f);
+    } else {
+      mk1[o * 2 + 0] = y1;
+      mk1[o * 2 + 1] = x1;
+      mk2[o * 2 + 0] = y2;
+      mk2[o * 2 + 1] = x2;
+      scores[o] = sc;
+    }
     valid[o] = ok ? 1 : 0;
     if (match_ij) {
       match_ij[o * 2 + 0] = ok ? (int32_t)i : -1;
@@ -218,7 +227,10 @@
   }
 }
 
+typedef float v2f __attribute__((ext_vector_type(2)));
+
 struct ZSourceF32 {
+  static constexpr bool HAS_CONSTS = false;
   const float *z;
   int pitch;
   struct Raw { float4 a, c; };
@@ -232,37 +244,40 @@
     if (j + 4 < m) r.c = *reinterpret_cast<const float4 *>(src + 4);
     return r;
   }
-  __device__ __forceinline__ void decode(const Raw &r, float (&out)[8]) const {
-    out[0] = r.a.x; out[1] = r.a.y; out[2] = r.a.z; out[3] = r.a.w;
-    out[4] = r.c.x; out[5] = r.c.y; out[6] = r.c.z; out[7] = r.c.w;
-  }
   __device__ __forceinline__ Row load_row(int, int, int) const { return Row(); }
-  __device__ __forceinline__ void begin_row(const Row &) {}
-  __device__ __forceinline__ float col(int, int) const { return 0.0f; }
-  __device__ __forceinline__ void finish(float (&)[8], const float2 (&)[8]) const {}
+  __device__ __forceinline__ float2 row_consts(const Row &) const { return make_float2(0.f, 0.f); }
+  __device__ __forceinline__ float2 col_consts(float2) const { return make_float2(0.f, 0.f); }
+  __device__ __forceinline__ v2f z_pair(const Raw &r, int q, float2, v2f, v2f) const {
+    const float x[8] = {r.a.x, r.a.y, r.a.z, r.a.w, r.c.x, r.c.y, r.c.z, r.c.w};
+    return v2f{x[q], x[q + 1]};
+  }
 };
 
+template <bool MIX>
 struct ZSourceDots {
+  static constexpr bool HAS_CONSTS = true;
   const uint16_t *dots;
   int pitch;
-  const float2 *row_info, *col_info;
+  const float2 *row_info;
   float neg_inv_eps;
-  float2 ri;
   typedef uint4 Raw;
   typedef float2 Row;
   __device__ __forceinline__ Raw load_raw(int b, int n, int i, int j, int m) const {
     return *reinterpret_cast<const uint4 *>(dots + ((size_t)b * n + i) * pitch + min(j, pitch - 8));
   }
-  __device__ __forceinline__ void decode(const Raw &r, float (&out)[8]) const {
-    const uint32_t w[4] = {r.x, r.y, r.z, r.w};
-#pragma unroll
-    for (int q = 0; q < 8; ++q) out[q] = (float)((q & 1) ? (w[q >> 1] >> 16) : (w[q >> 1] & 0xFFFFu));
-  }
   __device__ __forceinline__ Row load_row(int b, int n, int i) const { return row_info[(size_t)b * n + i]; }
-  __device__ __forceinline__ void begin_row(const Row &r) { ri = r; }
-  __device__ __forceinline__ void finish(float (&x)[8], const float2 (&ci)[8]) const {
-#pragma unroll
-    for (int q = 0; q < 8; ++q) x[q] = mi_z_from_dot(x[q], ri, ci[q], neg_inv_eps);
+  __device__ __forceinline__ float2 row_consts(const Row &r) const {
+    const float g = -2.0f * neg_inv_eps * r.x;
+    return make_float2(MIX ? g * 16777216.0f : g, r.y * neg_inv_eps);
+  }
+  __device__ __forceinline__ float2 col_consts(float2 c) const { return make_float2(c.x, c.y * neg_inv_eps); }
+  __device__ __forceinline__ v2f z_pair(const Raw &r, int q, float2 rk, v2f cx, v2f cy) const {
+    const uint32_t w4[4] = {r.x, r.y, r.z, r.w};
+    const uint32_t w = w4[q >> 1];
+    v2f t;
+    if constexpr (MIX) t = v2f{mix_mul_lo(w, cx.x), mix_mul_hi(w, cx.y)};
+    else t = v2f{(float)(w & 0xFFFFu), (float)(w >> 16)} * cx;
+    return __builtin_elementwise_fma(t, v2f{rk.x, rk.x}, cy) + v2f{rk.y, rk.y};
   }
 };
 
@@ -273,6 +288,7 @@
                                                            uint64_t *__restrict__ row_best,
                                                            uint64_t *__restrict__ col_part) {
   static_assert(!SPLIT || (E8 == 1 && NW % 2 == 0), "the split form runs the one-chunk code on wave pairs");
+  static_assert(RW == 4, "the rows' maxima are reduced four at a time (wave_max4)");
   constexpr int RG = SPLIT ? NW / 2 : NW;
   constexpr int BAND = RG * RW;
   constexpr int NC = 512 * E8 * (SPLIT ? 2 : 1);
@@ -295,7 +311,7 @@
     for (int e = 0; e < E8; ++e) raw[r][e] = src.load_raw(b, n, ic, cbase + e * 512 + lane * 8, m);
   }
   __shared__ float s_v[NC];
-  __shared__ float2 s_ci[NC];
+  __shared__ float s_cx[SRC::HAS_CONSTS ? NC : 1], s_cy[SRC::HAS_CONSTS ? NC : 1];
   {
     constexpr int PER = NC / (64 * NW);
     float tv[PER];
@@ -304,68 +320,98 @@
     for (int q = 0; q < PER; ++q) {
       const int c = threadIdx.x + q * 64 * NW;
       tv[q] = c < m ? v[(size_t)b * (m + 1) + c] : 0.0f;
-      tc[q] = (col_info && c < m) ? col_info[(size_t)b * m + c] : make_float2(0.f, 0.f);
+      if constexpr (SRC::HAS_CONSTS) tc[q] = c < m ? col_info[(size_t)b * m + c] : make_float2(0.f, 0.f);
     }
 #pragma unroll
     for (int q = 0; q < PER; ++q) {
       const int c = threadIdx.x + q * 64 * NW;
       s_v[c] = tv[q];
-      s_ci[c] = tc[q];
+      if constexpr (SRC::HAS_CONSTS) {
+        const float2 ck = src.col_consts(tc[q]);
+        s_cx[c] = ck.x;
+        s_cy[c] = ck.y;
+      }
     }
   }
   __syncthreads();
-  float vv[E8][8];
-  float2 ci[E8][8];
+  v2f vv[E8][4], cx[E8][4], cy[E8][4];
 #pragma unroll
   for (int e = 0; e < E8; ++e)
 #pragma unroll
+    for (int q = 0; q < 8; q += 2) {
+      const int c = cbase + e * 512 + lane * 8 + q;
+      vv[e][q >> 1] = v2f{s_v[c], s_v[c + 1]};
+      cx[e][q >> 1] = SRC::HAS_CONSTS ? v2f{s_cx[c], s_cx[c + 1]} : v2f{0.f, 0.f};
+      cy[e][q >> 1] = SRC::HAS_CONSTS ? v2f{s_cy[c], s_cy[c + 1]} : v2f{0.f, 0.f};
+    }
+
+  float p[RW][E8][8];
+  float rmax[RW];
+#pragma unroll
+  for (int r = 0; r < RW; ++r) {
+    const bool live = row0 + r < n;
+    const float ui = uis[r];
+    const float2 rk = src.row_consts(rowd[r]);
+    float lm = -1.0f;
+#pragma unroll
+    for (int e = 0; e < E8; ++e) {
+#pragma unroll
+      for (int q = 0; q < 8; q += 2) {
+        const v2f z = src.z_pair(raw[r][e], q, rk, cx[e][q >> 1], cy[e][q >> 1]);
+        const v2f t = ((z + v2f{ui, ui}) + vv[e][q >> 1]) * v2f{1.4426950408889634f, 1.4426950408889634f};
+        const float x[2] = {__builtin_amdgcn_exp2f(t.x), __builtin_amdgcn_exp2f(t.y)};
+#pragma unroll
+        for (int h = 0; h < 2; ++h) {
+          const int j = cbase + e * 512 + lane * 8 + q + h;
+          p[r][e][q + h] = (FULL || (live && j < m)) ? x[h] : -1.0f;
+        }
+      }
+#pragma unroll
+      for (int q = 0; q < 8; q += 2) lm = fmaxf(fmaxf(lm, p[r][e][q]), p[r][e][q + 1]);
+    }
+    rmax[r] = lm;
+  }
+  wave_max4(rmax);
+  uint64_t rkey[RW];
+#pragma unroll
+  for (int r = 0; r < RW; ++r) {
+    const float rm = rmax[r];
+    uint32_t jw = 0u;
+#pragma unroll
+    for (int e = E8 - 1; e >= 0; --e) {
+      uint64_t hit[8], any = 0ull;
+#pragma unroll
+      for (int q = 0; q < 8; ++q) {
+        hit[q] = __builtin_amdgcn_ballot_w64(p[r][e][q] == rm);
+        any |= hit[q];
+      }
+      const uint64_t first = any & (0ull - any);
+      uint32_t qw = 7u;
+#pragma unroll
+      for (int q = 6; q >= 0; --q) qw = (hit[q] & first) != 0ull ? (uint32_t)q : qw;
+      const uint32_t le = any != 0ull ? (uint32_t)__builtin_ctzll(any) : 0u;
+      jw = any != 0ull ? (uint32_t)(cbase + e * 512) + le * 8u + qw : jw;
+    }
+    rkey[r] = rm >= 0.0f ? best_key(rm, jw) : 0ull;
+  }
+  {
+    const uint64_t mine = lane == 0 ? rkey[0] : lane == 1 ? rkey[1] : lane == 2 ? rkey[2] : rkey[3];
+    if constexpr (SPLIT) {
+      if (lane < RW) halfkey[wave][lane] = mine;
+    } else {
+      if (lane < RW && row0 + lane < n) row_best[(size_t)b * n + row0 + lane] = mine;
+    }
+  }
+#pragma unroll
+  for (int e = 0; e < E8; ++e)
+#pragma unroll
     for (int q = 0; q < 8; ++q) {
-      vv[e][q] = s_v[cbase + e * 512 + lane * 8 + q];
-      ci[e][q] = s_ci[cbase + e * 512 + lane * 8 + q];
-    }
-
-  float cbest[E8][8];
-  int cidx[E8][8];
-#pragma unroll
-  for (int e = 0; e < E8; ++e)
-#pragma unroll
-    for (int q = 0; q < 8; ++q) { cbest[e][q] = -1.0f; cidx[e][q] = 0; }
-
-#pragma unroll
-  for (int r = 0; r < RW; ++r) {
-    const int i = row0 + r;
-    const bool live = i < n;
-    const float ui = uis[r];
-    src.begin_row(rowd[r]);
-    float rbest = -1.0f;
-    int rj = 0;
-#pragma unroll
-    for (int e = 0; e < E8; ++e) {
-      float x[8];
-      src.decode(raw[r][e], x);
-      src.finish(x, ci[e]);
-#pragma unroll
-      for (int q = 0; q < 8; ++q) {
-        const int j = cbase + e * 512 + lane * 8 + q;
-        float p = mi_prob_exp((x[q] + ui) + vv[e][q]);
-        if constexpr (!FULL) p = (live && j < m) ? p : -1.0f;
-        if (p > rbest) { rbest = p; rj = j; }
-        if (p > cbest[e][q]) { cbest[e][q] = p; cidx[e][q] = i; }
-      }
-    }
-    uint64_t key = rbest >= 0.0f ? best_key(rbest, (uint32_t)rj) : 0ull;
-    key = wave_max_u64(key);
-    if constexpr (SPLIT) {
-      if (lane == 0) halfkey[wave][r] = key;
-    } else {
-      if (lane == 0 && live) row_best[(size_t)b * n + i] = key;
-    }
-  }
-#pragma unroll
-  for (int e = 0; e < E8; ++e)
-#pragma unroll
-    for (int q = 0; q < 8; ++q)
-      red[rg][cbase + e * 512 + lane * 8 + q] = cbest[e][q] >= 0.0f ? best_key(cbest[e][q], (uint32_t)cidx[e][q]) : 0ull;
+      const float cm = fmaxf(fmaxf(fmaxf(fmaxf(p[0][e][q], p[1][e][q]), p[2][e][q]), p[3][e][q]), -1.0f);
+      uint32_t t = 3u;
+#pragma unroll
+      for (int r = 2; r >= 0; --r) t = p[r][e][q] == cm ? (uint32_t)r : t;
+      red[rg][cbase + e * 512 + lane * 8 + q] = cm >= 0.0f ? best_key(cm, (uint32_t)row0 + t) : 0ull;
+    }
   __syncthreads();
   if constexpr (SPLIT) {
     if (half == 0 && lane < RW && row0 + lane < n) {
@@ -417,15 +463,21 @@
   return w;
 }
 
+struct MatchOut {
+  float *mk1, *mk2, *scores, *record;
+  uint8_t *valid;
+  int32_t *match_ij;
+};
+
 template <typename SRC>
 int mnn_from_source(SRC src, const float2 *col_info, int batch, int n, int m, const float *u, const float *v,
                     const float *kpts1, const float *kpts2, int max_matches, float threshold, void *workspace,
-                    size_t workspace_bytes, const uint32_t *solver_status, float *mk1, float *mk2, float *scores,
-                    uint8_t *valid, int32_t *match_ij, hipStream_t s) {
-  if (!u || !v || !kpts1 || !kpts2 || !workspace || !mk1 || !mk2 || !scores || !valid) return MI_E_NULL;
+                    size_t workspace_bytes, const uint32_t *solver_status, const MatchOut &out, hipStream_t s) {
+  if (!u || !v || !kpts1 || !kpts2 || !workspace || !out.valid) return MI_E_NULL;
+  if (!out.record && (!out.mk1 || !out.mk2 || !out.scores)) return MI_E_NULL;
   if (batch <= 0 || n <= 0 || m <= 0 || batch > 65535) return MI_E_SHAPE;
   if (n > MX_MAX || m > 1024 || max_matches <= 0) return MI_E_PARAM;
-  if (((uintptr_t)workspace % 8) != 0) return MI_E_ALIGN;
+  if (((uintptr_t)workspace % 8) != 0 || ((uintptr_t)out.record % 8) != 0) return MI_E_ALIGN;
   if (workspace_bytes < duals_bytes(batch, n, m)) return MI_E_CAPACITY;
   const DualsWork w = duals_carve(workspace, batch, n, m);
   const int nb = ceil_div(n, DUALS_BAND);
@@ -448,37 +500,84 @@
   }
   if (batch <= 32) {
     hipLaunchKernelGGL(mnn_select_kernel, dim3(batch), dim3(MX_THREADS), 0, s, n, m, w.row_best, w.col_best,
-                       (const uint64_t *)w.col_part, nb, kpts1, kpts2, max_matches, threshold, solver_status, mk1, mk2,
-                       scores, valid, match_ij);
+                       (const uint64_t *)w.col_part, nb, kpts1, kpts2, max_matches, threshold, solver_status, out.mk1,
+                       out.mk2, out.scores, out.record, out.valid, out.match_ij);
     return mi_launch_status();
   }
   hipLaunchKernelGGL(mnn_colmerge_kernel, dim3(ceil_div(m, 256), batch), dim3(256), 0, s, w.col_part, nb, m,
                      w.col_best);
   hipLaunchKernelGGL(mnn_select_kernel, dim3(batch), dim3(MX_THREADS), 0, s, n, m, w.row_best, w.col_best,
-                     (const uint64_t *)nullptr, 0, kpts1, kpts2, max_matches, threshold, solver_status, mk1, mk2, scores,
-                     valid, match_ij);
+                     (const uint64_t *)nullptr, 0, kpts1, kpts2, max_matches, threshold, solver_status, out.mk1, out.mk2,
+                     out.scores, out.record, out.valid, out.match_ij);
   return mi_launch_status();
 }
 
-}
-
-extern "C" size_t mi_mnn_duals_workspace_bytes(int batch, int n, int m) {
-  if (batch <= 0 || n <= 0 || m <= 0 || m > 1024 || n > MX_MAX) return 0;
-  return duals_bytes(batch, n, m);
-}
-
-extern "C" int mi_mnn_from_duals(const float *z, int batch, int n, int m, int pitch, const float *u, const float *v,
-                                 const float *kpts1, const float *kpts2, int max_matches, float threshold,
-                                 void *workspace, size_t workspace_bytes, float *mk1, float *mk2, float *scores,
-                                 uint8_t *valid, int32_t *match_ij, mi_stream_t stream) {
-  MI_ENTER();
+int mnn_from_z(const float *z, int batch, int n, int m, int pitch, const float *u, const float *v, const float *kpts1,
+               const float *kpts2, int max_matches, float threshold, void *workspace, size_t workspace_bytes,
+               const MatchOut &out, hipStream_t s) {
   if (!z) return MI_E_NULL;
   if (pitch < m || pitch % 4 != 0 || ((uintptr_t)z % 16) != 0) return MI_E_ALIGN;
   ZSourceF32 src;
   src.z = z;
   src.pitch = pitch;
   return mnn_from_source(src, nullptr, batch, n, m, u, v, kpts1, kpts2, max_matches, threshold, workspace,
-                         workspace_bytes, nullptr, mk1, mk2, scores, valid, match_ij, (hipStream_t)stream);
+                         workspace_bytes, nullptr, out, s);
+}
+
+template <bool MIX>
+int mnn_from_dots_as(const uint16_t *dots, const float *row_info, const float *col_info, int batch, int n, int m,
+                     int pitch, double epsilon, const float *u, const float *v, const float *kpts1, const float *kpts2,
+                     int max_matches, float threshold, void *workspace, size_t workspace_bytes,
+                     const uint32_t *solver_status, const MatchOut &out, hipStream_t s) {
+  ZSourceDots<MIX> src;
+  src.dots = dots;
+  src.pitch = pitch;
+  src.row_info = reinterpret_cast<const float2 *>(row_info);
+  src.neg_inv_eps = (float)(-1.0 / epsilon);
+  return mnn_from_source(src, reinterpret_cast<const float2 *>(col_info), batch, n, m, u, v, kpts1, kpts2, max_matches,
+                         threshold, workspace, workspace_bytes, solver_status, out, s);
+}
+
+int mnn_from_dots(const uint16_t *dots, const float *row_info, const float *col_info, int batch, int n, int m, int pitch,
+                  double epsilon, const float *u, const float *v, const float *kpts1, const float *kpts2,
+                  int max_matches, float threshold, void *workspace, size_t workspace_bytes,
+                  const uint32_t *solver_status, int flags, const MatchOut &out, hipStream_t s) {
+  if (!dots || !row_info || !col_info) return MI_E_NULL;
+  if (pitch < m || pitch % 8 != 0 || ((uintptr_t)dots % 16) != 0) return MI_E_ALIGN;
+  if (!(epsilon > 0.0) || (flags & ~MI_SOLVER_DOTS_BELOW_1024) != 0) return MI_E_PARAM;
+  if (solver_status && ((uintptr_t)solver_status % 4) != 0) return MI_E_ALIGN;
+  if ((flags & MI_SOLVER_DOTS_BELOW_1024) != 0 && epsilon >= MI_DOTS_MIN_EPSILON)
+    return mnn_from_dots_as<true>(dots, row_info, col_info, batch, n, m, pitch, epsilon, u, v, kpts1, kpts2, max_matches,
+                                  threshold, workspace, workspace_bytes, solver_status, out, s);
+  return mnn_from_dots_as<false>(dots, row_info, col_info, batch, n, m, pitch, epsilon, u, v, kpts1, kpts2, max_matches,
+                                 threshold, workspace, workspace_bytes, solver_status, out, s);
+}
+
+}
+
+extern "C" size_t mi_mnn_duals_workspace_bytes(int batch, int n, int m) {
+  if (batch <= 0 || n <= 0 || m <= 0 || m > 1024 || n > MX_MAX) return 0;
+  return duals_bytes(batch, n, m);
+}
+
+extern "C" int mi_mnn_from_duals(const float *z, int batch, int n, int m, int pitch, const float *u, const float *v,
+                                 const float *kpts1, const float *kpts2, int max_matches, float threshold,
+                                 void *workspace, size_t workspace_bytes, float *mk1, float *mk2, float *scores,
+                                 uint8_t *valid, int32_t *match_ij, mi_stream_t stream) {
+  MI_ENTER();
+  if (!mk1 || !mk2 || !scores) return MI_E_NULL;
+  return mnn_from_z(z, batch, n, m, pitch, u, v, kpts1, kpts2, max_matches, threshold, workspace, workspace_bytes,
+                    MatchOut{mk1, mk2, scores, nullptr, valid, match_ij}, (hipStream_t)stream);
+}
+
+extern "C" int mi_mnn_from_duals_records(const float *z, int batch, int n, int m, int pitch, const float *u,
+                                         const float *v, const float *kpts1, const float *kpts2, int max_matches,
+                                         float threshold, void *workspace, size_t workspace_bytes, float *record,
+                                         uint8_t *valid, int32_t *match_ij, mi_stream_t stream) {
+  MI_ENTER();
+  if (!record) return MI_E_NULL;
+  return mnn_from_z(z, batch, n, m, pitch, u, v, kpts1, kpts2, max_matches, threshold, workspace, workspace_bytes,
+                    MatchOut{nullptr, nullptr, nullptr, record, valid, match_ij}, (hipStream_t)stream);
 }
 
 extern "C" int mi_mnn_from_duals_dots(const uint16_t *dots, const float *row_info, const float *col_info, int batch,
@@ -488,19 +587,23 @@
                                       float *mk1, float *mk2, float *scores, uint8_t *valid, int32_t *match_ij,
                                       mi_stream_t stream) {
   MI_ENTER();
-  if (!dots || !row_info || !col_info) return MI_E_NULL;
-  if (pitch < m || pitch % 8 != 0 || ((uintptr_t)dots % 16) != 0) return MI_E_ALIGN;
-  if (!(epsilon > 0.0)) return MI_E_PARAM;
-  ZSourceDots src;
-  src.dots = dots;
-  src.pitch = pitch;
-  src.row_info = reinterpret_cast<const float2 *>(row_info);
-  src.col_info = reinterpret_cast<const float2 *>(col_info);
-  src.neg_inv_eps = (float)(-1.0 / epsilon);
-  src.ri = make_float2(0.f, 0.f);
-  if (solver_status && ((uintptr_t)solver_status % 4) != 0) return MI_E_ALIGN;
-  return mnn_from_source(src, src.col_info, batch, n, m, u, v, kpts1, kpts2, max_matches, threshold, workspace,
-                         workspace_bytes, solver_status, mk1, mk2, scores, valid, match_ij, (hipStream_t)stream);
+  if (!mk1 || !mk2 || !scores) return MI_E_NULL;
+  return mnn_from_dots(dots, row_info, col_info, batch, n, m, pitch, epsilon, u, v, kpts1, kpts2, max_matches, threshold,
+                       workspace, workspace_bytes, solver_status, 0, MatchOut{mk1, mk2, scores, nullptr, valid, match_ij},
+                       (hipStream_t)stream);
+}
+
+extern "C" int mi_mnn_from_duals_dots_records(const uint16_t *dots, const float *row_info, const float *col_info,
+                                              int batch, int n, int m, int pitch, double epsilon, const float *u,
+                                              const float *v, const float *kpts1, const float *kpts2, int max_matches,
+                                              float threshold, void *workspace, size_t workspace_bytes,
+                                              const uint32_t *solver_status, int flags, float *record, uint8_t *valid,
+                                              int32_t *match_ij, mi_stream_t stream) {
+  MI_ENTER();
+  if (!record) return MI_E_NULL;
+  return mnn_from_dots(dots, row_info, col_info, batch, n, m, pitch, epsilon, u, v, kpts1, kpts2, max_matches, threshold,
+                       workspace, workspace_bytes, solver_status, flags,
+                       MatchOut{nullptr, nullptr, nullptr, record, valid, match_ij}, (hipStream_t)stream);
 }
 
 extern "C" int mi_mnn_extract(const float *p, int batch, int n, int m, const float *kpts1, const float *kpts2,
@@ -528,7 +631,7 @@
   }
   hipLaunchKernelGGL(mnn_select_kernel, dim3(batch), dim3(MX_THREADS), 0, s, n, m, row_best, col_best,
                      (const uint64_t *)nullptr, 0, kpts1, kpts2, max_matches, threshold, (const uint32_t *)nullptr, mk1,
-                     mk2, scores, valid, match_ij);
+                     mk2, scores, (float *)nullptr, valid, match_ij);
   return mi_launch_status();
 }
 
diff --git a/onnx_image_processing_amd/csrc/sinkhorn_dots.hip b/onnx_image_processing_amd/csrc/sinkhorn_dots.hip
--- a/onnx_image_processing_amd/csrc/sinkhorn_dots.hip
+++ b/onnx_image_processing_amd/csrc/sinkhorn_dots.hip
@@ -76,16 +76,6 @@
   return (vold + ((j == m) ? log_n : 0.0f)) - lse;
 }
 
-__device__ __forceinline__ float mix_mul_lo(uint32_t w, float t) {
-  float p;
-  asm("v_fma_mix_f32 %0, %1, %2, 0 op_sel_hi:[1,0,0]" : "=v"(p) : "v"(w), "v"(t));
-  return p;
-}
-__device__ __forceinline__ float mix_mul_hi(uint32_t w, float t) {
-  float p;
-  asm("v_fma_mix_f32 %0, %1, %2, 0 op_sel:[1,0,0] op_sel_hi:[1,0,0]" : "=v"(p) : "v"(w), "v"(t));
-  return p;
-}
 
 template <int E8, int RW, int NW, bool FAST, bool MIX = false, bool SPLIT = false>
 __global__ __launch_bounds__(64 * NW) void sk_band_dots_kernel(const uint16_t *__restrict__ dots, int n, int m,
diff --git a/onnx_image_processing_amd/distributed.py b/onnx_image_processing_amd/distributed.py
--- a/onnx_image_processing_amd/distributed.py
+++ b/onnx_image_processing_amd/distributed.py
@@ -41,7 +41,35 @@
     return begin, begin + base + (1 if rank < extra else 0)
 
 
+def tag_record(rec: torch.Tensor, valid: torch.Tensor) -> None:
+    valid._mi_record = (rec, rec._version, valid._version)
+
+
+def _tagged_record(mk1: torch.Tensor, mk2: torch.Tensor, scores: torch.Tensor, valid: torch.Tensor):
+    tag = getattr(valid, "_mi_record", None)
+    if tag is None:
+        return None
+    rec, rec_version, valid_version = tag
+    if rec._version != rec_version or valid._version != valid_version:
+        return None
+    if rec.dtype != torch.float32 or rec.dim() != 3 or rec.shape[2] != RECORD_FIELDS or not rec.is_contiguous():
+        return None
+    b, mx, f = rec.shape
+    if tuple(valid.shape) != (b, mx) or valid.device != rec.device:
+        return None
+    off = rec.storage_offset()
+    for t, shape, stride, first in ((mk1, (b, mx, 2), (mx * f, f, 1), 0), (mk2, (b, mx, 2), (mx * f, f, 1), 2),
+                                    (scores, (b, mx), (mx * f, f), 4)):
+        if (t._base is not rec or tuple(t.shape) != shape or tuple(t.stride()) != stride
+                or t.storage_offset() != off + first):
+            return None
+    return rec
+
+
 def pack_records(mk1: torch.Tensor, mk2: torch.Tensor, scores: torch.Tensor, valid: torch.Tensor) -> torch.Tensor:
+    rec = _tagged_record(mk1, mk2, scores, valid)
+    if rec is not None:
+        return rec
     return torch.cat([mk1, mk2, scores.unsqueeze(-1), valid.to(scores.dtype).unsqueeze(-1)], dim=-1).contiguous()
 
 
diff --git a/onnx_image_processing_amd/ops.py b/onnx_image_processing_amd/ops.py
--- a/onnx_image_processing_amd/ops.py
+++ b/onnx_image_processing_amd/ops.py
@@ -3,6 +3,7 @@
 import torch
 
 from . import _native as N
+from .distributed import RECORD_FIELDS, tag_record
 
 F32 = torch.float32
 
@@ -341,6 +342,10 @@
     return epsilon >= DOTS_MIN_EPSILON and int(N.load().mi_sinkhorn_dots_workspace_bytes(b, n, m)) > 0
 
 
+class DotsState(tuple):
+    num_bits = None
+
+
 def sinkhorn_bits(bits1: torch.Tensor, bits2: torch.Tensor, normalized: bool, epsilon: float, unused_score: float,
                   iterations: int, return_duals: bool = False, want_p: bool = True, return_state: bool = False):
     b, n, words = bits1.shape
@@ -370,7 +375,9 @@
            _solver_flags | (MI_SOLVER_DOTS_BELOW_1024 if words * 32 < 1024 else 0), N.stream_ptr())
     if return_state:
         status = N.load().mi_sinkhorn_dots_status_word(work.data_ptr(), b, n, m)
-        return p, u, v, (dots, row_info, col_info, pitch, (work, status))
+        state = DotsState((dots, row_info, col_info, pitch, (work, status)))
+        state.num_bits = words * 32
+        return p, u, v, state
     return (p, u, v) if (return_duals or not want_p) else p
 
 
@@ -416,14 +423,20 @@
     return out + (ij,) if return_indices else out
 
 
-def _mnn_outputs(b, max_matches, dev):
-    return (torch.empty((b, max_matches, 2), dtype=F32, device=dev), torch.empty((b, max_matches, 2), dtype=F32, device=dev),
-            torch.empty((b, max_matches), dtype=F32, device=dev), torch.empty((b, max_matches), dtype=torch.bool, device=dev),
-            torch.empty((b, max_matches, 2), dtype=torch.int32, device=dev))
-
-
 def mnn_duals_supported(b: int, n: int, m: int) -> bool:
     return int(N.load().mi_mnn_duals_workspace_bytes(b, n, m)) > 0
+
+
+def _mnn_record_outputs(b, max_matches, dev):
+    return (torch.empty((b, max_matches, RECORD_FIELDS), dtype=F32, device=dev),
+            torch.empty((b, max_matches), dtype=torch.bool, device=dev),
+            torch.empty((b, max_matches, 2), dtype=torch.int32, device=dev))
+
+
+def _mnn_record_views(rec, valid, ij, return_indices):
+    tag_record(rec, valid)
+    out = (rec[..., 0:2], rec[..., 2:4], rec[..., 4], valid)
+    return out + (ij,) if return_indices else out
 
 
 def mnn_from_duals(z: torch.Tensor, m: int, pitch: int, u: torch.Tensor, v: torch.Tensor, kpts1: torch.Tensor,
@@ -434,32 +447,34 @@
     if wbytes == 0:
         raise RuntimeError(f"mnn_from_duals supports N <= 4096 and M <= 1024, got ({n}, {m})")
     work = torch.empty((wbytes // 8,), dtype=torch.int64, device=z.device)
-    mk1, mk2, sc, valid, ij = _mnn_outputs(b, max_matches, z.device)
-    N.call("mi_mnn_from_duals", N.dev(z, F32, "z"), b, n, m, pitch, N.dev(u, F32, "u"), N.dev(v, F32, "v"),
+    rec, valid, ij = _mnn_record_outputs(b, max_matches, z.device)
+    N.call("mi_mnn_from_duals_records", N.dev(z, F32, "z"), b, n, m, pitch, N.dev(u, F32, "u"), N.dev(v, F32, "v"),
            N.dev(k1, F32, "keypoints1"), N.dev(k2, F32, "keypoints2"), int(max_matches), float(threshold),
-           work.data_ptr(), wbytes, mk1.data_ptr(), mk2.data_ptr(), sc.data_ptr(), valid.data_ptr(), ij.data_ptr(),
-           N.stream_ptr())
-    out = (mk1, mk2, sc, valid)
-    return out + (ij,) if return_indices else out
+           work.data_ptr(), wbytes, rec.data_ptr(), valid.data_ptr(), ij.data_ptr(), N.stream_ptr())
+    return _mnn_record_views(rec, valid, ij, return_indices)
 
 
 def mnn_from_duals_dots(state, m: int, epsilon: float, u: torch.Tensor, v: torch.Tensor, kpts1: torch.Tensor,
-                        kpts2: torch.Tensor, max_matches: int, threshold: float, return_indices: bool = False):
+                        kpts2: torch.Tensor, max_matches: int, threshold: float, return_indices: bool = False,
+                        dots_below_1024: bool | None = None):
     dots, row_info, col_info, pitch = state[:4]
     status = state[4][1] if len(state) > 4 else None
+    if dots_below_1024 is None:
+        num_bits = getattr(state, "num_bits", None)
+        dots_below_1024 = num_bits is not None and num_bits < 1024
     b, n, _ = dots.shape
     k1, k2 = kpts1.float().contiguous(), kpts2.float().contiguous()
     wbytes = int(N.load().mi_mnn_duals_workspace_bytes(b, n, m))
     if wbytes == 0:
         raise RuntimeError(f"mnn_from_duals_dots supports N <= 4096 and M <= 1024, got ({n}, {m})")
     work = torch.empty((wbytes // 8,), dtype=torch.int64, device=dots.device)
-    mk1, mk2, sc, valid, ij = _mnn_outputs(b, max_matches, dots.device)
-    N.call("mi_mnn_from_duals_dots", dots.data_ptr(), row_info.data_ptr(), col_info.data_ptr(), b, n, m, pitch,
+    rec, valid, ij = _mnn_record_outputs(b, max_matches, dots.device)
+    N.call("mi_mnn_from_duals_dots_records", dots.data_ptr(), row_info.data_ptr(), col_info.data_ptr(), b, n, m, pitch,
            float(epsilon), N.dev(u, F32, "u"), N.dev(v, F32, "v"), N.dev(k1, F32, "keypoints1"),
            N.dev(k2, F32, "keypoints2"), int(max_matches), float(threshold), work.data_ptr(), wbytes, status,
-           mk1.data_ptr(), mk2.data_ptr(), sc.data_ptr(), valid.data_ptr(), ij.data_ptr(), N.stream_ptr())
-    out = (mk1, mk2, sc, valid)
-    return out + (ij,) if return_indices else out
+           MI_SOLVER_DOTS_BELOW_1024 if dots_below_1024 else 0, rec.data_ptr(), valid.data_ptr(), ij.data_ptr(),
+           N.stream_ptr())
+    return _mnn_record_views(rec, valid, ij, return_indices)
 
 
 
```

After: 218,900 image-pairs/sec (median of 6 runs). 1.5% higher.
